# nooice98/HM16.9-NN_FME

Hardware: AMD Instinct MI355X
Metric: sub-pel PU refinements/sec @ 1080p lowdelay_P QP22; bit-exact MV/SATD vs HM (higher is better)
Workload: dtype int16/int32 (NN f32)

## Files before the change

### hm16.9-nn_fme_amd/csrc/fme_api.cpp

```cpp
#include <dlfcn.h>
#include <hsa/hsa.h>
#include <hsa/hsa_ext_amd.h>

#include <chrono>
#include <cmath>
#include <cstdarg>
#include <cstdio>
#include <memory>

#include "fme_ctx.h"

using namespace fme;

namespace {
thread_local std::string g_last_error = "";
}


int fme::fail(int code, const char* fmt, ...) {
  char buf[512];
  va_list ap;
  va_start(ap, fmt);
  vsnprintf(buf, sizeof(buf), fmt, ap);
  va_end(ap);
  g_last_error = buf;
  return code;
}


extern "C" {

int fme_abi_version(void) { return FME_ABI_VERSION; }

const char* fme_last_error(void) { return g_last_error.c_str(); }

int fme_create(int device, const fme_config* cfg, fme_ctx** out_ctx) {
  if (!cfg || !out_ctx) return fail(FME_E_INVALID, "fme_create: null argument");
  *out_ctx = nullptr;
  if (cfg->bit_depth != 8 && cfg->bit_depth != 10)
    return fail(FME_E_UNSUPPORTED, "fme_create: bit_depth %d (8, or 10 for the main10 configurations)", cfg->bit_depth);
  if (cfg->nn_mode < 0 || cfg->nn_mode > 2) return fail(FME_E_INVALID, "fme_create: nn_mode %d", cfg->nn_mode);
  int ndev = 0;
  HIP_TRY(hipGetDeviceCount(&ndev));
  if (device < 0 || device >= ndev) return fail(FME_E_INVALID, "fme_create: device %d of %d", device, ndev);
  HIP_TRY(hipSetDevice(device));
  std::unique_ptr<fme_ctx> c(new fme_ctx());
  c->device = device;
  c->cfg = *cfg;
  HIP_TRY(c->d_pics.reserve(kOvSlots * FME_MAX_PICTURES));
  HIP_TRY(c->d_mlambda.reserve(kOvSlots * FME_MAX_LAMBDAS));
  HIP_TRY(c->d_nn.reserve(kNnPkFloats));
  HIP_TRY(c->counts.reserve(kOvBlocks * kCountWords));
  HIP_TRY(hipMemset(c->counts.p, 0, kOvBlocks * kCountWords * sizeof(int32_t)));
  HIP_TRY(c->d_sched.reserve(kOvSlots));
  HIP_TRY(hipMemset(c->d_sched.p, 0, kOvSlots * sizeof(Schedule)));
  for (auto& e : c->done_ev) HIP_TRY(hipEventCreateWithFlags(&e, hipEventDisableTiming));
  c->sched_p = sched_params();
  {
    const char* m10 = std::getenv("FME_MAIN10_SEARCH");
    c->main10_px = m10 && std::strcmp(m10, "px") == 0;
  }
  HIP_TRY(c->nn_state.reserve(24));
  HIP_TRY(hipMemset(c->nn_state.p, 0, 24 * sizeof(uint32_t)));
  HIP_TRY(c->d_key_invalid.reserve(1));
  HIP_TRY(hipMemset(c->d_key_invalid.p, 0, sizeof(int32_t)));
  HIP_TRY(hipHostMalloc(reinterpret_cast<void**>(&c->h_counts), kCountWords * sizeof(int32_t), hipHostMallocDefault));
  if (cfg->max_jobs > 0) {
    const size_t n = (size_t)cfg->max_jobs;
    const size_t nb = (n + kJobsPerScanBlock - 1) / kJobsPerScanBlock;
    if (n * kNumClasses > (size_t)INT32_MAX) return fail(FME_E_INVALID, "fme_create: max_jobs %d", cfg->max_jobs);
    for (int b = 0; b < kOvSlots; b++) {
      HIP_TRY(c->cls[b].reserve(n));
      HIP_TRY(c->perm[b].reserve(n * kNumClasses));
      HIP_TRY(c->blk_agg[b].reserve(nb * 9));
      HIP_TRY(c->blk_prefix[b].reserve(nb * 9));
    }
  }
  *out_ctx = c.release();
  return FME_OK;
}

}
static int srv_stop(fme_ctx* c);
static hipEvent_t done_event(const fme_ctx* c, int back) {
  if (back < 1 || back > 2 || !c->ov.live[back - 1]) return nullptr;
  return c->done_ev[(c->ov.seq - back) % fme_ctx::kDoneRing];
}
static int wait_batches(fme_ctx* c, hipStream_t s) {
  for (int back = 1; back <= 2; back++)
    if (hipEvent_t e = done_event(c, back))
      if (c->ov.stream[back - 1] != s) HIP_TRY(hipStreamWaitEvent(s, e, 0));
  return FME_OK;
}
static void note_stream(fme_ctx* c, hipStream_t s) {
  for (int i = 0; i < c->n_used_streams; i++)
    if (c->used_streams[i] == s) return;
  if (c->n_used_streams < fme_ctx::kMaxStreams) c->used_streams[c->n_used_streams++] = s;
  else c->used_overflow = true;
}
static int drain_ctx(fme_ctx* c) {
  if (c->used_overflow) {
    HIP_TRY(hipDeviceSynchronize());
  } else {
    for (int i = 0; i < c->n_used_streams; i++) HIP_TRY(hipStreamSynchronize(c->used_streams[i]));
  }
  return FME_OK;
}
int fme::grow_keys(fme_ctx* c, size_t n) {
  c->keys_fresh = true;
  if (n <= c->d_keys.cap) return FME_OK;
  FME_TRY(drain_ctx(c));
  HIP_TRY(c->d_keys.reserve(n));
  return FME_OK;
}
extern "C" {
int fme_destroy(fme_ctx* c) {
  if (!c) return FME_OK;
  (void)hipSetDevice(c->device);
  (void)srv_stop(c);
  (void)hipDeviceSynchronize();
  for (int i = 0; i < FME_MAX_PICTURES; i++)
    if (c->pic_owned[i] && c->pics[i].luma) (void)hipFree(const_cast<uint8_t*>(c->pics[i].luma));
  for (int i = 0; i < FME_MAX_PICTURES; i++)
    if (c->chroma_owned[i]) (void)hipFree(c->chroma_owned[i]);
  c->d_mc_jobs.release(); c->d_mc_planes.release(); c->d_mc_invalid.release(); c->d_mc_wp.release();
  c->d_tz_ext.release(); c->d_tz_sad.release(); c->d_tz_nn_in.release();
  c->d_amvp.release(); c->d_amvp_sad.release(); c->d_bikey.release(); c->d_key_invalid.release(); c->d_ch_i32.release(); c->d_tz_emi.release();
  c->h_pi_tasks.release(); c->h_pi_tsad.release(); c->h_pi_jobs.release(); c->h_pi_ext.release();
  c->h_pi_idx.release(); c->h_pi_psrc.release(); c->h_pi_mv.release(); c->h_pi_last.release();
  c->h_pi_ures.release(); c->h_pi_seq.release(); c->h_pi_rs.release(); c->h_pi_rows.release();
  c->d_pi_jobs.release(); c->d_pi_ext.release(); c->d_pi_idx.release();
  for (auto& e : c->ev_tz)
    if (e) (void)hipEventDestroy(e);
  for (auto& e : c->ev_mc)
    if (e) (void)hipEventDestroy(e);
  c->d_pe_tasks.release(); c->d_pe_dist.release(); c->d_pe_invalid.release();
  for (auto& e : c->ev_pe)
    if (e) (void)hipEventDestroy(e);
  c->d_sse_tasks.release(); c->d_sse_out.release(); c->d_sse_invalid.release();
  for (auto& e : c->ev_sse)
    if (e) (void)hipEventDestroy(e);
  c->d_surf_jobs.release(); c->d_surf_probe.release(); c->d_surf_out.release(); c->d_surf_pick.release();
  c->d_surf_invalid.release();
  for (auto& e : c->ev_surf)
    if (e) (void)hipEventDestroy(e);
  c->d_pics.release(); c->d_mlambda.release(); c->d_keys.release(); c->d_nn.release(); c->d_net.release();
  c->d_jobs.release(); c->d_res.release(); c->d_res1.release(); c->d_mv.release();
  for (int b = 0; b < kOvSlots; b++) {
    c->koff[b].release(); c->cls[b].release(); c->perm[b].release(); c->blk_agg[b].release(); c->blk_prefix[b].release();
  }
  c->counts.release(); c->nn_state.release();
  c->d_sched.release();
  for (auto& e : c->done_ev)
    if (e) (void)hipEventDestroy(e);
  for (auto& e : c->state_read_ev)
    if (e) (void)hipEventDestroy(e);
  if (c->stage) (void)hipHostFree(c->stage);
  if (c->single_stream) (void)hipStreamDestroy(c->single_stream);
  if (c->box) (void)hipHostFree(c->box);
  if (c->srv_stream) (void)hipStreamDestroy(c->srv_stream);
  if (c->h_counts) (void)hipHostFree(c->h_counts);
  if (c->h_tab) (void)hipHostFree(c->h_tab);
  for (auto& e : c->tab_ev)
    if (e) (void)hipEventDestroy(e);
  for (auto& set : c->ev)
    for (auto& e : set)
      if (e) (void)hipEventDestroy(e);
  if (c->ev_fork) (void)hipEventDestroy(c->ev_fork);
  if (c->ev_join2) (void)hipEventDestroy(c->ev_join2);
  if (c->aux2) (void)hipStreamDestroy(c->aux2);
  if (c->ev_join) (void)hipEventDestroy(c->ev_join);
  if (c->aux) (void)hipStreamDestroy(c->aux);
  delete c;
  return FME_OK;
}

static void keep_chroma(fme_ctx* c, int id, int width, int height) {
  const PicDesc& o = c->pics[id];
  if (o.luma && o.width == width && o.height == height) return;
  if (c->chroma_owned[id]) (void)hipFree(c->chroma_owned[id]);
  c->chroma_owned[id] = nullptr;
  c->chroma_bytes[id] = 0;
  c->pics[id].cb = c->pics[id].cr = nullptr;
  c->pics[id].cstride = 0;
}

int fme_set_picture(fme_ctx* c, int id, const uint8_t* luma, int stride, int width, int height, void* stream) {
  if (!c || !luma) return fail(FME_E_INVALID, "fme_set_picture: null argument");
  if (id < 0 || id >= FME_MAX_PICTURES) return fail(FME_E_INVALID, "fme_set_picture: id %d", id);
  if (width <= 0 || height <= 0 || stride < width || width > 65535 || height > 65535)
    return fail(FME_E_INVALID, "fme_set_picture: %dx%d stride %d", width, height, stride);
  HIP_TRY(hipSetDevice(c->device));
  const size_t bps = c->cfg.bit_depth > 8 ? 2 : 1;
  const size_t bytes = (size_t)width * height * bps;
  uint8_t* dst = c->pic_owned[id] ? const_cast<uint8_t*>(c->pics[id].luma) : nullptr;
  if (!dst || c->pic_bytes[id] < bytes) {
    if (dst) HIP_TRY(hipFree(dst));
    dst = nullptr;
    HIP_TRY(hipMalloc(reinterpret_cast<void**>(&dst), bytes));
    c->pic_bytes[id] = bytes;
  }
  hipStream_t s = static_cast<hipStream_t>(stream);
  HIP_TRY(hipMemcpy2DAsync(dst, width * bps, luma, stride * bps, width * bps, height, hipMemcpyHostToDevice, s));
  HIP_TRY(hipStreamSynchronize(s));
  keep_chroma(c, id, width, height);
  c->pics[id] = PicDesc{dst, width, width, height, c->pics[id].cb, c->pics[id].cr, c->pics[id].cstride, 0};
  c->pic_owned[id] = true;
  c->tables_dirty = true;
  return FME_OK;
}

int fme_bind_picture_device(fme_ctx* c, int id, const uint8_t* d_luma, int stride, int width, int height) {
  if (!c || !d_luma) return fail(FME_E_INVALID, "fme_bind_picture_device: null argument");
  if (id < 0 || id >= FME_MAX_PICTURES) return fail(FME_E_INVALID, "fme_bind_picture_device: id %d", id);
  if (width <= 0 || height <= 0 || stride < width) return fail(FME_E_INVALID, "fme_bind_picture_device: geometry");
  HIP_TRY(hipSetDevice(c->device));
  if (c->pic_owned[id] && c->pics[id].luma) HIP_TRY(hipFree(const_cast<uint8_t*>(c->pics[id].luma)));
  c->pic_owned[id] = false;
  c->pic_bytes[id] = 0;
  keep_chroma(c, id, width, height);
  c->pics[id] = PicDesc{d_luma, stride, width, height, c->pics[id].cb, c->pics[id].cr, c->pics[id].cstride, 0};
  c->tables_dirty = true;
  return FME_OK;
}

int fme_set_picture_chroma(fme_ctx* c, int id, const uint8_t* cb, const uint8_t* cr, int stride, void* stream) {
  if (!c || !cb || !cr) return fail(FME_E_INVALID, "fme_set_picture_chroma: null argument");
  if (id < 0 || id >= FME_MAX_PICTURES) return fail(FME_E_INVALID, "fme_set_picture_chroma: id %d", id);
  if (!c->pics[id].luma) return fail(FME_E_STATE, "fme_set_picture_chroma: picture %d has no luma plane", id);
  const int cw = c->pics[id].width >> 1, ch = c->pics[id].height >> 1;
  if (stride < cw) return fail(FME_E_INVALID, "fme_set_picture_chroma: stride %d < %d", stride, cw);
  HIP_TRY(hipSetDevice(c->device));
  const size_t bps = c->cfg.bit_depth > 8 ? 2 : 1;
  const size_t bytes = 2 * (size_t)cw * ch * bps;
  if (!c->chroma_owned[id] || c->chroma_bytes[id] < bytes) {
    if (c->chroma_owned[id]) HIP_TRY(hipFree(c->chroma_owned[id]));
    c->chroma_owned[id] = nullptr;
    HIP_TRY(hipMalloc(reinterpret_cast<void**>(&c->chroma_owned[id]), bytes));
    c->chroma_bytes[id] = bytes;
  }
  uint8_t* dcb = c->chroma_owned[id];
  uint8_t* dcr = dcb + (size_t)cw * ch * bps;
  hipStream_t s = static_cast<hipStream_t>(stream);
  HIP_TRY(hipMemcpy2DAsync(dcb, cw * bps, cb, stride * bps, cw * bps, ch, hipMemcpyHostToDevice, s));
  HIP_TRY(hipMemcpy2DAsync(dcr, cw * bps, cr, stride * bps, cw * bps, ch, hipMemcpyHostToDevice, s));
  HIP_TRY(hipStreamSynchronize(s));
  c->pics[id].cb = dcb;
  c->pics[id].cr = dcr;
  c->pics[id].cstride = cw;
  c->tables_dirty = true;
  return FME_OK;
}

int fme_bind_picture_chroma_device(fme_ctx* c, int id, const uint8_t* d_cb, const uint8_t* d_cr, int stride) {
  if (!c || !d_cb || !d_cr) return fail(FME_E_INVALID, "fme_bind_picture_chroma_device: null argument");
  if (id < 0 || id >= FME_MAX_PICTURES) return fail(FME_E_INVALID, "fme_bind_picture_chroma_device: id %d", id);
  if (!c->pics[id].luma) return fail(FME_E_STATE, "fme_bind_picture_chroma_device: picture %d has no luma plane", id);
  if (stride < (c->pics[id].width >> 1)) return fail(FME_E_INVALID, "fme_bind_picture_chroma_device: stride %d", stride);
  HIP_TRY(hipSetDevice(c->device));
  if (c->chroma_owned[id]) HIP_TRY(hipFree(c->chroma_owned[id]));
  c->chroma_owned[id] = nullptr;
  c->chroma_bytes[id] = 0;
  c->pics[id].cb = d_cb;
  c->pics[id].cr = d_cr;
  c->pics[id].cstride = stride;
  c->tables_dirty = true;
  return FME_OK;
}

int fme_set_lambda(fme_ctx* c, int id, double lambda) {
  if (!c || id < 0 || id >= FME_MAX_LAMBDAS || !(lambda >= 0.0)) return fail(FME_E_INVALID, "fme_set_lambda: bad argument");
  const double sq = std::sqrt(lambda);
  c->mlambda[id] = 65536.0 * sq + 0;
  c->lambda_set[id] = true;
  c->tables_dirty = true;
  return FME_OK;
}

int fme_set_motion_lambda(fme_ctx* c, int id, double ml) {
  if (!c || id < 0 || id >= FME_MAX_LAMBDAS || !(ml >= 0.0)) return fail(FME_E_INVALID, "fme_set_motion_lambda: bad argument");
  c->mlambda[id] = ml;
  c->lambda_set[id] = true;
  c->tables_dirty = true;
  return FME_OK;
}

int fme_set_keys(fme_ctx* c, const int16_t* keys, size_t count, void* stream) {
  if (!c || (!keys && count)) return fail(FME_E_INVALID, "fme_set_keys: null argument");
  HIP_TRY(hipSetDevice(c->device));
  FME_TRY(srv_stop(c));
  FME_TRY(grow_keys(c, count));
  hipStream_t s = static_cast<hipStream_t>(stream);
  FME_TRY(wait_batches(c, s));
  if (count) HIP_TRY(hipMemcpyAsync(c->d_keys.p, keys, count * sizeof(int16_t), hipMemcpyHostToDevice, s));
  HIP_TRY(hipMemsetAsync(c->d_key_invalid.p, 0, sizeof(int32_t), s));
  HIP_TRY(hipStreamSynchronize(s));
  c->n_keys = count;
  return FME_OK;
}

int fme_load_nn_weights(fme_ctx* c, const float* params, int count) {
  if (!c || !params) return fail(FME_E_INVALID, "fme_load_nn_weights: null argument");
  if (count != FME_NN_PARAMS) return fail(FME_E_INVALID, "fme_load_nn_weights: %d params, expected %d", count, FME_NN_PARAMS);
  HIP_TRY(hipSetDevice(c->device));
  std::vector<float> packed(kNnPkFloats);
  nn_pack(params, packed.data());
  HIP_TRY(hipMemcpy(c->d_nn.p, packed.data(), kNnPkFloats * sizeof(float), hipMemcpyHostToDevice));
  c->nn_loaded = true;
  c->nn_gen++;
  return FME_OK;
}

int fme_nn_param_count(const fme_nn_net* n) {
  if (!n) return fail(FME_E_INVALID, "fme_nn_param_count: null descriptor");
  if (n->n_hidden < 1 || n->n_hidden > FME_NN_MAX_HIDDEN)
    return fail(FME_E_INVALID, "fme_nn_param_count: n_hidden %d", n->n_hidden);
  if (n->precision != FME_NN_F32 && n->precision != FME_NN_F64)
    return fail(FME_E_INVALID, "fme_nn_param_count: precision %d", n->precision);
  if (n->embedding < FME_NN_EMB_NONE || n->embedding > FME_NN_EMB_SWAP)
    return fail(FME_E_INVALID, "fme_nn_param_count: embedding %d", n->embedding);
  if (n->out_act != FME_NN_OUT_LINEAR && n->out_act != FME_NN_OUT_SIGMOID)
    return fail(FME_E_INVALID, "fme_nn_param_count: out_act %d", n->out_act);
  if (n->carry_hidden >> n->n_hidden) return fail(FME_E_INVALID, "fme_nn_param_count: carry_hidden 0x%x", n->carry_hidden);
  if (n->input_flags & ~(FME_NN_IN_SLOT_RESET | FME_NN_IN_TZ_RING))
    return fail(FME_E_INVALID, "fme_nn_param_count: input_flags 0x%x", n->input_flags);
  if ((n->input_flags & FME_NN_IN_TZ_RING) && ((n->input_flags & FME_NN_IN_SLOT_RESET) || n->carry_hidden))
    return fail(FME_E_INVALID, "fme_nn_param_count: FME_NN_IN_TZ_RING with FME_NN_IN_SLOT_RESET or carry_hidden");
  int count = n->embedding ? 64 : 0, fan = n->embedding ? 17 : 9;
  for (int l = 0; l < n->n_hidden; l++) {
    const int w = n->width[l];
    if (w < 1 || w > FME_NN_MAX_WIDTH) return fail(FME_E_INVALID, "fme_nn_param_count: width[%d] = %d", l, w);
    count += w * fan + 3 * w;
    fan = w;
  }
  return count + 49 * fan + 49 + 27;
}

int fme_load_nn_net(fme_ctx* c, const fme_nn_net* n, const double* params, int count) {
  if (!c || !n || !params) return fail(FME_E_INVALID, "fme_load_nn_net: null argument");
  const int need = fme_nn_param_count(n);
  if (need < 0) return need;
  if (count != need) return fail(FME_E_INVALID, "fme_load_nn_net: %d params, the descriptor needs %d", count, need);
  if (n->carry_hidden)
    return fail(FME_E_UNSUPPORTED, "fme_load_nn_net: carry_hidden 0x%x (hidden layers carried across calls) is not "
                "supported by the batch engines", n->carry_hidden);
  HIP_TRY(hipSetDevice(c->device));
  const size_t bytes = nn_deep_packed_bytes(*n);
  if (!bytes) return fail(FME_E_UNSUPPORTED, "fme_load_nn_net: no kernel for this net");
  std::vector<unsigned char> packed(bytes);
  nn_deep_pack(*n, params, packed.data());
  FME_TRY(drain_ctx(c));
  HIP_TRY(c->d_net.reserve(bytes));
  HIP_TRY(hipMemcpy(c->d_net.p, packed.data(), bytes, hipMemcpyHostToDevice));
  c->net = *n;
  c->net_loaded = true;
  return FME_OK;
}

int fme_set_nn_engine(fme_ctx* c, int engine) {
  if (!c || (engine != FME_NN_ENGINE_EXACT && engine != FME_NN_ENGINE_MFMA))
    return fail(FME_E_INVALID, "fme_set_nn_engine: bad argument");
  c->nn_engine = engine;
  return FME_OK;
}

int fme_set_nn_logit_output(fme_ctx* c, void* d_logits, int capacity) {
  if (!c) return fail(FME_E_INVALID, "fme_set_nn_logit_output: null ctx");
  if (d_logits && capacity <= 0) return fail(FME_E_INVALID, "fme_set_nn_logit_output: capacity %d", capacity);
  c->nn_logits = capacity > 0 ? d_logits : nullptr;
  c->nn_logits_cap = d_logits ? capacity : 0;
  return FME_OK;
}

int fme_set_nn_inputs(fme_ctx* c, const uint32_t* d_rows, int capacity) {
  if (!c) return fail(FME_E_INVALID, "fme_set_nn_inputs: null ctx");
  if (d_rows && capacity <= 0) return fail(FME_E_INVALID, "fme_set_nn_inputs: capacity %d", capacity);
  c->nn_in = capacity > 0 ? d_rows : nullptr;
  c->nn_in_cap = d_rows ? capacity : 0;
  return FME_OK;
}

int fme_set_nn_margin_output(fme_ctx* c, float* d_margin, int capacity) {
  if (!c) return fail(FME_E_INVALID, "fme_set_nn_margin_output: null ctx");
  if (d_margin && capacity <= 0) return fail(FME_E_INVALID, "fme_set_nn_margin_output: capacity %d", capacity);
  c->nn_margin = capacity > 0 ? d_margin : nullptr;
  c->nn_margin_cap = d_margin ? capacity : 0;
  return FME_OK;
}

int fme_nn_reset_state(fme_ctx* c) {
  if (!c) return fail(FME_E_INVALID, "fme_nn_reset_state: null ctx");
  for (uint32_t& v : c->pending_state) v = 0;
  c->state_pending = true;
  return FME_OK;
}

int fme_nn_get_state(fme_ctx* c, uint32_t* out12) {
  if (!c || !out12) return fail(FME_E_INVALID, "fme_nn_get_state: null argument");
  if (c->state_pending) {
    std::memcpy(out12, c->pending_state, sizeof(c->pending_state));
    return FME_OK;
  }
  HIP_TRY(hipSetDevice(c->device));
  FME_TRY(drain_ctx(c));
  HIP_TRY(hipMemcpy(out12, c->nn_state.p + 12 * c->state_cur, 12 * sizeof(uint32_t), hipMemcpyDeviceToHost));
  return FME_OK;
}

int fme_nn_set_state(fme_ctx* c, const uint32_t* in12) {
  if (!c || !in12) return fail(FME_E_INVALID, "fme_nn_set_state: null argument");
  std::memcpy(c->pending_state, in12, sizeof(c->pending_state));
  c->state_pending = true;
  return FME_OK;
}

int fme_nn_copy_state_device(fme_ctx* c, uint32_t* d_out12, void* stream) {
  if (!c || !d_out12) return fail(FME_E_INVALID, "fme_nn_copy_state_device: null argument");
  HIP_TRY(hipSetDevice(c->device));
  hipStream_t s = static_cast<hipStream_t>(stream);
  if (c->state_pending) {
    HIP_TRY(launch_put_state(d_out12, c->pending_state, s));
    return FME_OK;
  }
  FME_TRY(wait_batches(c, s));
  HIP_TRY(hipMemcpyAsync(d_out12, c->nn_state.p + 12 * c->state_cur, 12 * sizeof(uint32_t),
                         hipMemcpyDeviceToDevice, s));
  hipEvent_t& e = c->state_read_ev[c->state_reads++ % fme_ctx::kDoneRing];
  if (!e) HIP_TRY(hipEventCreateWithFlags(&e, hipEventDisableTiming));
  HIP_TRY(hipEventRecord(e, s));
  c->state_read_last = e;
  c->state_read_stream = s;
  return FME_OK;
}

}

static int ensure_work(fme_ctx* c, int n, bool* grows = nullptr) {
  const size_t nb = ((size_t)n + kJobsPerScanBlock - 1) / kJobsPerScanBlock;
  if ((size_t)n * kNumClasses > (size_t)INT32_MAX) return fail(FME_E_INVALID, "%d jobs in one batch", n);
  if (grows) *grows = (size_t)n > c->cls[0].cap || (size_t)n > c->koff[0].cap;
  for (int b = 0; b < kOvSlots; b++) {
    HIP_TRY(c->cls[b].reserve(n));
    HIP_TRY(c->perm[b].reserve((size_t)n * kNumClasses));
    HIP_TRY(c->blk_agg[b].reserve(nb * 9));
    HIP_TRY(c->blk_prefix[b].reserve(nb * 9));
    HIP_TRY(c->koff[b].reserve(n));
  }
  return FME_OK;
}

static WorkBufs work_bufs(fme_ctx* c, int slot, int block, int zeroed) {
  WorkBufs w{};
  w.cls = c->cls[slot].p;
  w.perm = c->perm[slot].p;
  w.perm_cap = (int32_t)(c->perm[slot].cap / kNumClasses);
  w.koff = c->koff[slot].p;
  w.counts = c->counts.p + block * kCountWords;
  w.counts_next = c->counts.p + zeroed * kCountWords;
  w.cursor = w.counts + kCursorWord;
  w.tile_ctr = w.counts + kTileCtrWord;
  w.blk_agg = c->blk_agg[slot].p;
  w.blk_prefix = c->blk_prefix[slot].p;
  w.nn_state = c->nn_state.p;
  w.sched = c->d_sched.p + slot;
  w.mv_out = nullptr;
  return w;
}

BatchArgs fme::batch_args(const fme_ctx* c, const fme_job* jobs, int n) {
  BatchArgs a{};
  a.jobs = jobs;
  a.keys = c->d_keys.p;
  a.n_keys = (int64_t)c->n_keys;
  a.key_invalid = c->d_key_invalid.p;
  a.mlambda = c->d_mlambda.p;
  a.pics = c->d_pics.p;
  a.n = n;
  a.use_hadamard = c->cfg.use_hadamard ? 1 : 0;
  a.fen = c->cfg.fast_inter_mode;
  return a;
}

static int put_tables(fme_ctx* c, int slot, hipStream_t s) {
  note_stream(c, s);
  FME_TRY(srv_stop(c));
  if (c->tables_dirty) {
    c->tab_gen++;
    c->tables_dirty = false;
  }
  if (c->slot_gen[slot] == c->tab_gen) return FME_OK;
  if (!c->h_tab) {
    void* p = nullptr;
    HIP_TRY(hipHostMalloc(&p, fme_ctx::kTabSlots * sizeof(TablesSlot), hipHostMallocMapped));
    c->h_tab = static_cast<TablesSlot*>(p);
    void* d = nullptr;
    HIP_TRY(hipHostGetDevicePointer(&d, p, 0));
    c->h_tab_dev = static_cast<TablesSlot*>(d);
    for (auto& e : c->tab_ev) HIP_TRY(hipEventCreateWithFlags(&e, hipEventDisableTiming));
  }
  const int k = c->tab_next;
  c->tab_next = (k + 1) % fme_ctx::kTabSlots;
  if (c->tab_used[k]) HIP_TRY(hipEventSynchronize(c->tab_ev[k]));
  std::memcpy(c->h_tab[k].pics, c->pics, sizeof(c->pics));
  std::memcpy(c->h_tab[k].ml, c->mlambda, sizeof(c->mlambda));
  HIP_TRY(launch_put_tables(c->d_pics.p + slot * FME_MAX_PICTURES, c->d_mlambda.p + slot * FME_MAX_LAMBDAS,
                            c->h_tab_dev + k, s));
  HIP_TRY(hipEventRecord(c->tab_ev[k], s));
  c->tab_used[k] = true;
  c->slot_gen[slot] = c->tab_gen;
  return FME_OK;
}

int fme::sync_tables(fme_ctx* c, hipStream_t s) {
  FME_TRY(wait_batches(c, s));
  return put_tables(c, 0, s);
}

static int batch_begin(fme_ctx* c, const OverlapPlan& plan, hipStream_t s, hipEvent_t* done) {
  hipEvent_t const prev_done = done_event(c, 1), slot_done = done_event(c, 2);
  *done = c->done_ev[c->ov.seq % fme_ctx::kDoneRing];
  if (c->ov.seq >= fme_ctx::kDoneRing)
    HIP_TRY(hipEventSynchronize(c->done_ev[(c->ov.seq + 2) % fme_ctx::kDoneRing]));
  if (plan.wait_prev_front) HIP_TRY(hipStreamWaitEvent(s, prev_done, 0));
  if (plan.wait_slot) HIP_TRY(hipStreamWaitEvent(s, slot_done, 0));
  if (plan.fill_blocks) {
    FME_TRY(drain_ctx(c));
    HIP_TRY(hipMemsetAsync(c->counts.p, 0, kOvBlocks * kCountWords * sizeof(int32_t), s));
  }
  return FME_OK;
}

static int apply_pending_state(fme_ctx* c, hipStream_t s) {
  if (!c->state_pending) return FME_OK;
  HIP_TRY(launch_put_state(c->nn_state.p + 12 * c->state_cur, c->pending_state, s));
  c->state_pending = false;
  return FME_OK;
}

static int harvest_events(fme_ctx* c, bool wait_all) {
  while (c->ev_tail != c->ev_head) {
    const int b = c->ev_tail % fme_ctx::kEvSets;
    hipEvent_t* e = c->ev[b];
    if (wait_all) {
      HIP_TRY(hipEventSynchronize(e[6]));
    } else {
      const hipError_t q = hipEventQuery(e[6]);
      if (q == hipErrorNotReady) break;
      HIP_TRY(q);
    }
    float* ms = c->last_ms;
    HIP_TRY(hipEventElapsedTime(&ms[0], e[0], e[3]));
    ms[1] = 0.f;
    HIP_TRY(hipEventElapsedTime(&ms[2], e[3], e[5]));
    HIP_TRY(hipEventElapsedTime(&ms[3], e[5], e[6]));
    HIP_TRY(hipEventElapsedTime(&ms[4], e[0], e[6]));
    HIP_TRY(hipEventElapsedTime(&ms[5], e[3], e[4]));
    ms[6] = 0.f;
    for (int i = 0; i < FME_NUM_TIMINGS; i++) c->acc_ms[i] += ms[i];
    c->acc_batches++;
    c->timed = true;
    c->ev_tail++;
  }
  return FME_OK;
}

int fme::refine_batch(fme_ctx* c, const fme_job* d_jobs, fme_result* d_res, fme_mv_result* d_mv, int n,
                      hipStream_t s, const fme_job_packed* d_pjobs, const int32_t* d_key_base) {
  if (c->cfg.nn_mode == 1 && !c->nn_loaded) return fail(FME_E_STATE, "fme_refine_device: nn_mode set but no weights loaded");
  if (c->cfg.nn_mode == 2 && !c->net_loaded) return fail(FME_E_STATE, "fme_refine_device: nn_mode 2 but no net loaded");
  if (c->cfg.nn_mode == 2 && c->nn_margin && n > c->nn_margin_cap)
    return fail(FME_E_INVALID, "fme_refine: %d jobs but the margin output holds %d", n, c->nn_margin_cap);
  if (c->cfg.nn_mode == 2 && c->nn_logits && n > c->nn_logits_cap)
    return fail(FME_E_INVALID, "fme_refine: %d jobs but the logit output holds %d", n, c->nn_logits_cap);
  HIP_TRY(hipSetDevice(c->device));
  bool grows = false;
  FME_TRY(ensure_work(c, n, &grows));
  const uint32_t features = (c->keys_fresh ? kOvKeys : 0u) | (c->cfg.nn_mode == 2 ? kOvDeepNn : 0u) |
                            (c->cfg.bit_depth > 8 && c->main10_px ? kOvPx : 0u) |
                            (d_jobs && d_jobs == c->d_jobs.p ? kOvStaged : 0u) | (grows ? kOvGrow : 0u);
  const OverlapPlan plan = overlap_plan(c->ov, s, features);
  hipEvent_t const prev_done = done_event(c, 1);
  hipEvent_t done = nullptr;
  FME_TRY(batch_begin(c, plan, s, &done));
  FME_TRY(put_tables(c, plan.slot, s));

  BatchArgs a = batch_args(c, d_jobs, n);
  a.pics = c->d_pics.p + plan.slot * FME_MAX_PICTURES;
  a.mlambda = c->d_mlambda.p + plan.slot * FME_MAX_LAMBDAS;
  a.pjobs = d_jobs ? nullptr : d_pjobs;
  a.key_base = d_key_base;
  a.koff = c->koff[plan.slot].p;
  a.res = d_res;
  a.nn_mode = c->cfg.nn_mode ? 1 : 0;
  a.nn_in = c->nn_in;
  a.nn_in_cap = c->nn_in_cap;
  WorkBufs w = work_bufs(c, plan.slot, plan.block, plan.block_zeroed);
  w.mv_out = d_mv;

  const bool prof = c->profiling;
  hipEvent_t* ev = nullptr;
  int eb = 0;
  if (prof) {
    FME_TRY(harvest_events(c, false));
    if (c->ev_head - c->ev_tail == fme_ctx::kEvSets) {
      HIP_TRY(hipEventSynchronize(c->ev[c->ev_tail % fme_ctx::kEvSets][6]));
      FME_TRY(harvest_events(c, false));
    }
    eb = c->ev_head % fme_ctx::kEvSets;
    ev = c->ev[eb];
    HIP_TRY(hipEventRecord(ev[0], s));
  }
  overlap_begin(c->ov);
  HIP_TRY(launch_front(a, w, c->sched_p, s));
  if (prof) HIP_TRY(hipEventRecord(ev[3], s));
  if (c->ev_search) HIP_TRY(hipEventRecord(c->ev_search, s));
  if (c->cfg.bit_depth > 8) {
    if (c->main10_px)
      HIP_TRY(launch_search_px(a, w, c->cfg.bit_depth, s, nullptr));
    else
      HIP_TRY(launch_search_lane10(a, w, s));
  } else {
    HIP_TRY(launch_search_lane(a, w, c->search_reserve, s));
  }
  if (prof) HIP_TRY(hipEventRecord(ev[4], s));
  if (plan.wait_prev_tail) HIP_TRY(hipStreamWaitEvent(s, prev_done, 0));
  if (c->state_read_last) {
    if (c->state_read_stream != s) HIP_TRY(hipStreamWaitEvent(s, c->state_read_last, 0));
    c->state_read_last = nullptr;
  }
  FME_TRY(apply_pending_state(c, s));
  if (prof) HIP_TRY(hipEventRecord(ev[5], s));
  HIP_TRY(c->cfg.nn_mode == 2
              ? launch_nn_deep_tail(c->net, c->d_net.p, c->nn_margin, c->nn_logits, a, w, c->state_cur, c->nn_engine, s)
              : launch_nn_tail(a, w, c->d_nn.p, c->state_cur, s));
  if (prof) {
    HIP_TRY(hipEventRecord(ev[6], s));
    c->ev_head++;
  }
  HIP_TRY(hipEventRecord(done, s));
  c->ev_done = done;
  c->last_slot = plan.slot;
  c->keys_fresh = false;
  overlap_commit(c->ov, s, features, plan);
  c->batch_issued = true;
  if (a.nn_mode) c->state_cur ^= 1;
  return FME_OK;
}

int fme::check_rejected(fme_ctx* c, hipStream_t s, const char* name, const char* what) {
  HIP_TRY(hipMemcpyAsync(c->h_counts, &c->d_sched.p[c->last_slot].invalid, sizeof(int32_t), hipMemcpyDeviceToHost, s));
  HIP_TRY(hipStreamSynchronize(s));
  if (c->h_counts[0] > 0)
    return fail(FME_E_INVALID, "%s: %d job(s) %s", name, c->h_counts[0], what);
  return FME_OK;
}

static int slot_records(fme_ctx* c, int n, fme_result** out) {
  DevBuf<fme_result>& b = c->ov.seq % kOvSlots ? c->d_res1 : c->d_res;
  HIP_TRY(b.reserve(n));
  *out = b.p;
  return FME_OK;
}

extern "C" {

int fme_refine_device(fme_ctx* c, const fme_job* d_jobs, fme_result* d_res, int n, void* stream) {
  if (!c || (n > 0 && (!d_jobs || !d_res))) return fail(FME_E_INVALID, "fme_refine_device: null argument");
  if (n < 0) return fail(FME_E_INVALID, "fme_refine_device: n = %d", n);
  if (n == 0) return FME_OK;
  return refine_batch(c, d_jobs, d_res, nullptr, n, static_cast<hipStream_t>(stream));
}

int fme_refine_mv_device(fme_ctx* c, const fme_job* d_jobs, fme_mv_result* d_out, int n, void* stream) {
  if (!c || (n > 0 && (!d_jobs || !d_out))) return fail(FME_E_INVALID, "fme_refine_mv_device: null argument");
  if (n < 0) return fail(FME_E_INVALID, "fme_refine_mv_device: n = %d", n);
  if (n == 0) return FME_OK;
  HIP_TRY(hipSetDevice(c->device));
  fme_result* d_res = nullptr;
  FME_TRY(slot_records(c, n, &d_res));
  return refine_batch(c, d_jobs, d_res, d_out, n, static_cast<hipStream_t>(stream));
}

int fme_pack_jobs(const fme_job* jobs, int n, fme_job_packed* out, int32_t* key_base) {
  if (n < 0 || (n > 0 && (!jobs || !out || !key_base))) return fail(FME_E_INVALID, "fme_pack_jobs: bad argument");
  const int waves = (n + FME_PACK_WAVE - 1) / FME_PACK_WAVE;
  for (int wv = 0; wv < waves; wv++) {
    int64_t next = -1;
    key_base[wv] = -1;
    const int e = std::min(n, (wv + 1) * FME_PACK_WAVE);
    for (int i = wv * FME_PACK_WAVE; i < e; i++) {
      const fme_job& j = jobs[i];
      const char* why = nullptr;
      if ((j.x & 3) || (j.y & 3) || (j.w & 3) || (j.h & 3) || j.w < 4 || j.w > 64 || j.h < 4 || j.h > 64)
        why = "PU off the 4x4 grid or not 4..64";
      else if (j.x >= 8192 || j.y >= 8192) why = "x or y >= 8192";
      else if (j.org_id >= 64 || j.ref_id >= 64 || j.lambda_id >= 32) why = "slot id >= 64 or lambda_id >= 32";
      else if (j.flags & ~15u) why = "unknown flags";
      else if (j.bits_in >= 64) why = "bits_in >= 64";
      else if (j.mv_x <= -32767 || j.mv_x >= 32766 || j.mv_y <= -32767 || j.mv_y >= 32766) why = "int16-extreme mv";
      else if (j.key_offset >= 0) {
        if (next < 0) key_base[wv] = j.key_offset;
        else if ((int64_t)j.key_offset != next) why = "key block not dense in job order within its wave";
        next = (int64_t)j.key_offset + (int64_t)j.w * j.h;
      }
      if (why) return fail(FME_E_UNSUPPORTED, "fme_pack_jobs: job %d: %s (use fme_job)", i, why);
      uint32_t rg = 0;
      if (j.mv_y - 1 >= j.lt_y) rg |= FME_PK_RANGE_TOP;
      if (j.mv_y + 1 <= j.rb_y) rg |= FME_PK_RANGE_BOTTOM;
      if (j.mv_x - 1 >= j.lt_x) rg |= FME_PK_RANGE_LEFT;
      if (j.mv_x + 1 <= j.rb_x) rg |= FME_PK_RANGE_RIGHT;
      fme_job_packed p;
      p.pu = (uint32_t)(j.x >> 2) | ((uint32_t)(j.y >> 2) << 11) | ((uint32_t)((j.w >> 2) - 1) << 22) |
             ((uint32_t)((j.h >> 2) - 1) << 26);
      p.ctl = (uint32_t)j.org_id | ((uint32_t)j.ref_id << 6) | ((uint32_t)j.lambda_id << 12) |
              ((uint32_t)j.flags << 17) | ((uint32_t)(j.key_offset >= 0) << 21) | (rg << 22) |
              ((uint32_t)j.bits_in << 26);
      p.mv_x = j.mv_x;
      p.mv_y = j.mv_y;
      p.mvp_x = j.mvp_x;
      p.mvp_y = j.mvp_y;
      out[i] = p;
    }
  }
  return FME_OK;
}

int fme_unpack_jobs(const fme_job_packed* packed, const int32_t* key_base, int n, fme_job* out) {
  if (n < 0 || (n > 0 && (!packed || !key_base || !out))) return fail(FME_E_INVALID, "fme_unpack_jobs: bad argument");
  int64_t next = 0;
  for (int i = 0; i < n; i++) {
    const fme_job_packed& p = packed[i];
    if (i % FME_PACK_WAVE == 0) next = key_base[i / FME_PACK_WAVE];
    fme_job j;
    j.x = (uint16_t)((p.pu & 2047u) * 4u);
    j.y = (uint16_t)(((p.pu >> 11) & 2047u) * 4u);
    j.w = (uint8_t)((((p.pu >> 22) & 15u) + 1u) * 4u);
    j.h = (uint8_t)((((p.pu >> 26) & 15u) + 1u) * 4u);
    j.org_id = (uint8_t)(p.ctl & 63u);
    j.ref_id = (uint8_t)((p.ctl >> 6) & 63u);
    j.lambda_id = (uint8_t)((p.ctl >> 12) & 31u);
    j.flags = (uint8_t)((p.ctl >> 17) & 15u);
    const uint32_t rg = (p.ctl >> 22) & 15u;
    j.bits_in = (uint16_t)(p.ctl >> 26);
    j.mv_x = p.mv_x;
    j.mv_y = p.mv_y;
    j.mvp_x = p.mvp_x;
    j.mvp_y = p.mvp_y;
    j.lt_x = (int16_t)(p.mv_x - ((rg & FME_PK_RANGE_LEFT) ? 1 : 0));
    j.rb_x = (int16_t)(p.mv_x + ((rg & FME_PK_RANGE_RIGHT) ? 1 : 0));
    j.lt_y = (int16_t)(p.mv_y - ((rg & FME_PK_RANGE_TOP) ? 1 : 0));
    j.rb_y = (int16_t)(p.mv_y + ((rg & FME_PK_RANGE_BOTTOM) ? 1 : 0));
    if ((p.ctl >> 21) & 1u) {
      j.key_offset = (int32_t)next;
      next += (int64_t)j.w * j.h;
    } else {
      j.key_offset = -1;
    }
    out[i] = j;
  }
  return FME_OK;
}

static int refine_packed(fme_ctx* c, const fme_job_packed* d_jobs, const int32_t* d_key_base, fme_result* d_res,
                         fme_mv_result* d_mv, int n, void* stream, const char* fn) {
  if (!c || (n > 0 && (!d_jobs || !d_key_base || !(d_res || d_mv)))) return fail(FME_E_INVALID, "%s: null argument", fn);
  if (n < 0) return fail(FME_E_INVALID, "%s: n = %d", fn, n);
  if (n == 0) return FME_OK;
  HIP_TRY(hipSetDevice(c->device));
  if (!d_res) FME_TRY(slot_records(c, n, &d_res));
  return refine_batch(c, nullptr, d_res, d_mv, n, static_cast<hipStream_t>(stream), d_jobs, d_key_base);
}

int fme_refine_packed_device(fme_ctx* c, const fme_job_packed* d_jobs, const int32_t* d_key_base, fme_result* d_res,
                             int n, void* stream) {
  if (c && n > 0 && !d_res) return fail(FME_E_INVALID, "fme_refine_packed_device: null argument");
  return refine_packed(c, d_jobs, d_key_base, d_res, nullptr, n, stream, "fme_refine_packed_device");
}

int fme_refine_mv_packed_device(fme_ctx* c, const fme_job_packed* d_jobs, const int32_t* d_key_base,
                                fme_mv_result* d_out, int n, void* stream) {
  if (c && n > 0 && !d_out) return fail(FME_E_INVALID, "fme_refine_mv_packed_device: null argument");
  return refine_packed(c, d_jobs, d_key_base, nullptr, d_out, n, stream, "fme_refine_mv_packed_device");
}

int fme_set_search_event(fme_ctx* c, void* event) {
  if (!c) return fail(FME_E_INVALID, "fme_set_search_event: null ctx");
  c->ev_search = static_cast<hipEvent_t>(event);
  return FME_OK;
}

int fme_set_search_reserve(fme_ctx* c, int workgroups) {
  if (!c || workgroups < 0 || workgroups > 4096) return fail(FME_E_INVALID, "fme_set_search_reserve: bad argument");
  c->search_reserve = workgroups;
  return FME_OK;
}

int fme_download_device(fme_ctx* c, const void* d_src, void* h_dst, size_t bytes, int workgroups, void* stream) {
  if (!c || (bytes && (!d_src || !h_dst))) return fail(FME_E_INVALID, "fme_download_device: null argument");
  if ((bytes & 15) || (reinterpret_cast<uintptr_t>(d_src) & 15) || (reinterpret_cast<uintptr_t>(h_dst) & 15))
    return fail(FME_E_INVALID, "fme_download_device: pointers and size must be 16-byte multiples");
  if (workgroups < 0 || workgroups > 1024) return fail(FME_E_INVALID, "fme_download_device: %d workgroups", workgroups);
  if (!bytes) return FME_OK;
  HIP_TRY(hipSetDevice(c->device));
  void* dst = nullptr;
  if (hipHostGetDevicePointer(&dst, h_dst, 0) != hipSuccess || !dst) {
    (void)hipGetLastError();
    return fail(FME_E_INVALID, "fme_download_device: h_dst is not pinned host memory");
  }
  HIP_TRY(launch_download(d_src, dst, bytes / 16, workgroups ? workgroups : 8, static_cast<hipStream_t>(stream)));
  return FME_OK;
}

namespace {
struct HsaCopyApi {
  hsa_status_t (*iterate_agents)(hsa_status_t (*)(hsa_agent_t, void*), void*);
  hsa_status_t (*agent_get_info)(hsa_agent_t, hsa_agent_info_t, void*);
  hsa_status_t (*signal_create)(hsa_signal_value_t, uint32_t, const hsa_agent_t*, hsa_signal_t*);
  hsa_status_t (*signal_destroy)(hsa_signal_t);
  hsa_signal_value_t (*signal_wait)(hsa_signal_t, hsa_signal_condition_t, hsa_signal_value_t, uint64_t,
                                    hsa_wait_state_t);
  hsa_status_t (*copy_on_engine)(void*, hsa_agent_t, const void*, hsa_agent_t, size_t, uint32_t,
                                 const hsa_signal_t*, hsa_signal_t, hsa_amd_sdma_engine_id_t, bool);
};
bool hsa_copy_api(HsaCopyApi& a) {
  void* h = dlopen("libhsa-runtime64.so.1", RTLD_LAZY | RTLD_NOLOAD);
  if (!h) h = dlopen("libhsa-runtime64.so.1", RTLD_LAZY);
  if (!h) return false;
  a.iterate_agents = reinterpret_cast<decltype(a.iterate_agents)>(dlsym(h, "hsa_iterate_agents"));
  a.agent_get_info = reinterpret_cast<decltype(a.agent_get_info)>(dlsym(h, "hsa_agent_get_info"));
  a.signal_create = reinterpret_cast<decltype(a.signal_create)>(dlsym(h, "hsa_signal_create"));
  a.signal_destroy = reinterpret_cast<decltype(a.signal_destroy)>(dlsym(h, "hsa_signal_destroy"));
  a.signal_wait = reinterpret_cast<decltype(a.signal_wait)>(dlsym(h, "hsa_signal_wait_scacquire"));
  a.copy_on_engine = reinterpret_cast<decltype(a.copy_on_engine)>(dlsym(h, "hsa_amd_memory_async_copy_on_engine"));
  return a.iterate_agents && a.agent_get_info && a.signal_create && a.signal_destroy && a.signal_wait &&
         a.copy_on_engine;
}
struct AgentPick {
  const HsaCopyApi* api;
  uint32_t bdf, domain;
  bool have_gpu = false, have_cpu = false;
  hsa_agent_t gpu{}, cpu{};
};
hsa_status_t pick_agent(hsa_agent_t ag, void* data) {
  AgentPick* p = static_cast<AgentPick*>(data);
  hsa_device_type_t t;
  if (p->api->agent_get_info(ag, HSA_AGENT_INFO_DEVICE, &t) != HSA_STATUS_SUCCESS) return HSA_STATUS_SUCCESS;
  if (t == HSA_DEVICE_TYPE_CPU && !p->have_cpu) {
    p->cpu = ag;
    p->have_cpu = true;
  } else if (t == HSA_DEVICE_TYPE_GPU && !p->have_gpu) {
    uint32_t bdf = 0, dom = 0;
    p->api->agent_get_info(ag, static_cast<hsa_agent_info_t>(HSA_AMD_AGENT_INFO_BDFID), &bdf);
    p->api->agent_get_info(ag, static_cast<hsa_agent_info_t>(HSA_AMD_AGENT_INFO_DOMAIN), &dom);
    if (bdf == p->bdf && dom == p->domain) {
      p->gpu = ag;
      p->have_gpu = true;
    }
  }
  return HSA_STATUS_SUCCESS;
}
}

int fme_warm_copy_engines(fme_ctx* c, int* engines) {
  if (!c) return fail(FME_E_INVALID, "fme_warm_copy_engines: null ctx");
  if (engines) *engines = 0;
  HIP_TRY(hipSetDevice(c->device));
  HsaCopyApi api{};
  if (!hsa_copy_api(api)) return fail(FME_E_DEVICE, "fme_warm_copy_engines: HSA runtime symbols not found");
  int bus = 0, dev = 0, dom = 0;
  HIP_TRY(hipDeviceGetAttribute(&bus, hipDeviceAttributePciBusId, c->device));
  HIP_TRY(hipDeviceGetAttribute(&dev, hipDeviceAttributePciDeviceId, c->device));
  HIP_TRY(hipDeviceGetAttribute(&dom, hipDeviceAttributePciDomainID, c->device));
  AgentPick pk{&api, (uint32_t)((bus << 8) | (dev << 3)), (uint32_t)dom};
  api.iterate_agents(pick_agent, &pk);
  if (!pk.have_gpu || !pk.have_cpu) return fail(FME_E_DEVICE, "fme_warm_copy_engines: HSA agents not found");
  uint32_t n_sdma = 0, n_xgmi = 0;
  api.agent_get_info(pk.gpu, static_cast<hsa_agent_info_t>(HSA_AMD_AGENT_INFO_NUM_SDMA_ENG), &n_sdma);
  api.agent_get_info(pk.gpu, static_cast<hsa_agent_info_t>(HSA_AMD_AGENT_INFO_NUM_SDMA_XGMI_ENG), &n_xgmi);
  const int n_eng = std::min(16, (int)(n_sdma + n_xgmi));
  constexpr size_t kBytes = 4096;
  void* d = nullptr;
  void* h = nullptr;
  HIP_TRY(hipMalloc(&d, kBytes));
  if (hipHostMalloc(&h, kBytes, hipHostMallocDefault) != hipSuccess) {
    (void)hipFree(d);
    return fail(FME_E_NOMEM, "fme_warm_copy_engines: host buffer");
  }
  std::memset(h, 0, kBytes);
  int warmed = 0;
  for (int e = 0; e < n_eng; e++) {
    bool ok = true;
    for (int dir = 0; dir < 2 && ok; dir++) {
      hsa_signal_t sig;
      if (api.signal_create(1, 0, nullptr, &sig) != HSA_STATUS_SUCCESS) {
        ok = false;
        break;
      }
      const auto eid = static_cast<hsa_amd_sdma_engine_id_t>(1u << e);
      const hsa_status_t st = dir == 0 ? api.copy_on_engine(d, pk.gpu, h, pk.cpu, kBytes, 0, nullptr, sig, eid, true)
                                       : api.copy_on_engine(h, pk.cpu, d, pk.gpu, kBytes, 0, nullptr, sig, eid, true);
      if (st == HSA_STATUS_SUCCESS)
        api.signal_wait(sig, HSA_SIGNAL_CONDITION_LT, 1, UINT64_MAX, HSA_WAIT_STATE_BLOCKED);
      else
        ok = false;
      api.signal_destroy(sig);
    }
    warmed += ok ? 1 : 0;
  }
  (void)hipHostFree(h);
  (void)hipFree(d);
  if (engines) *engines = warmed;
  return FME_OK;
}

int fme_refine_status(fme_ctx* c) {
  if (!c) return fail(FME_E_INVALID, "fme_refine_status: null ctx");
  if (!c->batch_issued) return 0;
  HIP_TRY(hipSetDevice(c->device));
  HIP_TRY(hipEventSynchronize(c->ev_done));
  int32_t v = 0;
  HIP_TRY(hipMemcpy(&v, &c->d_sched.p[c->last_slot].invalid, sizeof(v), hipMemcpyDeviceToHost));
  return v;
}

int fme_debug_front(fme_ctx* c, int32_t* perm_out, long long perm_words, int32_t* sched_out, int sched_words,
                    int32_t* cap_out) {
  if (!c || !c->batch_issued) return fail(FME_E_STATE, "fme_debug_front: no batch issued");
  if (perm_words < 0 || (size_t)perm_words > c->perm[c->last_slot].cap || sched_words < 0 ||
      (size_t)sched_words * sizeof(int32_t) > sizeof(Schedule))
    return fail(FME_E_INVALID, "fme_debug_front: length");
  HIP_TRY(hipSetDevice(c->device));
  HIP_TRY(hipEventSynchronize(c->ev_done));
  if (perm_out && perm_words) HIP_TRY(hipMemcpy(perm_out, c->perm[c->last_slot].p, (size_t)perm_words * sizeof(int32_t), hipMemcpyDeviceToHost));
  if (sched_out && sched_words) HIP_TRY(hipMemcpy(sched_out, c->d_sched.p + c->last_slot, (size_t)sched_words * sizeof(int32_t), hipMemcpyDeviceToHost));
  if (cap_out) *cap_out = (int32_t)(c->perm[c->last_slot].cap / kNumClasses);
  return FME_OK;
}

}

int fme::tz_run(fme_ctx* c, fme_job* d_jobs, const fme_tz_ext* d_ext, uint32_t* d_sad, int n, void* stream,
                int16_t* d_emi, uint32_t* d_nn_in, int ext_stride) {
  if (!c || (n > 0 && (!d_jobs || !d_ext))) return fail(FME_E_INVALID, "fme_integer_search_device: null argument");
  if (n < 0) return fail(FME_E_INVALID, "fme_integer_search_device: n = %d", n);
  if (n == 0) return FME_OK;
  int cw = 0, ch = 0, npic = 0;
  for (int i = 0; i < FME_MAX_PICTURES; i++)
    if (c->pics[i].luma) {
      cw = std::max(cw, (c->pics[i].width + 63) / 64);
      ch = std::max(ch, (c->pics[i].height + 63) / 64);
      npic = i + 1;
    }
  const long long np = (long long)npic * cw * ch;
  if (np > kTzMaxPairs)
    return fail(FME_E_UNSUPPORTED, "fme_integer_search_device: %lld (picture slot, CTU) pairs (%d slots x %d x %d CTUs), the limit is %lld",
                np, npic, cw, ch, kTzMaxPairs);
  HIP_TRY(hipSetDevice(c->device));
  hipStream_t s = static_cast<hipStream_t>(stream);
  FME_TRY(ensure_work(c, n));
  FME_TRY(sync_tables(c, s));
  BatchArgs a = batch_args(c, d_jobs, n);
  a.nn_in = c->nn_in;
  a.nn_in_cap = c->nn_in_cap;
  const OverlapPlan plan = overlap_plan(c->ov, s, kOvForeign);
  hipEvent_t done = nullptr;
  FME_TRY(batch_begin(c, plan, s, &done));
  WorkBufs w = work_bufs(c, plan.slot, plan.block, plan.block_zeroed);
  if (c->profiling) {
    if (!c->ev_tz[0]) {
      HIP_TRY(hipEventCreate(&c->ev_tz[0]));
      HIP_TRY(hipEventCreate(&c->ev_tz[1]));
    }
  }
  overlap_begin(c->ov);
  HIP_TRY(launch_classify(a, w, s));
  HIP_TRY(hipMemcpyAsync(c->h_counts, w.counts, kCountWords * sizeof(int32_t), hipMemcpyDeviceToHost, s));
  HIP_TRY(hipStreamSynchronize(s));
  if (c->h_counts[kNumClasses] > 0)
    return fail(FME_E_INVALID, "fme_integer_search_device: %d job(s) with an unsupported PU size or unset picture/lambda/key",
                c->h_counts[kNumClasses]);
  const bool keyed = c->h_counts[kKeyedWord] > 0;
  HIP_TRY(launch_scatter(a, w, c->sched_p, s));
  TzArgs ta{};
  ta.a = a;
  ta.perm = w.perm;
  ta.jobs_out = d_jobs;
  ta.ext = d_ext;
  ta.ext_stride = ext_stride;
  ta.sad = d_sad;
  ta.emi_mv = d_emi;
  ta.nn_in = d_nn_in;
  if (c->profiling) HIP_TRY(hipEventRecord(c->ev_tz[0], s));
  if (!c->aux) HIP_TRY(hipStreamCreateWithFlags(&c->aux, hipStreamNonBlocking));
  if (!c->aux2) HIP_TRY(hipStreamCreateWithFlags(&c->aux2, hipStreamNonBlocking));
  if (!c->ev_fork) HIP_TRY(hipEventCreateWithFlags(&c->ev_fork, hipEventDisableTiming));
  if (!c->ev_join) HIP_TRY(hipEventCreateWithFlags(&c->ev_join, hipEventDisableTiming));
  if (!c->ev_join2) HIP_TRY(hipEventCreateWithFlags(&c->ev_join2, hipEventDisableTiming));
  const size_t words = 8 + 12 * (size_t)np;
  if (c->d_tzp.cap < words || c->d_tzp_perm.cap < (size_t)n) {
    FME_TRY(drain_ctx(c));
    HIP_TRY(c->d_tzp.reserve(words));
    HIP_TRY(c->d_tzp_perm.reserve(n));
  }
  TzPairs tp{};
  int32_t* b = c->d_tzp.p;
  tp.nseg = b;
  tp.cnt = b + 8;
  tp.cursor = tp.cnt + 3 * np;
  tp.off = tp.cursor + 3 * np;
  tp.seg = tp.off + 3 * np;
  tp.perm = c->d_tzp_perm.p;
  tp.np = (int32_t)np;
  tp.cw = cw;
  tp.ch = ch;
  HIP_TRY(hipMemsetAsync(b, 0, (8 + 3 * (size_t)np) * sizeof(int32_t), s));
  HIP_TRY(launch_tz_pairs(ta, tp, w.cls, n, s));
  HIP_TRY(hipEventRecord(c->ev_fork, s));
  HIP_TRY(hipStreamWaitEvent(c->aux, c->ev_fork, 0));
  HIP_TRY(hipStreamWaitEvent(c->aux2, c->ev_fork, 0));
  HIP_TRY(launch_tz_staged(ta, tp, 0, keyed, c->cfg.bit_depth, c->aux));
  HIP_TRY(launch_tz_staged(ta, tp, 1, keyed, c->cfg.bit_depth, c->aux2));
  HIP_TRY(launch_tz_staged(ta, tp, 2, keyed, c->cfg.bit_depth, s));
  HIP_TRY(hipEventRecord(c->ev_join, c->aux));
  HIP_TRY(hipEventRecord(c->ev_join2, c->aux2));
  HIP_TRY(hipStreamWaitEvent(s, c->ev_join, 0));
  HIP_TRY(hipStreamWaitEvent(s, c->ev_join2, 0));
  if (c->profiling) HIP_TRY(hipEventRecord(c->ev_tz[1], s));
  c->tz_timed = c->profiling;
  HIP_TRY(hipEventRecord(done, s));
  overlap_commit(c->ov, s, kOvForeign, plan);
  return FME_OK;
}

static int tz_run_host(fme_ctx* c, fme_job* jobs, const fme_tz_ext* ext, uint32_t* sad, int n, void* stream,
                       int16_t* emi, uint32_t* nn_in = nullptr, int ext_stride = (int)sizeof(fme_tz_ext)) {
  if (!c || (n > 0 && (!jobs || !ext))) return fail(FME_E_INVALID, "fme_integer_search: null argument");
  if (n <= 0) return n == 0 ? FME_OK : fail(FME_E_INVALID, "fme_integer_search: n = %d", n);
  HIP_TRY(hipSetDevice(c->device));
  hipStream_t s = static_cast<hipStream_t>(stream);
  HIP_TRY(c->d_jobs.reserve(n));
  HIP_TRY(c->d_tz_ext.reserve(((size_t)n * ext_stride + sizeof(fme_tz_ext) - 1) / sizeof(fme_tz_ext)));
  HIP_TRY(c->d_tz_sad.reserve(n));
  if (emi) HIP_TRY(c->d_tz_emi.reserve((size_t)2 * n));
  if (nn_in) HIP_TRY(c->d_tz_nn_in.reserve((size_t)9 * n));
  HIP_TRY(hipMemcpyAsync(c->d_jobs.p, jobs, (size_t)n * sizeof(fme_job), hipMemcpyHostToDevice, s));
  HIP_TRY(hipMemcpyAsync(c->d_tz_ext.p, ext, (size_t)n * ext_stride, hipMemcpyHostToDevice, s));
  if (nn_in) HIP_TRY(hipMemcpyAsync(c->d_tz_nn_in.p, nn_in, (size_t)9 * n * sizeof(uint32_t), hipMemcpyHostToDevice, s));
  int rc = tz_run(c, c->d_jobs.p, c->d_tz_ext.p, c->d_tz_sad.p, n, stream, emi ? c->d_tz_emi.p : nullptr,
                  nn_in ? c->d_tz_nn_in.p : nullptr, ext_stride);
  if (rc) return rc;
  HIP_TRY(hipMemcpyAsync(jobs, c->d_jobs.p, (size_t)n * sizeof(fme_job), hipMemcpyDeviceToHost, s));
  if (sad) HIP_TRY(hipMemcpyAsync(sad, c->d_tz_sad.p, (size_t)n * sizeof(uint32_t), hipMemcpyDeviceToHost, s));
  if (emi) HIP_TRY(hipMemcpyAsync(emi, c->d_tz_emi.p, (size_t)n * 2 * sizeof(int16_t), hipMemcpyDeviceToHost, s));
  if (nn_in) HIP_TRY(hipMemcpyAsync(nn_in, c->d_tz_nn_in.p, (size_t)9 * n * sizeof(uint32_t), hipMemcpyDeviceToHost, s));
  HIP_TRY(hipStreamSynchronize(s));
  return FME_OK;
}

extern "C" {

int fme_integer_search_device(fme_ctx* c, fme_job* d_jobs, const fme_tz_ext* d_ext, uint32_t* d_sad, int n,
                              void* stream) {
  return tz_run(c, d_jobs, d_ext, d_sad, n, stream, nullptr);
}

int fme_integer_search(fme_ctx* c, fme_job* jobs, const fme_tz_ext* ext, uint32_t* sad, int n, void* stream) {
  return tz_run_host(c, jobs, ext, sad, n, stream, nullptr);
}

int fme_integer_search2_device(fme_ctx* c, fme_job* d_jobs, const fme_tz_ext2* d_ext, uint32_t* d_sad, int n,
                               void* stream) {
  return tz_run(c, d_jobs, reinterpret_cast<const fme_tz_ext*>(d_ext), d_sad, n, stream, nullptr, nullptr,
                (int)sizeof(fme_tz_ext2));
}

int fme_integer_search2(fme_ctx* c, fme_job* jobs, const fme_tz_ext2* ext, uint32_t* sad, int n, void* stream) {
  return tz_run_host(c, jobs, reinterpret_cast<const fme_tz_ext*>(ext), sad, n, stream, nullptr, nullptr,
                     (int)sizeof(fme_tz_ext2));
}

int fme_integer_search_ring_device(fme_ctx* c, fme_job* d_jobs, const fme_tz_ext* d_ext, uint32_t* d_sad,
                                   uint32_t* d_nn_in, int n, void* stream) {
  if (!d_nn_in && n > 0) return fail(FME_E_INVALID, "fme_integer_search_ring_device: null nn_in");
  return tz_run(c, d_jobs, d_ext, d_sad, n, stream, nullptr, d_nn_in);
}

int fme_integer_search_ring(fme_ctx* c, fme_job* jobs, const fme_tz_ext* ext, uint32_t* sad, uint32_t* nn_in,
                            int n, void* stream) {
  if (!nn_in && n > 0) return fail(FME_E_INVALID, "fme_integer_search_ring: null nn_in");
  return tz_run_host(c, jobs, ext, sad, n, stream, nullptr, nn_in);
}

int fme_integer_search_last_ms(fme_ctx* c, float* ms) {
  if (!c || !ms) return fail(FME_E_INVALID, "fme_integer_search_last_ms: null argument");
  if (!c->tz_timed) return fail(FME_E_STATE, "fme_integer_search_last_ms: no profiled integer search");
  HIP_TRY(hipEventSynchronize(c->ev_tz[1]));
  HIP_TRY(hipEventElapsedTime(ms, c->ev_tz[0], c->ev_tz[1]));
  return FME_OK;
}

static int refine_host(fme_ctx* c, const fme_job* jobs, fme_result* res, fme_mv_result* mv, int n, void* stream,
                       const char* name) {
  if (!c || (n > 0 && (!jobs || (!res && !mv)))) return fail(FME_E_INVALID, "%s: null argument", name);
  if (n <= 0) return n == 0 ? FME_OK : fail(FME_E_INVALID, "%s: n = %d", name, n);
  HIP_TRY(hipSetDevice(c->device));
  hipStream_t s = static_cast<hipStream_t>(stream);
  HIP_TRY(c->d_jobs.reserve(n));
  HIP_TRY(c->d_res.reserve(n));
  if (mv) HIP_TRY(c->d_mv.reserve(n));
  HIP_TRY(hipMemcpyAsync(c->d_jobs.p, jobs, (size_t)n * sizeof(fme_job), hipMemcpyHostToDevice, s));
  FME_TRY(refine_batch(c, c->d_jobs.p, c->d_res.p, mv ? c->d_mv.p : nullptr, n, s));
  if (mv)
    HIP_TRY(hipMemcpyAsync(mv, c->d_mv.p, (size_t)n * sizeof(fme_mv_result), hipMemcpyDeviceToHost, s));
  else
    HIP_TRY(hipMemcpyAsync(res, c->d_res.p, (size_t)n * sizeof(fme_result), hipMemcpyDeviceToHost, s));
  return check_rejected(c, s, name, "with an unsupported PU size or unset picture/lambda/key");
}

int fme_refine(fme_ctx* c, const fme_job* jobs, fme_result* res, int n, void* stream) {
  return refine_host(c, jobs, res, nullptr, n, stream, "fme_refine");
}

int fme_refine_mv(fme_ctx* c, const fme_job* jobs, fme_mv_result* out, int n, void* stream) {
  return refine_host(c, jobs, nullptr, out, n, stream, "fme_refine_mv");
}

static int ensure_stage(fme_ctx* c) {
  if (c->stage) return FME_OK;
  void* p = nullptr;
  HIP_TRY(hipHostMalloc(&p, sizeof(SingleStage), hipHostMallocMapped));
  c->stage = static_cast<SingleStage*>(p);
  void* d = nullptr;
  HIP_TRY(hipHostGetDevicePointer(&d, p, 0));
  c->stage_dev = static_cast<uint8_t*>(d);
  HIP_TRY(hipStreamCreateWithFlags(&c->single_stream, hipStreamNonBlocking));
  std::memset(c->stage, 0, sizeof(SingleStage));
  return FME_OK;
}

static int class_of(int w, int h) {
  for (int k = 0; k < kNumClasses; k++)
    if (kClassW[k] == w && kClassH[k] == h) return k;
  return -1;
}

static int single_wait(fme_ctx* c, uint32_t seq) {
  volatile uint32_t* f = &c->stage->flag;
  for (long it = 1; *f != seq; it++) {
    __builtin_ia32_pause();
    if ((it & 1023) == 0) {
      const hipError_t q = hipStreamQuery(c->single_stream);
      if (q != hipErrorNotReady && *f != seq) {
        if (q != hipSuccess) return fail(FME_E_DEVICE, "single-PU kernel: %s", hipGetErrorString(q));
        return fail(FME_E_DEVICE, "single-PU kernel ended without its completion word");
      }
    }
  }
  __atomic_thread_fence(__ATOMIC_ACQUIRE);
  return FME_OK;
}

constexpr uint64_t kSrvIdleUs = 2000;
constexpr uint64_t kSrvLifeMs = 100;

static int srv_open(fme_ctx* c) {
  if (c->box) return FME_OK;
  void* p = nullptr;
  HIP_TRY(hipHostMalloc(&p, sizeof(SrvBox), hipHostMallocMapped));
  std::memset(p, 0, sizeof(SrvBox));
  c->box = static_cast<SrvBox*>(p);
  void* d = nullptr;
  HIP_TRY(hipHostGetDevicePointer(&d, p, 0));
  c->box_dev = static_cast<SrvBox*>(d);
  HIP_TRY(hipStreamCreateWithFlags(&c->srv_stream, hipStreamNonBlocking));
  int khz = 0;
  if (hipDeviceGetAttribute(&khz, hipDeviceAttributeWallClockRate, c->device) == hipSuccess && khz > 0)
    c->srv_khz = (uint64_t)khz;
  return FME_OK;
}

static int srv_launch(fme_ctx* c) {
  if (c->srv_orphan) {
    const hipError_t q = hipStreamQuery(c->srv_stream);
    if (q == hipErrorNotReady)
      return fail(FME_E_DEVICE, "single-call server: the instance that timed out is still running");
    (void)hipGetLastError();
    c->srv_orphan = false;
  }
  __atomic_store_n(&c->box->req[0][3], 0u, __ATOMIC_RELEASE);
  const uint32_t epoch = ++c->srv_epoch;
  c->srv_nn_gen = c->nn_gen;
  HIP_TRY(launch_server(c->box_dev, c->nn_loaded ? c->d_nn.p : nullptr, c->srv_done, epoch,
                        kSrvIdleUs * c->srv_khz / 1000, kSrvLifeMs * c->srv_khz, c->cfg.bit_depth, c->srv_stream));
  c->srv_running = true;
  return FME_OK;
}

constexpr double kSrvWaitLimitS = 2.0;
static bool srv_waited_too_long(std::chrono::steady_clock::time_point t0) {
  return std::chrono::duration<double>(std::chrono::steady_clock::now() - t0).count() > kSrvWaitLimitS;
}

static int srv_join(fme_ctx* c) {
  volatile uint32_t* st = &c->box->stopped;
  const auto t0 = std::chrono::steady_clock::now();
  for (long it = 1; *st != c->srv_epoch; it++) {
    __builtin_ia32_pause();
    if ((it & 1023) == 0) {
      const hipError_t q = hipStreamQuery(c->srv_stream);
      if (q != hipErrorNotReady && *st != c->srv_epoch) {
        c->srv_running = false;
        if (q != hipSuccess) return fail(FME_E_DEVICE, "single-call server: %s", hipGetErrorString(q));
        return fail(FME_E_DEVICE, "single-call server ended without its stop word");
      }
      if (srv_waited_too_long(t0)) {
        c->srv_running = false;
        c->srv_orphan = true;
        return fail(FME_E_DEVICE, "single-call server: no stop word after %.1f s", kSrvWaitLimitS);
      }
    }
  }
  c->srv_running = false;
  HIP_TRY(hipStreamSynchronize(c->srv_stream));
  return FME_OK;
}

static int srv_stop(fme_ctx* c) {
  if (!c->srv_running) return FME_OK;
  __atomic_store_n(&c->box->req[0][3], 1u, __ATOMIC_RELEASE);
  return srv_join(c);
}

static int srv_call(fme_ctx* c, bool uses_nn) {
  int rc = FME_OK;
  if (c->srv_running && uses_nn && c->srv_nn_gen != c->nn_gen) rc = srv_stop(c);
  if (!rc && !c->srv_running) rc = srv_launch(c);
  if (rc) return rc;
  const uint32_t seq = c->srv_done + 1;
  __atomic_store_n(&c->box->req[0][0], seq, __ATOMIC_RELEASE);
  volatile uint32_t* done = &c->box->res[0];
  volatile uint32_t* st = &c->box->stopped;
  const auto t0 = std::chrono::steady_clock::now();
  for (long it = 1; *done != seq; it++) {
    __builtin_ia32_pause();
    if (*st == c->srv_epoch && *done != seq) {
      c->srv_running = false;
      HIP_TRY(hipStreamSynchronize(c->srv_stream));
      if (srv_waited_too_long(t0))
        return fail(FME_E_DEVICE, "single-call server: call %u unanswered after %.1f s", seq, kSrvWaitLimitS);
      FME_TRY(srv_launch(c));
    } else if ((it & 4095) == 0) {
      const hipError_t q = hipStreamQuery(c->srv_stream);
      if (q != hipErrorNotReady && q != hipSuccess) {
        c->srv_running = false;
        return fail(FME_E_DEVICE, "single-call server: %s", hipGetErrorString(q));
      }
      if (srv_waited_too_long(t0)) {
        __atomic_store_n(&c->box->req[0][3], 1u, __ATOMIC_RELEASE);
        if (srv_join(c) != FME_OK) c->srv_orphan = true;
        c->srv_running = false;
        return fail(FME_E_DEVICE, "single-call server: call %u unanswered after %.1f s", seq, kSrvWaitLimitS);
      }
    }
  }
  __atomic_thread_fence(__ATOMIC_ACQUIRE);
  c->srv_done = seq;
  return FME_OK;
}

int fme_frac_dif_single(fme_ctx* c, int lossless, const int16_t* key, int key_stride, int w, int h,
                        const int16_t* ref, int ref_stride, int mv_int_x, int mv_int_y, int mvp_x,
                        int mvp_y, double motion_lambda, int16_t* half_xy, int16_t* qtr_xy,
                        uint32_t* cost) {
  if (!c || !key || !ref || !half_xy || !qtr_xy || !cost) return fail(FME_E_INVALID, "fme_frac_dif_single: null argument");
  const int cls = class_of(w, h);
  if (cls < 0) return fail(FME_E_UNSUPPORTED, "fme_frac_dif_single: %dx%d", w, h);
  const int px = mvp_x - 4 * mv_int_x, py = mvp_y - 4 * mv_int_y;
  if (px < -32768 || px > 32767 || py < -32768 || py > 32767) return fail(FME_E_INVALID, "fme_frac_dif_single: predictor out of range");
  HIP_TRY(hipSetDevice(c->device));
  FME_TRY(srv_open(c));
  SrvBox* b = c->box;
  srv_pack_frac(b, c->srv_done + 1, c->cfg.bit_depth, lossless || !c->cfg.use_hadamard, c->srv_marks, key, key_stride, w,
                h, ref, ref_stride, mv_int_x, mv_int_y, px, py, motion_lambda);
  FME_TRY(srv_call(c, false));
  const uint32_t hq = b->res[2];
  half_xy[0] = (int16_t)(int8_t)(hq & 0xFF);
  half_xy[1] = (int16_t)(int8_t)((hq >> 8) & 0xFF);
  qtr_xy[0] = (int16_t)(int8_t)((hq >> 16) & 0xFF);
  qtr_xy[1] = (int16_t)(int8_t)(hq >> 24);
  *cost = b->res[1];
  return FME_OK;
}

int fme_nn_pred_single(fme_ctx* c, const uint32_t* e, uint32_t cc, int pu_h, int pu_w, int* nn_class, int16_t* out4) {
  if (!c || !e || !nn_class) return fail(FME_E_INVALID, "fme_nn_pred_single: null argument");
  const bool deep = c->cfg.nn_mode == 2;
  if (deep ? !c->net_loaded : !c->nn_loaded) return fail(FME_E_STATE, "fme_nn_pred_single: no weights loaded");
  HIP_TRY(hipSetDevice(c->device));
  int rc;
  if (!deep) {
    FME_TRY(srv_open(c));
    const uint32_t in[12] = {e[0], e[1], e[2], e[3], e[4], e[5], e[6], e[7], cc, (uint32_t)pu_h, (uint32_t)pu_w, 0u};
    const uint32_t seq = c->srv_done + 1;
    for (int b = 1; b < 5; b++) {
      for (int k = 0; k < 3; k++) c->box->req[b][1 + k] = in[3 * (b - 1) + k];
      __atomic_store_n(&c->box->req[b][0], seq, __ATOMIC_RELEASE);
    }
    c->box->req[0][1] = kSrvNn | (c->srv_marks ? (uint32_t)kSrvMarks : 0u);
    FME_TRY(srv_call(c, true));
    *nn_class = (int)c->box->res[1];
  } else {
  rc = srv_stop(c);
  if (!rc) rc = ensure_stage(c);
  if (rc) return rc;
  NnIn11 in{};
  for (int s = 0; s < 8; s++) in.v[s] = e[s];
  in.v[8] = cc;
  in.v[9] = (uint32_t)pu_h;
  in.v[10] = (uint32_t)pu_w;
  int32_t* d_out = reinterpret_cast<int32_t*>(c->stage_dev + offsetof(SingleStage, nn_out));
  uint32_t* d_flag = reinterpret_cast<uint32_t*>(c->stage_dev + offsetof(SingleStage, flag));
  const uint32_t seq = ++c->single_seq;
  HIP_TRY(launch_nn_deep_single(c->net, c->d_net.p, in, d_out, d_flag, seq, c->single_stream));
  FME_TRY(single_wait(c, seq));
  *nn_class = c->stage->nn_out[0];
  }
  const int cls = *nn_class;
  if (out4) {
    const int ox = cls % 7 - 3, oy = cls / 7 - 3;
    auto split = [](int o, int16_t& hf, int16_t& qt) {
      static const int8_t H[7] = {-1, -1, 0, 0, 0, 1, 1}, Q[7] = {-1, 0, -1, 0, 1, 0, 1};
      hf = H[o + 3];
      qt = Q[o + 3];
    };
    split(ox, out4[0], out4[1]);
    split(oy, out4[2], out4[3]);
  }
  return FME_OK;
}

int fme_single_last_device_us(fme_ctx* c, float* us, int count) {
  if (!c || (count > 0 && !us)) return fail(FME_E_INVALID, "fme_single_last_device_us: null argument");
  const double k = 1000.0 / (double)c->srv_khz;
  if (count > 1) c->srv_marks = true;
  for (int i = 0; i < count && i < 5; i++)
    us[i] = !c->box ? 0.0f : (float)((double)(i == 0 ? c->box->res[3] : c->box->marks[i - 1]) * k);
  return FME_OK;
}

int fme_search_kernel_of_shape(int width, int height) {
  for (int k = 0; k < kNumClasses; k++)
    if (kClassW[k] == width && kClassH[k] == height) {
      return 0;
    }
  return -1;
}

static const char* mc_job_problem(const fme_ctx* c, const fme_mc_job& j, int width, int height) {
  if (j.w < 4 || j.h < 4 || j.w > 64 || j.h > 64 || (j.w & 3) || (j.h & 3)) return "PU size";
  if (!(j.flags & (FME_MC_L0 | FME_MC_L1)) || (j.flags & ~(FME_MC_L0 | FME_MC_L1 | FME_MC_WP))) return "list flags";
  if ((int)j.x + j.w > width || (int)j.y + j.h > height) return "PU outside the picture";
  for (int l = 0; l < 2; l++) {
    if (!(j.flags & (1u << l))) continue;
    if (j.ref_id[l] >= FME_MAX_PICTURES) return "reference id";
    const PicDesc& p = c->pics[j.ref_id[l]];
    if (!p.luma || !p.cb || !p.cr) return "reference picture without luma + chroma";
    if (p.width != width || p.height != height) return "reference picture dimensions";
  }
  return nullptr;
}

static int mc_launch(fme_ctx* c, const fme_mc_job* d_jobs, int n, uint8_t* y, int ys, uint8_t* cb, uint8_t* cr,
                     int cs, int width, int height, hipStream_t s) {
  HIP_TRY(c->d_mc_invalid.reserve(1));
  HIP_TRY(hipMemsetAsync(c->d_mc_invalid.p, 0, sizeof(int32_t), s));
  if (int e = sync_tables(c, s)) return e;
  if (!c->wp_init) {
    for (auto& l : c->h_wp)
      for (auto& p : l)
        for (auto& q : p) q = fme_wp_param{1, 0, 0, {0, 0, 0}};
    c->wp_init = true;
  }
  if (c->wp_dirty) {
    HIP_TRY(c->d_mc_wp.reserve(sizeof(c->h_wp) / sizeof(fme_wp_param)));
    HIP_TRY(hipMemcpyAsync(c->d_mc_wp.p, c->h_wp, sizeof(c->h_wp), hipMemcpyHostToDevice, s));
    c->wp_dirty = false;
  }
  McArgs a{};
  a.wp = c->d_mc_wp.p;
  a.jobs = d_jobs;
  a.pics = c->d_pics.p;
  a.y = y;
  a.cb = cb;
  a.cr = cr;
  a.invalid = c->d_mc_invalid.p;
  a.n = n;
  a.y_stride = ys;
  a.c_stride = cs;
  a.width = width;
  a.height = height;
  a.bit_depth = c->cfg.bit_depth;
  if (c->profiling) {
    if (!c->ev_mc[0]) {
      HIP_TRY(hipEventCreate(&c->ev_mc[0]));
      HIP_TRY(hipEventCreate(&c->ev_mc[1]));
    }
    HIP_TRY(hipEventRecord(c->ev_mc[0], s));
  }
  HIP_TRY(launch_mc(a, s));
  if (c->profiling) HIP_TRY(hipEventRecord(c->ev_mc[1], s));
  c->mc_timed = c->profiling;
  return FME_OK;
}

static int mc_check_planes(const void* y, int ys, const void* cb, const void* cr, int cs, int width, int height) {
  if (!y || !cb || !cr) return fail(FME_E_INVALID, "motion compensation: null plane");
  if (width <= 0 || height <= 0 || (width & 1) || (height & 1) || ys < width || cs < width / 2)
    return fail(FME_E_INVALID, "motion compensation: geometry %dx%d strides %d/%d", width, height, ys, cs);
  return FME_OK;
}

int fme_motion_compensate(fme_ctx* c, const fme_mc_job* jobs, int n, uint8_t* y, int ys, uint8_t* cb, uint8_t* cr,
                          int cs, int width, int height, void* stream) {
  if (!c || (n > 0 && !jobs) || n < 0) return fail(FME_E_INVALID, "fme_motion_compensate: bad argument");
  if (int e = mc_check_planes(y, ys, cb, cr, cs, width, height)) return e;
  for (int i = 0; i < n; i++)
    if (const char* why = mc_job_problem(c, jobs[i], width, height))
      return fail(FME_E_INVALID, "fme_motion_compensate: job %d: %s", i, why);
  if (n == 0) return FME_OK;
  HIP_TRY(hipSetDevice(c->device));
  hipStream_t s = static_cast<hipStream_t>(stream);
  const size_t bps = c->cfg.bit_depth > 8 ? 2 : 1;
  const size_t ly = (size_t)width * height * bps, lc = ly / 4;
  HIP_TRY(c->d_mc_jobs.reserve(n));
  HIP_TRY(c->d_mc_planes.reserve(ly + 2 * lc));
  uint8_t* dy = c->d_mc_planes.p;
  uint8_t* dcb = dy + ly;
  uint8_t* dcr = dcb + lc;
  const int cw = width / 2, ch = height / 2;
  HIP_TRY(hipMemcpyAsync(c->d_mc_jobs.p, jobs, n * sizeof(fme_mc_job), hipMemcpyHostToDevice, s));
  HIP_TRY(hipMemcpy2DAsync(dy, width * bps, y, ys * bps, width * bps, height, hipMemcpyHostToDevice, s));
  HIP_TRY(hipMemcpy2DAsync(dcb, cw * bps, cb, cs * bps, cw * bps, ch, hipMemcpyHostToDevice, s));
  HIP_TRY(hipMemcpy2DAsync(dcr, cw * bps, cr, cs * bps, cw * bps, ch, hipMemcpyHostToDevice, s));
  if (int e = mc_launch(c, c->d_mc_jobs.p, n, dy, width, dcb, dcr, cw, width, height, s)) return e;
  HIP_TRY(hipMemcpy2DAsync(y, ys * bps, dy, width * bps, width * bps, height, hipMemcpyDeviceToHost, s));
  HIP_TRY(hipMemcpy2DAsync(cb, cs * bps, dcb, cw * bps, cw * bps, ch, hipMemcpyDeviceToHost, s));
  HIP_TRY(hipMemcpy2DAsync(cr, cs * bps, dcr, cw * bps, cw * bps, ch, hipMemcpyDeviceToHost, s));
  HIP_TRY(hipStreamSynchronize(s));
  return FME_OK;
}

int fme_motion_compensate_device(fme_ctx* c, const fme_mc_job* d_jobs, int n, uint8_t* d_y, int ys, uint8_t* d_cb,
                                 uint8_t* d_cr, int cs, int width, int height, void* stream) {
  if (!c || (n > 0 && !d_jobs) || n < 0) return fail(FME_E_INVALID, "fme_motion_compensate_device: bad argument");
  if (int e = mc_check_planes(d_y, ys, d_cb, d_cr, cs, width, height)) return e;
  HIP_TRY(hipSetDevice(c->device));
  return mc_launch(c, d_jobs, n, d_y, ys, d_cb, d_cr, cs, width, height, static_cast<hipStream_t>(stream));
}

int fme_mc_invalid_count(fme_ctx* c) {
  if (!c) return fail(FME_E_INVALID, "fme_mc_invalid_count: null ctx");
  if (!c->d_mc_invalid.p) return 0;
  HIP_TRY(hipSetDevice(c->device));
  int32_t v = 0;
  FME_TRY(drain_ctx(c));
  HIP_TRY(hipMemcpy(&v, c->d_mc_invalid.p, sizeof(v), hipMemcpyDeviceToHost));
  return v;
}

int fme_set_wp(fme_ctx* c, int list, int ref_id, const fme_wp_param* p) {
  if (!c || !p) return fail(FME_E_INVALID, "fme_set_wp: null argument");
  if (list < 0 || list > 1 || ref_id < 0 || ref_id >= FME_MAX_PICTURES)
    return fail(FME_E_INVALID, "fme_set_wp: list %d reference %d", list, ref_id);
  for (int k = 0; k < 3; k++)
    if (p[k].log2_denom > 7) return fail(FME_E_INVALID, "fme_set_wp: log2 denominator %d", (int)p[k].log2_denom);
  if (!c->wp_init) {
    for (auto& l : c->h_wp)
      for (auto& q : l)
        for (auto& r : q) r = fme_wp_param{1, 0, 0, {0, 0, 0}};
    c->wp_init = true;
  }
  for (int k = 0; k < 3; k++) c->h_wp[list][ref_id][k] = p[k];
  c->wp_dirty = true;
  return FME_OK;
}

int fme_mc_last_ms(fme_ctx* c, float* ms) {
  if (!c || !ms) return fail(FME_E_INVALID, "fme_mc_last_ms: null argument");
  if (!c->mc_timed) return fail(FME_E_STATE, "fme_mc_last_ms: no profiled motion compensation");
  HIP_TRY(hipEventSynchronize(c->ev_mc[1]));
  HIP_TRY(hipEventElapsedTime(ms, c->ev_mc[0], c->ev_mc[1]));
  return FME_OK;
}

int fme_set_profiling(fme_ctx* c, int enable) {
  if (!c) return fail(FME_E_INVALID, "fme_set_profiling: null ctx");
  HIP_TRY(hipSetDevice(c->device));
  if (enable && !c->events_made) {
    for (auto& set : c->ev)
      for (auto& e : set) HIP_TRY(hipEventCreate(&e));
    c->events_made = true;
  }
  if (!enable) FME_TRY(harvest_events(c, true));
  c->profiling = enable != 0;
  return FME_OK;
}

int fme_last_timings(fme_ctx* c, float* ms, int count) {
  if (!c || !ms || count < 0) return fail(FME_E_INVALID, "fme_last_timings: null argument");
  HIP_TRY(hipSetDevice(c->device));
  FME_TRY(harvest_events(c, true));
  if (!c->timed) return fail(FME_E_STATE, "fme_last_timings: no profiled batch");
  for (int i = 0; i < count && i < FME_NUM_TIMINGS; i++) ms[i] = c->last_ms[i];
  return FME_OK;
}

int fme_accumulated_timings(fme_ctx* c, double* ms, int count, int reset) {
  if (!c || (count > 0 && !ms) || count < 0) return fail(FME_E_INVALID, "fme_accumulated_timings: null argument");
  HIP_TRY(hipSetDevice(c->device));
  FME_TRY(harvest_events(c, true));
  const int n = c->acc_batches;
  for (int i = 0; i < count && i < FME_NUM_TIMINGS; i++) ms[i] = c->acc_ms[i];
  if (reset) {
    for (double& v : c->acc_ms) v = 0.0;
    c->acc_batches = 0;
  }
  return n;
}

}
```

### hm16.9-nn_fme_amd/csrc/fme_ctx.h

```cpp
#pragma once

#include <hip/hip_runtime.h>

#include <algorithm>
#include <cstdlib>
#include <cstring>
#include <string>
#include <thread>
#include <vector>

#include "fme_device.h"
#include "fme_overlap_host.h"

namespace fme {

int fail(int code, const char* fmt, ...);

#define HIP_TRY(expr)                                                                            \
  do {                                                                                           \
    hipError_t _e = (expr);                                                                      \
    if (_e != hipSuccess)                                                                        \
      return fme::fail(_e == hipErrorOutOfMemory ? FME_E_NOMEM : FME_E_DEVICE, "%s: %s (%s:%d)", \
                       #expr, hipGetErrorString(_e), __FILE__, __LINE__);                        \
  } while (0)

#define FME_TRY(expr)           \
  do {                          \
    const int _rc = (expr);     \
    if (_rc) return _rc;        \
  } while (0)

template <typename T, bool kPinned>
struct Buf {
  T* p = nullptr;
  size_t cap = 0;
  hipError_t reserve(size_t n) {
    if (n <= cap) return hipSuccess;
    release();
    const size_t want = std::max<size_t>(kPinned ? n + n / 4 : n, 1);
    void** const pp = reinterpret_cast<void**>(&p);
    hipError_t e = kPinned ? hipHostMalloc(pp, want * sizeof(T), hipHostMallocDefault) : hipMalloc(pp, want * sizeof(T));
    if (e == hipSuccess) cap = kPinned ? want : n;
    return e;
  }
  void release() {
    if (p) (void)(kPinned ? hipHostFree(p) : hipFree(p));
    p = nullptr;
    cap = 0;
  }
};
template <typename T> using DevBuf = Buf<T, false>;
template <typename T> using HostBuf = Buf<T, true>;

template <typename F>
void par_for(int n, F&& f) {
  const unsigned hc = std::thread::hardware_concurrency();
  const int nt = n < 32768 ? 1 : (int)std::min<unsigned>(8u, hc ? hc : 1u);
  if (nt <= 1) {
    f(0, n);
    return;
  }
  std::vector<std::thread> th;
  th.reserve((size_t)nt - 1);
  for (int t = 1; t < nt; t++)
    th.emplace_back([&f, n, nt, t] { f((int)((long long)n * t / nt), (int)((long long)n * (t + 1) / nt)); });
  f(0, (int)((long long)n / nt));
  for (auto& x : th) x.join();
}
}

struct SingleStage {
  int32_t nn_out[4];
  uint32_t flag;
};

struct fme_ctx {
  int device = 0;
  fme_config cfg{};
  fme::PicDesc pics[FME_MAX_PICTURES]{};
  bool pic_owned[FME_MAX_PICTURES]{};
  size_t pic_bytes[FME_MAX_PICTURES]{};
  double mlambda[FME_MAX_LAMBDAS]{};
  bool lambda_set[FME_MAX_LAMBDAS]{};
  bool tables_dirty = true;

  fme::DevBuf<fme::PicDesc> d_pics;
  fme::DevBuf<double> d_mlambda;
  unsigned long long tab_gen = 1, slot_gen[fme::kOvSlots] = {};
  static constexpr int kTabSlots = 16;
  fme::TablesSlot* h_tab = nullptr;
  fme::TablesSlot* h_tab_dev = nullptr;
  hipEvent_t tab_ev[kTabSlots] = {};
  bool tab_used[kTabSlots] = {};
  int tab_next = 0;
  fme::DevBuf<int16_t> d_keys;
  size_t n_keys = 0;
  fme::DevBuf<float> d_nn;
  bool nn_loaded = false;
  fme_nn_net net{};
  fme::DevBuf<uint8_t> d_net;
  bool net_loaded = false;
  int nn_engine = FME_NN_ENGINE_EXACT;
  float* nn_margin = nullptr;
  int nn_margin_cap = 0;
  void* nn_logits = nullptr;
  int nn_logits_cap = 0;
  const uint32_t* nn_in = nullptr;
  int nn_in_cap = 0;

  fme::DevBuf<fme_job> d_jobs;
  fme::DevBuf<fme_result> d_res;
  fme::DevBuf<fme_result> d_res1;
  fme::DevBuf<fme_mv_result> d_mv;
  fme::DevBuf<int32_t> koff[fme::kOvSlots];
  fme::DevBuf<uint8_t> cls[fme::kOvSlots];
  fme::DevBuf<int32_t> perm[fme::kOvSlots];
  fme::DevBuf<int32_t> blk_agg[fme::kOvSlots];
  fme::DevBuf<int32_t> blk_prefix[fme::kOvSlots];
  fme::DevBuf<int32_t> counts;
  fme::OverlapState ov;
  static constexpr int kDoneRing = 16;
  hipEvent_t done_ev[kDoneRing] = {};
  hipEvent_t state_read_ev[kDoneRing] = {};
  long long state_reads = 0;
  hipEvent_t state_read_last = nullptr;
  hipStream_t state_read_stream = nullptr;
  int last_slot = 0;
  bool keys_fresh = false;
  fme::DevBuf<uint32_t> nn_state;
  int state_cur = 0;
  bool state_pending = false;
  uint32_t pending_state[12] = {};
  fme::DevBuf<fme::Schedule> d_sched;
  fme::SchedParams sched_p{};
  int32_t* h_counts = nullptr;

  uint8_t* chroma_owned[FME_MAX_PICTURES]{};
  size_t chroma_bytes[FME_MAX_PICTURES]{};
  fme::DevBuf<fme_mc_job> d_mc_jobs;
  fme::DevBuf<uint8_t> d_mc_planes;
  fme::DevBuf<int32_t> d_mc_invalid;
  fme_wp_param h_wp[2][FME_MAX_PICTURES][3] = {};
  bool wp_init = false, wp_dirty = true;
  fme::DevBuf<fme_wp_param> d_mc_wp;
  hipEvent_t ev_mc[2] = {nullptr, nullptr};
  bool mc_timed = false;
  fme::DevBuf<fme_pe_task> d_pe_tasks;
  fme::DevBuf<uint32_t> d_pe_dist;
  fme::DevBuf<int32_t> d_pe_invalid;
  std::vector<fme_pe_task> h_pe_tasks;
  std::vector<uint32_t> h_pe_dist;
  hipStream_t pe_stream = nullptr;
  hipEvent_t ev_pe[2] = {nullptr, nullptr};
  bool pe_timed = false;
  fme::DevBuf<fme_sse_task> d_sse_tasks;
  fme::DevBuf<uint32_t> d_sse_out;
  fme::DevBuf<int32_t> d_sse_invalid;
  std::vector<fme_sse_task> h_sse_tasks;
  std::vector<uint32_t> h_sse_out;
  hipStream_t sse_stream = nullptr;
  hipEvent_t ev_sse[2] = {nullptr, nullptr};
  bool sse_timed = false;
  fme::DevBuf<fme_job> d_surf_jobs;
  fme::DevBuf<uint8_t> d_surf_probe;
  fme::DevBuf<fme_surface> d_surf_out;
  fme::DevBuf<fme_surface_pick> d_surf_pick;
  fme::DevBuf<int32_t> d_surf_invalid;
  hipStream_t surf_stream = nullptr;
  hipEvent_t ev_surf[2] = {nullptr, nullptr};
  bool surf_timed = false;
  fme::DevBuf<fme_tz_ext> d_tz_ext;
  fme::DevBuf<uint32_t> d_tz_sad;
  fme::DevBuf<uint32_t> d_tz_nn_in;
  hipEvent_t ev_tz[2] = {nullptr, nullptr};
  bool tz_timed = false;
  double pi_ms[FME_PI_PHASES] = {};
  int16_t int_mv_2n[2][FME_MAX_REFS][2] = {};
  fme::DevBuf<fme::AmvpTask> d_amvp;
  fme::DevBuf<int16_t> d_tz_emi;
  fme::DevBuf<uint32_t> d_amvp_sad;
  fme::DevBuf<fme::BiKeyTask> d_bikey;
  fme::DevBuf<int32_t> d_key_invalid;
  fme::DevBuf<int32_t> d_ch_i32;
  fme::DevBuf<int32_t> d_tzp;
  fme::DevBuf<int32_t> d_tzp_perm;
  fme::HostBuf<fme::AmvpTask> h_pi_tasks;
  fme::HostBuf<uint32_t> h_pi_tsad;
  fme::HostBuf<fme_job> h_pi_jobs;
  fme::HostBuf<fme_tz_ext> h_pi_ext;
  fme::HostBuf<int32_t> h_pi_idx;
  fme::HostBuf<int32_t> h_pi_psrc;
  fme::HostBuf<fme_mv_result> h_pi_mv;
  fme::HostBuf<fme_result> h_pi_last;
  fme::HostBuf<fme_result> h_pi_ures;
  fme::HostBuf<fme_job> h_pi_seq;
  fme::HostBuf<fme_mv_result> h_pi_rs;
  fme::HostBuf<uint32_t> h_pi_rows;
  std::vector<int> pi_base, pi_task, pi_src, pi_lvl, pi_start, pi_byarea;
  std::vector<int32_t> pi_off, pi_fill;
  std::vector<uint8_t> pi_amvp_idx;
  fme::DevBuf<fme_job> d_pi_jobs;
  fme::DevBuf<fme_tz_ext> d_pi_ext;
  fme::DevBuf<int32_t> d_pi_idx;

  struct SingleStage* stage = nullptr;
  uint8_t* stage_dev = nullptr;
  hipStream_t single_stream = nullptr;
  uint32_t single_seq = 0;
  fme::SrvBox* box = nullptr;
  fme::SrvBox* box_dev = nullptr;
  hipStream_t srv_stream = nullptr;
  bool srv_running = false;
  bool srv_orphan = false;
  static constexpr int kMaxStreams = 8;
  hipStream_t used_streams[kMaxStreams] = {};
  int n_used_streams = 0;
  bool used_overflow = false;
  uint32_t srv_epoch = 0;
  uint32_t srv_done = 0;
  uint32_t srv_nn_gen = 0;
  uint32_t nn_gen = 0;
  uint64_t srv_khz = 100000;
  bool srv_marks = false;

  static constexpr int kEv = 9;
  static constexpr int kEvSets = 32;
  bool profiling = false;
  bool events_made = false;
  hipEvent_t ev[kEvSets][kEv] = {};
  long long ev_head = 0;
  long long ev_tail = 0;
  bool timed = false;
  hipEvent_t ev_done = nullptr;
  hipEvent_t ev_search = nullptr;
  int search_reserve = 0;
  bool main10_px = false;
  bool batch_issued = false;
  float last_ms[FME_NUM_TIMINGS] = {};
  double acc_ms[FME_NUM_TIMINGS] = {};
  int acc_batches = 0;

  hipStream_t aux = nullptr;
  hipStream_t aux2 = nullptr;
  hipEvent_t ev_join2 = nullptr;
  hipEvent_t ev_fork = nullptr, ev_join = nullptr;
};

namespace fme {
size_t nn_deep_packed_bytes(const fme_nn_net& n);
void nn_deep_pack(const fme_nn_net& n, const double* params, void* out);
hipError_t launch_nn_deep_tail(const fme_nn_net& n, const void* packed, float* margin, void* logits, const BatchArgs& a,
                               const WorkBufs& w, int state_in, int engine, hipStream_t s);
hipError_t launch_nn_deep_single(const fme_nn_net& n, const void* packed, const NnIn11& in11, int32_t* out,
                                 uint32_t* flag, uint32_t seq, hipStream_t s);

int sync_tables(fme_ctx* c, hipStream_t s);
int grow_keys(fme_ctx* c, size_t n);
BatchArgs batch_args(const fme_ctx* c, const fme_job* jobs, int n);
int refine_batch(fme_ctx* c, const fme_job* d_jobs, fme_result* d_res, fme_mv_result* d_mv, int n, hipStream_t s,
                 const fme_job_packed* d_pjobs = nullptr, const int32_t* d_key_base = nullptr);
int tz_run(fme_ctx* c, fme_job* d_jobs, const fme_tz_ext* d_ext, uint32_t* d_sad, int n, void* stream, int16_t* d_emi,
           uint32_t* d_nn_in = nullptr, int ext_stride = (int)sizeof(fme_tz_ext));
int check_rejected(fme_ctx* c, hipStream_t s, const char* name, const char* what);
}
```

### hm16.9-nn_fme_amd/csrc/fme_device.h

```cpp
#pragma once

#include <hip/hip_runtime.h>
#include <stdint.h>

#include "../../include/fme.h"
#include "../../include/fme_merge.h"
#include "../../include/fme_skip.h"
#include "../../include/fme_surface.h"
#include "fme_srv_pack.h"

namespace fme {

constexpr int kNumClasses = 24;

#ifndef FME_LANE_ORDER
#define FME_LANE_ORDER 0
#endif
__host__ __device__ __forceinline__ constexpr int lane_class_at(int pos) {
  return FME_LANE_ORDER == 1 ? kNumClasses - 1 - pos
         : FME_LANE_ORDER == 2 ? ((pos & 1) ? kNumClasses - 1 - (pos >> 1) : (pos >> 1))
                               : pos;
}
constexpr int kBlock = 256;
constexpr int kJobsPerScanBlock = 1024;
constexpr int kKeyedWord = 25;
constexpr int kTicketWord = 28;
constexpr int kCursorWord = 32;
constexpr int kTileCtrWord = 64;
constexpr int kCountWords = 96;
static_assert(kNumClasses < kKeyedWord && kKeyedWord < kTicketWord && kTicketWord < 32 && kCursorWord + kNumClasses + 2 <= 64 &&
                  kTileCtrWord + 8 <= kCountWords, "counter block");

constexpr int kClassW[kNumClasses] = {4, 8, 8, 4, 16, 8, 16, 12, 16, 16, 8, 32,
                                      16, 32, 24, 32, 32, 16, 64, 32, 64, 48, 64, 64};
constexpr int kClassH[kNumClasses] = {8, 4, 8, 16, 4, 16, 8, 16, 12, 16, 32, 8,
                                      32, 16, 32, 24, 32, 64, 16, 64, 32, 64, 48, 64};

struct PicDesc {
  const uint8_t* luma;
  int32_t stride, width, height;
  const uint8_t* cb;
  const uint8_t* cr;
  int32_t cstride;
  int32_t pad_;
};

template <class Args>
inline hipError_t launch_by_depth(void (*k8)(Args), void (*k10)(Args), int grid, int block, const Args& a,
                                  hipStream_t s) {
  if (a.n > 0) hipLaunchKernelGGL(a.bit_depth > 8 ? k10 : k8, dim3(grid), dim3(block), 0, s, a);
  return hipGetLastError();
}

struct McArgs {
  const fme_mc_job* jobs;
  const PicDesc* pics;
  uint8_t* y;
  uint8_t* cb;
  uint8_t* cr;
  int32_t* invalid;
  int32_t n, y_stride, c_stride, width, height;
  int32_t bit_depth;
  const fme_wp_param* wp;
};
hipError_t launch_mc(const McArgs& a, hipStream_t s);

struct AmvpTask {
  uint16_t x, y;
  uint8_t w, h, org_id, ref_id;
  uint16_t cu_x, cu_y;
  int16_t mv_x, mv_y;
};
static_assert(sizeof(AmvpTask) == 16, "AmvpTask layout");
struct AmvpArgs {
  const AmvpTask* tasks;
  const PicDesc* pics;
  uint32_t* sad;
  int32_t n;
  int32_t bit_depth;
};
hipError_t launch_amvp_sad(const AmvpArgs& a, hipStream_t s);

struct BiKeyTask {
  uint16_t x, y;
  uint8_t w, h, org_id, ref_id;
  uint16_t cu_x, cu_y;
  int16_t mv_x, mv_y;
  int32_t key_off;
  uint32_t clip;
};
static_assert(sizeof(BiKeyTask) == 24, "BiKeyTask layout");
struct BiKeyArgs {
  const BiKeyTask* tasks;
  const PicDesc* pics;
  int16_t* keys;
  int32_t n;
  int32_t* invalid;
  int64_t n_keys;
  int32_t bit_depth;
};
hipError_t launch_bi_key(const BiKeyArgs& a, hipStream_t s);

struct PeArgs {
  const fme_pe_task* tasks;
  const PicDesc* pics;
  uint32_t* dist;
  int32_t* invalid;
  int32_t n;
  int32_t bit_depth;
  int32_t use_hadamard;
};
hipError_t launch_pred_err(const PeArgs& a, hipStream_t s);

struct SseArgs {
  const fme_sse_task* tasks;
  const PicDesc* pics;
  uint32_t* sse;
  int32_t* invalid;
  int32_t n;
  int32_t bit_depth;
};
hipError_t launch_pred_sse(const SseArgs& a, hipStream_t s);

struct SurfArgs {
  const fme_job* jobs;
  const uint8_t* probe;
  fme_surface* surf;
  fme_surface_pick* pick;
  const PicDesc* pics;
  const double* mlambda;
  const int16_t* keys;
  int64_t n_keys;
  int32_t* invalid;
  int32_t n;
  int32_t bit_depth;
  int32_t use_hadamard;
};
hipError_t launch_cost_surface(const SurfArgs& a, hipStream_t s);


struct BatchArgs {
  const fme_job* jobs;
  const fme_job_packed* pjobs;
  const int32_t* key_base;
  const int32_t* koff;
  fme_result* res;
  const int16_t* keys;
  int64_t n_keys;
  const double* mlambda;
  const PicDesc* pics;
  int32_t n;
  int32_t use_hadamard;
  int32_t fen;
  int32_t nn_mode;
  const int32_t* key_invalid;
  const uint32_t* nn_in;
  int32_t nn_in_cap;
};

struct Schedule;

struct WorkBufs {
  uint8_t* cls;
  int32_t* perm;
  int32_t* koff;
  int32_t* counts;
  int32_t* counts_next;
  int32_t* cursor;
  int32_t* blk_agg;
  int32_t* blk_prefix;
  uint32_t* nn_state;
  Schedule* sched;
  int32_t* tile_ctr;
  fme_mv_result* mv_out;
  int32_t perm_cap;
};
__device__ __forceinline__ const fme_result* search_rec(const BatchArgs& a, const WorkBufs&, int i) { return a.res + i; }

struct Schedule {
  int32_t prefix[kNumClasses + 1];
  int32_t class_off[kNumClasses];
  int32_t class_cnt[kNumClasses];
  int32_t xq[8][kNumClasses + 1];
  int32_t invalid;
  int32_t pad_[3];
};
__device__ __forceinline__ int sched_count(const Schedule* sc, int c0, int c1) {
  int n = 0;
  for (int c = c0; c < c1; c++) n += sc->class_cnt[c];
  return n;
}
__device__ __forceinline__ int sched_perm_index(const Schedule* sc, int c0, int c1, int q) {
  int c = c0;
  for (; c < c1 - 1 && q >= sc->class_cnt[c]; c++) q -= sc->class_cnt[c];
  return sc->class_off[c] + q;
}

struct SchedParams {
  int32_t lanes[kNumClasses];
};
SchedParams sched_params();

struct TzArgs {
  BatchArgs a;
  const int32_t* perm;
  fme_job* jobs_out;
  const fme_tz_ext* ext;
  uint32_t* sad;
  int16_t* emi_mv;
  uint32_t* nn_in;
  int32_t ext_stride;
};
__device__ __forceinline__ fme_tz_ext tz_ext_at(const TzArgs& ta, int i) {
  return *reinterpret_cast<const fme_tz_ext*>(reinterpret_cast<const uint8_t*>(ta.ext) + (size_t)ta.ext_stride * i);
}
__device__ __forceinline__ void tz_pred_at(const TzArgs& ta, int i, int k, int& x, int& y) {
  if (ta.ext_stride < (int)sizeof(fme_tz_ext2)) {
    x = y = 0;
    return;
  }
  const fme_tz_ext2* e = reinterpret_cast<const fme_tz_ext2*>(reinterpret_cast<const uint8_t*>(ta.ext) + (size_t)ta.ext_stride * i);
  x = e->preds[k][0];
  y = e->preds[k][1];
}
constexpr long long kTzMaxPairs = 1LL << 20;
struct TzPairs {
  int32_t* cnt;
  int32_t* cursor;
  int32_t* off;
  int32_t* seg;
  int32_t* nseg;
  int32_t* perm;
  int32_t np, cw, ch;
};
hipError_t launch_tz_pairs(const TzArgs& ta, const TzPairs& tp, const uint8_t* cls, int n, hipStream_t s);
hipError_t launch_tz_staged(const TzArgs& ta, const TzPairs& tp, int kid, bool keyed, int bit_depth, hipStream_t s);
struct TzChain {
  const int32_t* psrc;
  int32_t nlev;
};
hipError_t launch_tz_levels(const TzArgs& ta, const TzChain& ch, const int32_t* h_lvl_off, int bit_depth, hipStream_t s);

hipError_t launch_front(const BatchArgs& a, const WorkBufs& w, const SchedParams& p, hipStream_t s);
hipError_t launch_classify(const BatchArgs& a, const WorkBufs& w, hipStream_t s);
hipError_t launch_scatter(const BatchArgs& a, const WorkBufs& w, const SchedParams& p, hipStream_t s);
hipError_t launch_put_state(uint32_t* dst, const uint32_t* v12, hipStream_t s);
struct TablesSlot {
  PicDesc pics[FME_MAX_PICTURES];
  double ml[FME_MAX_LAMBDAS];
};
hipError_t launch_put_tables(PicDesc* d_pics, double* d_ml, const TablesSlot* t_dev, hipStream_t s);
hipError_t launch_search_lane(const BatchArgs& a, const WorkBufs& w, int reserve, hipStream_t s);
hipError_t launch_search_px(const BatchArgs& a, const WorkBufs& w, int bit_depth, hipStream_t s, hipStream_t s_big);
hipError_t launch_search_lane10(const BatchArgs& a, const WorkBufs& w, hipStream_t s);
struct NnIn11 {
  uint32_t v[11];
};
hipError_t launch_server(SrvBox* box, const float* nn, uint32_t served, uint32_t epoch, uint64_t idle_ticks,
                         uint64_t life_ticks, int bit_depth, hipStream_t s);
int lane_lanes_per_pu(int cls);
int lane_grid(int n, int reserve);
int cu_count(int device);
constexpr int kNnPkPfx = 0;
constexpr int kNnPkW1 = kNnPkPfx + 64 * 22;
constexpr int kNnPkW2 = kNnPkW1 + 11 * 9 * 2;
constexpr int kNnPkW3 = kNnPkW2 + 10 * 22 * 2;
constexpr int kNnPkB1 = kNnPkW3 + 25 * 20 * 2;
constexpr int kNnPkG1 = kNnPkB1 + 22;
constexpr int kNnPkBE1 = kNnPkG1 + 22;
constexpr int kNnPkB2 = kNnPkBE1 + 22;
constexpr int kNnPkG2 = kNnPkB2 + 20;
constexpr int kNnPkBE2 = kNnPkG2 + 20;
constexpr int kNnPkBout = kNnPkBE2 + 20;
constexpr int kNnPkGin = kNnPkBout + 50;
constexpr int kNnPkMean = kNnPkGin + 9;
constexpr int kNnPkStd = kNnPkMean + 9;
constexpr int kNnPkFloats = kNnPkStd + 9 + 1;
static_assert(kNnPkW1 % 2 == 0 && kNnPkW2 % 2 == 0 && kNnPkW3 % 2 == 0 && kNnPkB1 % 2 == 0 &&
              kNnPkG1 % 2 == 0 && kNnPkBE1 % 2 == 0 && kNnPkB2 % 2 == 0 && kNnPkG2 % 2 == 0 &&
              kNnPkBE2 % 2 == 0 && kNnPkBout % 2 == 0, "pair regions must be 8-byte aligned");
void nn_pack(const float* params, float* packed);
__device__ __forceinline__ int emb_row_h(int h) {
  return h == 4 ? 1 : h == 8 ? 2 : h == 16 ? 3 : h == 12 ? 4 : h == 24 ? 5 : h == 32 ? 6 : h == 64 ? 7 : 0;
}
__device__ __forceinline__ int emb_row_w(int w) {
  return w == 4 ? 1 : w == 8 ? 2 : w == 12 ? 3 : w == 16 ? 4 : w == 24 ? 5 : w == 32 ? 6 : w == 64 ? 7 : 0;
}
typedef float f2 __attribute__((ext_vector_type(2)));
__device__ __forceinline__ f2 ld2(const float* __restrict__ Q, int o) { return *(const f2*)(Q + o); }
__device__ __forceinline__ f2 relu2(f2 s) {
  s.x = s.x < 0.0f ? 0.0f : s.x;
  s.y = s.y < 0.0f ? 0.0f : s.y;
  return s;
}
hipError_t launch_download(const void* src, void* dst, size_t n16, int wgs, hipStream_t s);
hipError_t launch_gather_jobs(const fme_job* src, const fme_tz_ext* src_ext, const int32_t* idx, fme_job* dst,
                              fme_tz_ext* dst_ext, int n, hipStream_t s);
hipError_t launch_nn_tail(const BatchArgs& a, const WorkBufs& w, const float* nn_params,
                          int state_in, hipStream_t s);

typedef uint32_t job_u4 __attribute__((ext_vector_type(4), aligned(4)));
typedef __attribute__((address_space(1))) const job_u4 g_job_u4;
typedef __attribute__((address_space(1))) const uint32_t g_job_u32;
typedef __attribute__((address_space(1))) const int32_t g_job_i32;

__device__ __forceinline__ bool packed_keyed(uint32_t ctl) { return ((ctl >> 21) & 1u) != 0; }
__device__ __forceinline__ fme_job expand_job(job_u4 p, int32_t key_offset) {
  const uint32_t pu = p.x, ctl = p.y;
  const uint32_t rg = (ctl >> 22) & 15u;
  const int16_t mv_x = (int16_t)(p.z & 0xFFFFu), mv_y = (int16_t)(p.z >> 16);
  fme_job j;
  j.x = (uint16_t)((pu & 2047u) * 4u);
  j.y = (uint16_t)(((pu >> 11) & 2047u) * 4u);
  j.w = (uint8_t)((((pu >> 22) & 15u) + 1u) * 4u);
  j.h = (uint8_t)((((pu >> 26) & 15u) + 1u) * 4u);
  j.org_id = (uint8_t)(ctl & 63u);
  j.ref_id = (uint8_t)((ctl >> 6) & 63u);
  j.lambda_id = (uint8_t)((ctl >> 12) & 31u);
  j.flags = (uint8_t)((ctl >> 17) & 15u);
  j.bits_in = (uint16_t)(ctl >> 26);
  j.mv_x = mv_x;
  j.mv_y = mv_y;
  j.mvp_x = (int16_t)(p.w & 0xFFFFu);
  j.mvp_y = (int16_t)(p.w >> 16);
  j.lt_x = (int16_t)(mv_x - ((rg & FME_PK_RANGE_LEFT) ? 1 : 0));
  j.rb_x = (int16_t)(mv_x + ((rg & FME_PK_RANGE_RIGHT) ? 1 : 0));
  j.lt_y = (int16_t)(mv_y - ((rg & FME_PK_RANGE_TOP) ? 1 : 0));
  j.rb_y = (int16_t)(mv_y + ((rg & FME_PK_RANGE_BOTTOM) ? 1 : 0));
  j.key_offset = packed_keyed(ctl) ? key_offset : -1;
  return j;
}
__device__ __forceinline__ job_u4 packed_row(const BatchArgs& a, int i) { return *((g_job_u4*)a.pjobs + i); }

__device__ __forceinline__ fme_job load_job(const BatchArgs& a, int i) {
  if (a.pjobs) {
    const job_u4 p = packed_row(a, i);
    int32_t ko = -1;
    if (packed_keyed(p.y)) ko = ((g_job_i32*)a.koff)[i];
    return expand_job(p, ko);
  }
  g_job_u4* const src = (g_job_u4*)(a.jobs + i);
  const job_u4 q0 = src[0], q1 = src[1];
  const uint32_t tmp[8] = {q0.x, q0.y, q0.z, q0.w, q1.x, q1.y, q1.z, q1.w};
  fme_job j;
  __builtin_memcpy(&j, tmp, sizeof(j));
  return j;
}
static_assert(sizeof(fme_job) == 32 && sizeof(fme_job_packed) == 16, "job layouts");
__device__ __forceinline__ void load_job_wh(const BatchArgs& a, int i, uint32_t& w, uint32_t& h) {
  if (a.pjobs) {
    const uint32_t pu = *(g_job_u32*)&a.pjobs[i].pu;
    w = (((pu >> 22) & 15u) + 1u) * 4u;
    h = (((pu >> 26) & 15u) + 1u) * 4u;
  } else {
    const uint32_t q = ((g_job_u32*)(a.jobs + i))[1];
    w = q & 0xFFu;
    h = (q >> 8) & 0xFFu;
  }
}

__device__ __forceinline__ int nn_pushes(const fme_job& j) {
  if (j.flags & FME_JOB_NN_IN) return 8;
  if (!(j.flags & FME_JOB_EMI)) return 0;
  const bool top = j.mv_y - 1 >= j.lt_y, bot = j.mv_y + 1 <= j.rb_y;
  const bool left = j.mv_x - 1 >= j.lt_x, right = j.mv_x + 1 <= j.rb_x;
  const int cols = 1 + (left ? 1 : 0) + (right ? 1 : 0);
  return (top ? cols : 0) + (left ? 1 : 0) + (right ? 1 : 0) + (bot ? cols : 0);
}
__device__ __forceinline__ bool nn_writes_c(const fme_job& j) { return (j.flags & (FME_JOB_EMI | FME_JOB_NN_IN)) != 0; }

__device__ __forceinline__ void store_outputs(fme_result* r, const fme_result* src, fme_mv_result* mv_out, int i,
                                              int fx, int fy, uint32_t cost, uint32_t bits, uint8_t cls,
                                              uint16_t status) {
  if (mv_out) {
    fme_mv_result o;
    o.mv_x = (int16_t)fx;
    o.mv_y = (int16_t)fy;
    o.cost = cost;
    o.bits = bits;
    o.nn_class = cls;
    o.reserved = 0;
    o.status = status;
    mv_out[i] = o;
  } else {
    if (src != r) *r = *src;
    r->mv_x = (int16_t)fx;
    r->mv_y = (int16_t)fy;
    r->cost = cost;
    r->bits = bits;
    r->nn_class = cls;
    r->status = status;
  }
}

template <int NW>
__device__ __forceinline__ void writer_scan(const int (&run)[9], const int (&carry)[9], int base,
                                            int32_t (*wave_tot)[9], int (&src)[9], int (&tot)[9]) {
  const int lane = (int)threadIdx.x & 63, wid = (int)threadIdx.x >> 6;
  const int wbase = base + 64 * wid;
  const unsigned long long below = ~0ull >> (63 - lane);
  int incl[9];
#pragma unroll
  for (int f = 0; f < 9; f++) {
    const unsigned long long mask = __ballot(run[f] >= 0);
    const unsigned long long m = mask & below;
    incl[f] = m ? wbase + 63 - __clzll(m) : -1;
    if (lane == 0) wave_tot[wid][f] = mask ? wbase + 63 - __clzll(mask) : -1;
  }
  __syncthreads();
#pragma unroll
  for (int f = 0; f < 9; f++) {
    const int t = lane < NW ? wave_tot[lane][f] : -1;
    const unsigned long long pm = __ballot(lane < wid && t >= 0);
    const unsigned long long am = __ballot(t >= 0);
    const int prev = pm ? __builtin_amdgcn_readlane(t, 63 - __clzll(pm)) : carry[f];
    src[f] = max(incl[f], prev);
    tot[f] = am ? __builtin_amdgcn_readlane(t, 63 - __clzll(am)) : carry[f];
  }
}

__device__ __forceinline__ void writer_scan_wave(const BatchArgs& a, const int (&run)[9], const int32_t* carry,
                                                 int wbase, int (&src)[9]) {
  const int lane = (int)threadIdx.x & 63;
  const unsigned long long below = ~0ull >> (63 - lane);
  int prev[9];
  unsigned open = 0x1FFu;
  for (int pb = wbase - 64; pb >= (wbase & ~(kJobsPerScanBlock - 1)) && open; pb -= 64) {
    const fme_job pj = load_job(a, pb + lane);
    const bool wr = nn_writes_c(pj);
    const int np = wr ? nn_pushes(pj) : 0;
#pragma unroll
    for (int f = 0; f < 9; f++) {
      const unsigned long long mask = __ballot(f < 8 ? np > f : wr);
      if ((open >> f & 1u) && mask) {
        prev[f] = pb + 63 - __clzll(mask);
        open &= ~(1u << f);
      }
    }
  }
#pragma unroll
  for (int f = 0; f < 9; f++) {
    if (open >> f & 1u) prev[f] = carry[f];
    const unsigned long long m = __ballot(run[f] >= 0) & below;
    src[f] = m ? wbase + 63 - __clzll(m) : prev[f];
  }
}

__device__ __forceinline__ void reject_job(const BatchArgs& a, const WorkBufs& w, int i, int state_in) {
  if (w.mv_out)
    w.mv_out[i].status = FME_RES_REJECTED;
  else
    a.res[i].status = FME_RES_REJECTED;
  if (i == 0)
    for (int k = 0; k < 12; k++) w.nn_state[12 * (state_in ^ 1) + k] = w.nn_state[12 * state_in + k];
}
}
```

### hm16.9-nn_fme_amd/csrc/fme_kernels.hip

```cpp
#include <hip/hip_runtime.h>

#include <algorithm>

#include "fme_device.h"
#include "fme_simd.h"

namespace fme {

__device__ __forceinline__ void luma_taps(int f, int (&c)[8]) {
  if (f == 1) {
    c[0] = -1; c[1] = 4; c[2] = -10; c[3] = 58; c[4] = 17; c[5] = -5; c[6] = 1; c[7] = 0;
  } else if (f == 2) {
    c[0] = -1; c[1] = 4; c[2] = -11; c[3] = 40; c[4] = 40; c[5] = -11; c[6] = 4; c[7] = -1;
  } else {
    c[0] = 0; c[1] = 1; c[2] = -5; c[3] = 17; c[4] = 58; c[5] = -10; c[6] = 4; c[7] = -1;
  }
}

__device__ __forceinline__ int decode_offset(uint32_t code) { return code == 1 ? -1 : (code == 2 ? 1 : 0); }
__device__ __forceinline__ int refine_dx(int half, int i) {
  (void)half;
  return decode_offset((0x666u >> (2 * (8 - i))) & 3u);
}
__device__ __forceinline__ int refine_dy(int half, int i) {
  return decode_offset(((half ? 0x605au : 0x650au) >> (2 * (8 - i))) & 3u);
}

__host__ __device__ __forceinline__ int class_of(int w, int h) {
  for (int c = 0; c < kNumClasses; c++)
    if (kClassW[c] == w && kClassH[c] == h) return c;
  return 255;
}

struct ClassLut {
  uint8_t v[256];
  constexpr ClassLut() : v() {
    for (int i = 0; i < 256; i++) v[i] = 255;
    for (int c = 0; c < kNumClasses; c++) v[((kClassW[c] >> 2) - 1) * 16 + (kClassH[c] >> 2) - 1] = (uint8_t)c;
  }
};
__constant__ ClassLut kClassLut = ClassLut();

struct FrontTables {
  uint8_t lut[256];
  int32_t pic_w[FME_MAX_PICTURES], pic_h[FME_MAX_PICTURES];
  int32_t keys_bad;
};
constexpr int kFrontQ = kJobsPerScanBlock / kBlock;

__device__ __forceinline__ void front_load(const BatchArgs& a, const WorkBufs& w, int base, fme_job (&jb)[kFrontQ]) {
  const int tid = threadIdx.x;
  if (a.pjobs) {
    job_u4 row[kFrontQ];
#pragma unroll
    for (int q = 0; q < kFrontQ; q++) {
      const int i = base + q * kBlock + tid;
      row[q] = job_u4{0u, 0u, 0u, 0u};
      if (i < a.n) row[q] = packed_row(a, i);
    }
#pragma unroll
    for (int q = 0; q < kFrontQ; q++) {
      const int i = base + q * kBlock + tid;
      const bool keyed_q = i < a.n && packed_keyed(row[q].y);
      int ko = -1;
      if (__ballot(keyed_q)) {
        const int wh = (int)((((row[q].x >> 22) & 15u) + 1u) * 4u) * (int)((((row[q].x >> 26) & 15u) + 1u) * 4u);
        const int lane = tid & 63;
        int s = keyed_q ? wh : 0;
#pragma unroll
        for (int off = 1; off < 64; off <<= 1) {
          const int o = __shfl_up(s, off, 64);
          if (lane >= off) s += o;
        }
        if (keyed_q) {
          ko = a.key_base[i >> 6] + s - wh;
          w.koff[i] = ko;
        }
      }
      jb[q] = expand_job(row[q], ko);
    }
  } else {
#pragma unroll
    for (int q = 0; q < kFrontQ; q++) {
      const int i = base + q * kBlock + tid;
      if (i < a.n) jb[q] = load_job(a, i);
    }
  }
}

__device__ __forceinline__ void front_tables(const BatchArgs& a, FrontTables& T) {
  const int tid = threadIdx.x;
  if (tid == 0) T.keys_bad = a.key_invalid ? *a.key_invalid : 0;
  T.lut[tid] = kClassLut.v[tid];
  if (tid < FME_MAX_PICTURES) {
    const PicDesc p = a.pics[tid];
    T.pic_w[tid] = p.luma ? p.width : -1;
    T.pic_h[tid] = p.height;
  }
}

__device__ __forceinline__ int front_class(const BatchArgs& a, const FrontTables& T, const fme_job& j, int i) {
  const int c = ((j.w | j.h) & 3) == 0 && j.w >= 4 && j.w <= 64 && j.h >= 4 && j.h <= 64
                    ? T.lut[((j.w >> 2) - 1) * 16 + (j.h >> 2) - 1] : 255;
  bool ok = j.ref_id < FME_MAX_PICTURES && j.lambda_id < FME_MAX_LAMBDAS && T.pic_w[j.ref_id] >= 0;
  if (ok) {
    if (j.key_offset >= 0) {
      ok = (int64_t)j.key_offset + (int64_t)j.w * j.h <= a.n_keys && T.keys_bad == 0;
    } else {
      ok = j.org_id < FME_MAX_PICTURES && T.pic_w[j.org_id] >= 0 &&
           (int)j.x + j.w <= T.pic_w[j.org_id] && (int)j.y + j.h <= T.pic_h[j.org_id];
    }
  }
  if ((j.flags & FME_JOB_NN_IN) && (!a.nn_in || i >= a.nn_in_cap)) ok = false;
  return ok ? c : 255;
}

__device__ __forceinline__ void front_writers(const fme_job& j, int i, int (&mx)[9]) {
  if (!nn_writes_c(j)) return;
  const int np = nn_pushes(j);
#pragma unroll
  for (int s = 0; s < 8; s++)
    if (np > s) mx[s] = max(mx[s], i);
  mx[8] = max(mx[8], i);
}

__global__ __launch_bounds__(kBlock) void k_classify(BatchArgs a, WorkBufs w) {
  __shared__ FrontTables T;
  __shared__ int32_t hist[kNumClasses + 1];
  __shared__ int32_t agg[9];
  __shared__ int32_t keyed;
  const int tid = threadIdx.x;
  const int base = blockIdx.x * kJobsPerScanBlock;
  fme_job jb[kFrontQ];
  front_load(a, w, base, jb);
  front_tables(a, T);
  if (tid == 0) keyed = 0;
  if (tid < kNumClasses + 1) hist[tid] = 0;
  if (tid < 9) agg[tid] = -1;
  __syncthreads();
  int mx[9];
#pragma unroll
  for (int f = 0; f < 9; f++) mx[f] = -1;
#pragma unroll
  for (int q = 0; q < kFrontQ; q++) {
    const int i = base + q * kBlock + tid;
    if (i < a.n) {
      const fme_job& j = jb[q];
      const int c = front_class(a, T, j, i);
      w.cls[i] = (uint8_t)c;
      atomicAdd(&hist[c == 255 ? kNumClasses : c], 1);
      if (j.key_offset >= 0) atomicAdd(&keyed, 1);
      front_writers(j, i, mx);
    }
  }
#pragma unroll
  for (int f = 0; f < 9; f++)
    if (mx[f] >= 0) atomicMax(&agg[f], mx[f]);
  __syncthreads();
  if (tid < kNumClasses + 1 && hist[tid]) atomicAdd(&w.counts[tid], hist[tid]);
  if (tid == 0 && keyed) atomicAdd(&w.counts[kKeyedWord], keyed);
  if (tid < 9) w.blk_agg[blockIdx.x * 9 + tid] = agg[tid];
}

__device__ __forceinline__ int wave_excl_scan(int v) {
  const int lane = (int)threadIdx.x & 63;
  int s = v;
#pragma unroll
  for (int off = 1; off < 64; off <<= 1) {
    const int o = __shfl_up(s, off, 64);
    if (lane >= off) s += o;
  }
  return s - v;
}

__device__ __forceinline__ int build_schedule(int cnt, int inv, const SchedParams& p, Schedule* sc, bool publish, int cap) {
  const int c = (int)threadIdx.x & 63;
  const int off = cap > 0 ? c * cap : wave_excl_scan(cnt);
  if (!publish) return off;
  const int nb = cnt > 0 ? (int)(((long long)cnt * p.lanes[c < kNumClasses ? c : 0] + 63) / 64) : 0;
  if (c < kNumClasses) {
    sc->class_off[c] = off;
    sc->class_cnt[c] = cnt;
  }
  {
    const int ex = wave_excl_scan(nb);
    if (c <= kNumClasses) sc->prefix[c] = ex;
  }
  auto band_lo = [&](int B) { return (int)(((long long)nb * B) / 8); };
#pragma unroll 1
  for (int x = 0; x < 8; x++) {
    const int mine_c = c < kNumClasses ? band_lo(x + 1) - band_lo(x) : 0;
    const int mine = __shfl(mine_c, c < kNumClasses ? lane_class_at(c) : c);
    const int ex = wave_excl_scan(mine);
    if (c <= kNumClasses) sc->xq[x][c] = ex;
  }
  if (c == 0) sc->invalid = inv;
  return off;
}

__device__ __forceinline__ int ld_agent(const int32_t* p) {
  return __hip_atomic_load(p, __ATOMIC_RELAXED, __HIP_MEMORY_SCOPE_AGENT);
}
__device__ __forceinline__ void st_agent(int32_t* p, int v) {
  __hip_atomic_store(p, v, __ATOMIC_RELAXED, __HIP_MEMORY_SCOPE_AGENT);
}

constexpr int kPfxAhead = 4;
__device__ __forceinline__ void front_agg_load(const WorkBufs& w, int b, int b1, int (&v)[kPfxAhead][9]) {
#pragma unroll
  for (int k = 0; k < kPfxAhead; k++) {
#pragma unroll
    for (int f = 0; f < 9; f++) v[k][f] = b + k < b1 ? ld_agent(w.blk_agg + (b + k) * 9 + f) : -1;
  }
}
__device__ __forceinline__ void front_blk_prefix(const WorkBufs& w, int nb) {
  __shared__ int32_t red[kBlock / 64][9];
  const int tid = threadIdx.x, lane = tid & 63, wv = tid >> 6;
  const int per = (nb + kBlock - 1) / kBlock;
  const int b0 = min(tid * per, nb), b1 = min(b0 + per, nb);
  int m[9], v[kPfxAhead][9];
#pragma unroll
  for (int f = 0; f < 9; f++) m[f] = -1;
  for (int b = b0; b < b1 || b == b0; b += kPfxAhead) {
    front_agg_load(w, b, b1, v);
#pragma unroll
    for (int k = 0; k < kPfxAhead; k++) {
#pragma unroll
      for (int f = 0; f < 9; f++) m[f] = max(m[f], v[k][f]);
    }
  }
  int run[9];
#pragma unroll
  for (int f = 0; f < 9; f++) {
    int s = m[f];
#pragma unroll
    for (int off = 1; off < 64; off <<= 1) {
      const int o = __shfl_up(s, off, 64);
      if (lane >= off) s = max(s, o);
    }
    if (lane == 63) red[wv][f] = s;
    const int e = __shfl_up(s, 1, 64);
    run[f] = lane ? e : -1;
  }
  __syncthreads();
#pragma unroll
  for (int f = 0; f < 9; f++)
    for (int q = 0; q < wv; q++) run[f] = max(run[f], red[q][f]);
  for (int b = b0; b < b1; b += kPfxAhead) {
    if (per > kPfxAhead) front_agg_load(w, b, b1, v);
#pragma unroll
    for (int k = 0; k < kPfxAhead; k++) {
      if (b + k < b1) {
#pragma unroll
        for (int f = 0; f < 9; f++) {
          w.blk_prefix[(b + k) * 9 + f] = run[f];
          run[f] = max(run[f], v[k][f]);
        }
      }
    }
  }
}

__global__ __launch_bounds__(kBlock) void k_front(BatchArgs a, WorkBufs w, SchedParams sp) {
  constexpr int kSeg = kFrontQ * (kBlock / 64);
  __shared__ FrontTables T;
  __shared__ int32_t seg[kSeg][kNumClasses + 1];
  __shared__ int32_t basep[kNumClasses];
  __shared__ int32_t agg[9];
  __shared__ int32_t keyed, last;
  const int tid = threadIdx.x, lane = tid & 63;
  const int base = blockIdx.x * kJobsPerScanBlock;
  fme_job jb[kFrontQ];
  front_load(a, w, base, jb);
  front_tables(a, T);
  if (tid == 0) keyed = 0;
  for (int k = tid; k < kSeg * (kNumClasses + 1); k += kBlock) (&seg[0][0])[k] = 0;
  if (tid < 9) agg[tid] = -1;
  __syncthreads();
  int mx[9], cls[kFrontQ], rank[kFrontQ];
#pragma unroll
  for (int f = 0; f < 9; f++) mx[f] = -1;
  int nkeyed = 0;
#pragma unroll
  for (int q = 0; q < kFrontQ; q++) {
    const int i = base + q * kBlock + tid;
    const bool valid = i < a.n;
    cls[q] = kNumClasses;
    rank[q] = 0;
    if (valid) {
      const fme_job& j = jb[q];
      const int c = front_class(a, T, j, i);
      w.cls[i] = (uint8_t)c;
      cls[q] = c == 255 ? kNumClasses : c;
      front_writers(j, i, mx);
    }
    nkeyed += __popcll(__ballot(valid && jb[q].key_offset >= 0));
    int32_t* sg = seg[q * (kBlock / 64) + (tid >> 6)];
    unsigned long long rem = __ballot(valid);
    while (rem) {
      const int cl = __shfl(cls[q], __ffsll((long long)rem) - 1);
      const unsigned long long m = __ballot(valid && cls[q] == cl);
      if (valid && cls[q] == cl) {
        rank[q] = __popcll(m & ((1ull << lane) - 1ull));
        if (rank[q] == 0) sg[cl] = __popcll(m);
      }
      rem &= ~m;
    }
  }
  if (lane == 0 && nkeyed) atomicAdd(&keyed, nkeyed);
#pragma unroll
  for (int f = 0; f < 9; f++) {
#pragma unroll
    for (int off = 32; off >= 1; off >>= 1) mx[f] = max(mx[f], __shfl_xor(mx[f], off));
  }
  if (lane < 9) {
    int v = mx[0];
#pragma unroll
    for (int f = 1; f < 9; f++) v = lane == f ? mx[f] : v;
    if (v >= 0) atomicMax(&agg[lane], v);
  }
  __syncthreads();
  if (tid < kNumClasses + 2) {
    int tot = keyed;
    if (tid < kNumClasses + 1) {
      tot = 0;
      for (int s = 0; s < kSeg; s++) {
        const int t = seg[s][tid];
        seg[s][tid] = tot;
        tot += t;
      }
    }
    const int old = tot ? atomicAdd(&w.cursor[tid], tot) : 0;
    if (tid < kNumClasses) basep[tid] = old;
  } else if (tid >= 64 && tid < 64 + 9) {
    st_agent(w.blk_agg + blockIdx.x * 9 + tid - 64, agg[tid - 64]);
  }
  asm volatile("s_waitcnt vmcnt(0)" ::: "memory");
  __syncthreads();
  if (tid == 0)
    last = __hip_atomic_fetch_add(&w.counts[kTicketWord], 1, __ATOMIC_RELAXED, __HIP_MEMORY_SCOPE_AGENT) == (int)gridDim.x - 1;
#pragma unroll
  for (int q = 0; q < kFrontQ; q++) {
    const int i = base + q * kBlock + tid;
    const int c = cls[q];
    if (c < kNumClasses)
      w.perm[(size_t)c * w.perm_cap + basep[c] + seg[q * (kBlock / 64) + (tid >> 6)][c] + rank[q]] = i;
  }
  __syncthreads();
  if (!last) return;
  if (tid == 0) {
    __builtin_amdgcn_fence(__ATOMIC_ACQUIRE, "agent");
    asm volatile("s_waitcnt vmcnt(0)" ::: "memory");
  }
  __syncthreads();
  int inv = 0, tot = 0;
  if (tid < 64) {
    inv = ld_agent(w.cursor + kNumClasses);
    tot = tid < kNumClasses ? ld_agent(w.cursor + tid) : 0;
  } else if (tid < 64 + kCountWords) {
    w.counts_next[tid - 64] = 0;
  }
  front_blk_prefix(w, (int)gridDim.x);
  if (tid < 64) build_schedule(inv == 0 ? tot : 0, inv, sp, w.sched, true, w.perm_cap);
}

__global__ __launch_bounds__(kBlock) void k_scatter(BatchArgs a, WorkBufs w, SchedParams sp) {
  __shared__ int32_t cnt[kNumClasses], basep[kNumClasses], class_off[kNumClasses];
  const int tid = threadIdx.x;
  const int base = blockIdx.x * kJobsPerScanBlock;
  int rank[kJobsPerScanBlock / kBlock];
  int cls[kJobsPerScanBlock / kBlock];
#pragma unroll
  for (int q = 0; q < kJobsPerScanBlock / kBlock; q++) {
    const int i = base + q * kBlock + tid;
    cls[q] = 255;
    if (i < a.n) cls[q] = w.cls[i];
  }
  if (tid < 64) {
    const int inv = w.counts[kNumClasses];
    const int off = build_schedule((tid < kNumClasses && inv == 0) ? w.counts[tid] : 0, inv, sp, w.sched, blockIdx.x == 0, 0);
    if (tid < kNumClasses) class_off[tid] = off;
  } else if (blockIdx.x == 0 && tid < 64 + kCountWords) {
    w.counts_next[tid - 64] = 0;
  }
  if (w.counts[kNumClasses]) return;
  if (tid < kNumClasses) cnt[tid] = 0;
  __syncthreads();
#pragma unroll
  for (int q = 0; q < kJobsPerScanBlock / kBlock; q++)
    if (cls[q] < kNumClasses) rank[q] = atomicAdd(&cnt[cls[q]], 1);
  __syncthreads();
  if (tid < kNumClasses) basep[tid] = cnt[tid] ? atomicAdd(&w.cursor[tid], cnt[tid]) : 0;
  __syncthreads();
#pragma unroll
  for (int q = 0; q < kJobsPerScanBlock / kBlock; q++) {
    const int i = base + q * kBlock + tid;
    if (cls[q] < kNumClasses) w.perm[class_off[cls[q]] + basep[cls[q]] + rank[q]] = i;
  }
}

enum {
  P_EMB0 = 0, P_EMB1 = 32, P_W1 = 64, P_W2 = 438, P_W3 = 878, P_B1 = 1858, P_G1 = 1880,
  P_BE1 = 1902, P_B2 = 1924, P_G2 = 1944, P_BE2 = 1964, P_BOUT = 1984, P_GIN = 2033,
  P_MEAN = 2042, P_STD = 2051
};


void nn_pack(const float* P, float* Q) {
  for (int i = 0; i < kNnPkFloats; i++) Q[i] = 0.0f;
  for (int rh = 0; rh < 8; rh++)
    for (int rw = 0; rw < 8; rw++)
      for (int r = 0; r < 22; r++) {
        float s = 0.0f;
        for (int k = 0; k < 4; k++) s = s + P[P_W1 + r * 17 + k] * P[P_EMB0 + rh * 4 + k];
        for (int k = 0; k < 4; k++) s = s + P[P_W1 + r * 17 + 4 + k] * P[P_EMB1 + rw * 4 + k];
        Q[kNnPkPfx + (rh * 8 + rw) * 22 + r] = s;
      }
  for (int r = 0; r < 22; r++)
    for (int k = 0; k < 9; k++) Q[kNnPkW1 + ((r / 2) * 9 + k) * 2 + (r & 1)] = P[P_W1 + r * 17 + 8 + k];
  for (int r = 0; r < 20; r++)
    for (int k = 0; k < 22; k++) Q[kNnPkW2 + ((r / 2) * 22 + k) * 2 + (r & 1)] = P[P_W2 + r * 22 + k];
  for (int r = 0; r < 49; r++)
    for (int k = 0; k < 20; k++) Q[kNnPkW3 + ((r / 2) * 20 + k) * 2 + (r & 1)] = P[P_W3 + r * 20 + k];
  for (int r = 0; r < 22; r++) {
    Q[kNnPkB1 + r] = P[P_B1 + r];
    Q[kNnPkG1 + r] = P[P_G1 + r];
    Q[kNnPkBE1 + r] = P[P_BE1 + r];
  }
  for (int r = 0; r < 20; r++) {
    Q[kNnPkB2 + r] = P[P_B2 + r];
    Q[kNnPkG2 + r] = P[P_G2 + r];
    Q[kNnPkBE2 + r] = P[P_BE2 + r];
  }
  for (int r = 0; r < 49; r++) Q[kNnPkBout + r] = P[P_BOUT + r];
  for (int k = 0; k < 9; k++) {
    Q[kNnPkGin + k] = P[P_GIN + k];
    Q[kNnPkMean + k] = P[P_MEAN + k];
    Q[kNnPkStd + k] = P[P_STD + k];
  }
}


__device__ __forceinline__ int nn_forward(const float* __restrict__ Q, const uint32_t (&e)[8], uint32_t c, int pu_h,
                                          int pu_w) {
  const int t = emb_row_h(pu_h) * 8 + emb_row_w(pu_w);
  float in[9];
  const uint32_t raw[9] = {e[0], e[1], e[2], e[3], c, e[4], e[5], e[6], e[7]};
#pragma unroll
  for (int k = 0; k < 9; k++) {
    float v = (float)raw[k];
    v = (v - Q[kNnPkMean + k]) / Q[kNnPkStd + k];
    in[k] = v * Q[kNnPkGin + k];
  }
  const float* pfx = Q + kNnPkPfx + t * 22;
  f2 x1[11];
#pragma unroll
  for (int rp = 0; rp < 11; rp++) {
    f2 s = {pfx[2 * rp], pfx[2 * rp + 1]};
#pragma unroll
    for (int k = 0; k < 9; k++) s = s + ld2(Q, kNnPkW1 + (rp * 9 + k) * 2) * (f2){in[k], in[k]};
    s = relu2(s + ld2(Q, kNnPkB1 + 2 * rp));
    x1[rp] = s * ld2(Q, kNnPkG1 + 2 * rp) + ld2(Q, kNnPkBE1 + 2 * rp);
  }
  f2 x2[10];
#pragma unroll
  for (int rp = 0; rp < 10; rp++) {
    f2 s = {0.0f, 0.0f};
#pragma unroll
    for (int k = 0; k < 22; k++) {
      const float xk = (k & 1) ? x1[k / 2].y : x1[k / 2].x;
      s = s + ld2(Q, kNnPkW2 + (rp * 22 + k) * 2) * (f2){xk, xk};
    }
    s = relu2(s + ld2(Q, kNnPkB2 + 2 * rp));
    x2[rp] = s * ld2(Q, kNnPkG2 + 2 * rp) + ld2(Q, kNnPkBE2 + 2 * rp);
  }
  int best = 0;
  float bv = 0.0f;
#pragma unroll 1
  for (int rp = 0; rp < 25; rp++) {
    f2 s = {0.0f, 0.0f};
#pragma unroll
    for (int k = 0; k < 20; k++) {
      const float xk = (k & 1) ? x2[k / 2].y : x2[k / 2].x;
      s = s + ld2(Q, kNnPkW3 + (rp * 20 + k) * 2) * (f2){xk, xk};
    }
    s = s + ld2(Q, kNnPkBout + 2 * rp);
    if (rp == 0 || s.x > bv) {
      bv = s.x;
      best = 2 * rp;
    }
    if (rp < 24 && s.y > bv) {
      bv = s.y;
      best = 2 * rp + 1;
    }
  }
  return best;
}

typedef uint32_t u32x4 __attribute__((ext_vector_type(4)));

__device__ __forceinline__ void tail_job(const BatchArgs& a, const WorkBufs& w, const float* __restrict__ nnp_g,
                                         int state_in, int i, const fme_job& j, const int (&src)[9], u32x4 r0,
                                         u32x4 r1, u32x4 r2, u32x4 r3) {
  const uint32_t* st_in = w.nn_state + 12 * state_in;
  uint32_t* st_out = w.nn_state + 12 * (state_in ^ 1);
  fme_result* r = a.res + i;
  const fme_result* sr = search_rec(a, w, i);
  const double ml = a.mlambda[j.lambda_id];
  const int mvx = (int16_t)(r0.x & 0xFFFF), mvy = (int16_t)(r0.x >> 16);
  const uint32_t own_emi[8] = {r1.w, r2.x, r2.y, r2.z, r2.w, r3.x, r3.y, r3.z};
  const uint32_t own_c = r1.z, own_n_emi = r3.w & 0xFF, frac_cost = r0.w;
  int offx, offy, cls = 255;
  uint16_t status = 0;
  if (a.nn_mode) {
    uint32_t e[8];
    uint32_t written = st_in[11];
#pragma unroll
    for (int s = 0; s < 8; s++) {
      if (src[s] == i) {
        e[s] = own_emi[s];
        written |= 1u << s;
      } else if (src[s] >= 0) {
        e[s] = search_rec(a, w, src[s])->emi[s];
        written |= 1u << s;
      } else {
        e[s] = st_in[s];
      }
    }
    uint32_t c, ph, pw;
    if (src[8] == i) {
      c = own_c;
      ph = j.h;
      pw = j.w;
      written |= 0x100u;
    } else if (src[8] >= 0) {
      c = search_rec(a, w, src[8])->c;
      load_job_wh(a, src[8], pw, ph);
      written |= 0x100u;
    } else {
      c = st_in[8];
      ph = st_in[9];
      pw = st_in[10];
    }
    cls = nn_forward(nnp_g, e, c, (int)ph, (int)pw);
    if (!nn_writes_c(j) || own_n_emi < 8) status |= FME_RES_NN_STALE;
    if ((written & 0x1FFu) != 0x1FFu) status |= FME_RES_NN_UNINIT;
    offx = cls % 7 - 3;
    offy = cls / 7 - 3;
    if (i == a.n - 1) {
#pragma unroll
      for (int s = 0; s < 8; s++) st_out[s] = e[s];
      st_out[8] = c;
      st_out[9] = ph;
      st_out[10] = pw;
      st_out[11] = written;
    }
  } else {
    const int8_t hx = (int8_t)(r0.z & 0xFF), hy = (int8_t)((r0.z >> 8) & 0xFF);
    const int8_t qx = (int8_t)((r0.z >> 16) & 0xFF), qy = (int8_t)(r0.z >> 24);
    offx = 2 * hx + qx;
    offy = 2 * hy + qy;
  }
  const int fx = 4 * mvx + offx, fy = 4 * mvy + offy;
  const uint32_t mvb = simd::mv_bits(fx, fy, 0, j.mvp_x, j.mvp_y);
  const uint32_t bits = (uint32_t)j.bits_in + mvb;
  const double fw = (j.flags & FME_JOB_BIPRED) ? 0.5 : 1.0;
  const double val = floor(fw * ((double)frac_cost - (double)simd::mv_cost(ml, mvb))) + (double)simd::mv_cost(ml, bits);
  store_outputs(r, sr, w.mv_out, i, fx, fy, (uint32_t)(int64_t)val, bits, (uint8_t)cls, status);
}

constexpr int kTailNT = 64;

__global__ __launch_bounds__(kTailNT) __attribute__((amdgpu_waves_per_eu(4, 4)))
void k_nn_tail(BatchArgs a, WorkBufs w, const float* __restrict__ nnp_g, int state_in) {
  const int wbase = (int)blockIdx.x * kTailNT;
  const int i = wbase + (int)threadIdx.x;
  const bool valid = i < a.n;
  if (w.sched->invalid) {
    if (valid) reject_job(a, w, i, state_in);
    return;
  }
  fme_job j{};
  u32x4 r0{}, r1{}, r2{}, r3{};
  if (valid) {
    j = load_job(a, i);
    const u32x4* rb = reinterpret_cast<const u32x4*>(search_rec(a, w, i));
    r0 = rb[0];
    r1 = rb[1];
    r2 = rb[2];
    r3 = rb[3];
  }
  int run[9];
  {
    const bool wr = valid && nn_writes_c(j);
    const int np = wr ? nn_pushes(j) : 0;
#pragma unroll
    for (int s = 0; s < 8; s++) run[s] = (np > s) ? i : -1;
    run[8] = wr ? i : -1;
  }
  int src[9];
  writer_scan_wave(a, run, w.blk_prefix + (wbase / kJobsPerScanBlock) * 9, wbase, src);
  if (valid) tail_job(a, w, nnp_g, state_in, i, j, src, r0, r1, r2, r3);
}


static int nblocks(int n) { return (n + kJobsPerScanBlock - 1) / kJobsPerScanBlock; }

hipError_t launch_front(const BatchArgs& a, const WorkBufs& w, const SchedParams& p, hipStream_t s) {
  hipLaunchKernelGGL(k_front, dim3(nblocks(a.n)), dim3(kBlock), 0, s, a, w, p);
  return hipGetLastError();
}

hipError_t launch_classify(const BatchArgs& a, const WorkBufs& w, hipStream_t s) {
  hipLaunchKernelGGL(k_classify, dim3(nblocks(a.n)), dim3(kBlock), 0, s, a, w);
  return hipGetLastError();
}

struct State12 {
  uint32_t v[12];
};
__global__ void k_put_state(uint32_t* dst, State12 st) {
  if (threadIdx.x < 12) dst[threadIdx.x] = st.v[threadIdx.x];
}

__global__ __launch_bounds__(256) void k_put_tables(PicDesc* __restrict__ pics, double* __restrict__ ml,
                                                    const TablesSlot* __restrict__ t) {
  const int i = threadIdx.x;
  if (i < FME_MAX_PICTURES) pics[i] = t->pics[i];
  if (i < FME_MAX_LAMBDAS) ml[i] = t->ml[i];
}

hipError_t launch_put_tables(PicDesc* d_pics, double* d_ml, const TablesSlot* t_dev, hipStream_t s) {
  hipLaunchKernelGGL(k_put_tables, dim3(1), dim3(256), 0, s, d_pics, d_ml, t_dev);
  return hipGetLastError();
}

hipError_t launch_put_state(uint32_t* dst, const uint32_t* v12, hipStream_t s) {
  State12 st;
  for (int k = 0; k < 12; k++) st.v[k] = v12[k];
  hipLaunchKernelGGL(k_put_state, dim3(1), dim3(64), 0, s, dst, st);
  return hipGetLastError();
}

hipError_t launch_scatter(const BatchArgs& a, const WorkBufs& w, const SchedParams& p, hipStream_t s) {
  hipLaunchKernelGGL(k_scatter, dim3(nblocks(a.n)), dim3(kBlock), 0, s, a, w, p);
  return hipGetLastError();
}

SchedParams sched_params() {
  SchedParams p{};
  for (int c = 0; c < kNumClasses; c++) p.lanes[c] = lane_lanes_per_pu(c);
  return p;
}

int cu_count(int device) {
  int v = 0;
  if (hipDeviceGetAttribute(&v, hipDeviceAttributeMultiprocessorCount, device) != hipSuccess || v <= 0) v = 256;
  return v;
}

constexpr int kDlThreads = 256;
__device__ __forceinline__ void dl_store(u32x4* p, u32x4 v) { __builtin_nontemporal_store(v, p); }
__global__ __launch_bounds__(kDlThreads) void k_download(const u32x4* __restrict__ src, u32x4* dst, long n16) {
  const long stride = (long)gridDim.x * kDlThreads;
  long i = (long)blockIdx.x * kDlThreads + threadIdx.x;
  for (; i + 3 * stride < n16; i += 4 * stride) {
    const u32x4 a = src[i], b = src[i + stride], c = src[i + 2 * stride], d = src[i + 3 * stride];
    dl_store(dst + i, a);
    dl_store(dst + i + stride, b);
    dl_store(dst + i + 2 * stride, c);
    dl_store(dst + i + 3 * stride, d);
  }
  for (; i < n16; i += stride) dl_store(dst + i, src[i]);
}

__global__ __launch_bounds__(kBlock) void k_gather_jobs(const fme_job* __restrict__ src,
                                                       const fme_tz_ext* __restrict__ src_ext,
                                                       const int32_t* __restrict__ idx, fme_job* __restrict__ dst,
                                                       fme_tz_ext* __restrict__ dst_ext, int n) {
  const int q = blockIdx.x * kBlock + threadIdx.x;
  if (q >= n) return;
  const int u = idx[q];
  dst[q] = src[u];
  if (dst_ext) dst_ext[q] = src_ext[u];
}

hipError_t launch_gather_jobs(const fme_job* src, const fme_tz_ext* src_ext, const int32_t* idx, fme_job* dst,
                              fme_tz_ext* dst_ext, int n, hipStream_t s) {
  if (n <= 0) return hipSuccess;
  hipLaunchKernelGGL(k_gather_jobs, dim3((n + kBlock - 1) / kBlock), dim3(kBlock), 0, s, src, src_ext, idx, dst,
                     dst_ext, n);
  return hipGetLastError();
}

hipError_t launch_download(const void* src, void* dst, size_t n16, int wgs, hipStream_t s) {
  const long need = (long)((n16 + kDlThreads - 1) / kDlThreads);
  const int g = (int)std::min<long>(wgs, std::max<long>(need, 1));
  hipLaunchKernelGGL(k_download, dim3(g), dim3(kDlThreads), 0, s, static_cast<const u32x4*>(src),
                     static_cast<u32x4*>(dst), (long)n16);
  return hipGetLastError();
}

hipError_t launch_nn_tail(const BatchArgs& a, const WorkBufs& w, const float* nn_params,
                          int state_in, hipStream_t s) {
  const int nb = (a.n + kTailNT - 1) / kTailNT;
  hipLaunchKernelGGL(k_nn_tail, dim3(nb), dim3(kTailNT), 0, s, a, w, nn_params, state_in);
  return hipGetLastError();
}

}
```

### hm16.9-nn_fme_amd/csrc/fme_overlap_host.h

```cpp
#pragma once

#include <cstdint>

namespace fme {

constexpr int kOvSlots = 2;
constexpr int kOvBlocks = 4;

enum : uint32_t {
  kOvKeys = 1u << 0,
  kOvDeepNn = 1u << 1,
  kOvPx = 1u << 2,
  kOvStaged = 1u << 3,
  kOvGrow = 1u << 4,
  kOvForeign = 1u << 5,
  kOvFill = 1u << 6,
};

struct OverlapPlan {
  int slot = 0;
  int block = 0;
  int block_zeroed = 0;
  bool serial = false;
  bool fill_blocks = false;
  bool wait_slot = false;
  bool wait_prev_front = false;
  bool wait_prev_tail = false;
};

struct OverlapState {
  long long seq = 0;
  bool dirty = false;
  const void* stream[2] = {nullptr, nullptr};
  bool live[2] = {false, false};
  uint32_t prev_features = 0;
};

inline OverlapPlan overlap_plan(const OverlapState& st, const void* stream, uint32_t features) {
  OverlapPlan p;
  p.slot = (int)(st.seq % kOvSlots);
  p.block = (int)(st.seq % kOvBlocks);
  p.block_zeroed = (int)((st.seq + 2) % kOvBlocks);
  p.fill_blocks = st.dirty;
  p.serial = features != 0 || st.dirty || st.prev_features != 0;
  const bool other1 = st.live[0] && st.stream[0] != stream;
  const bool other2 = st.live[1] && st.stream[1] != stream;
  p.wait_slot = other2;
  p.wait_prev_front = p.serial && other1;
  p.wait_prev_tail = other1 && !p.wait_prev_front;
  return p;
}

inline void overlap_begin(OverlapState& st) { st.dirty = true; }

inline void overlap_commit(OverlapState& st, const void* stream, uint32_t features, const OverlapPlan& plan) {
  st.seq++;
  st.prev_features = features | (plan.fill_blocks ? (uint32_t)kOvFill : 0u);
  st.dirty = false;
  st.stream[1] = st.stream[0];
  st.live[1] = st.live[0];
  st.stream[0] = stream;
  st.live[0] = true;
}

}
```

### hm16.9-nn_fme_amd/nnfme/pipeline.py

```python
import ctypes
import sys
import time

import numpy as np

from . import dist as fdist
from .abi import JOB_DTYPE, MV_RESULT_DTYPE

_hip = None


def _hip_lib():
    global _hip
    if _hip is None:
        h = ctypes.CDLL("libamdhip64.so.7")
        h.hipMemcpyAsync.argtypes = [ctypes.c_void_p, ctypes.c_void_p, ctypes.c_size_t, ctypes.c_int, ctypes.c_void_p]
        h.hipMemcpyAsync.restype = ctypes.c_int
        h.hipEventCreateWithFlags.argtypes = [ctypes.POINTER(ctypes.c_void_p), ctypes.c_uint]
        h.hipEventCreateWithFlags.restype = ctypes.c_int
        h.hipEventDestroy.argtypes = [ctypes.c_void_p]
        h.hipEventDestroy.restype = ctypes.c_int
        h.hipStreamWaitEvent.argtypes = [ctypes.c_void_p, ctypes.c_void_p, ctypes.c_uint]
        h.hipStreamWaitEvent.restype = ctypes.c_int
        _hip = h
    return _hip


SLOW_CALLS = []


def _memcpy_async(dst, src, nbytes, kind, stream):
    t0 = time.perf_counter()
    rc = _hip_lib().hipMemcpyAsync(dst.data_ptr(), src.data_ptr(), nbytes, kind, stream.cuda_stream)
    dt = (time.perf_counter() - t0) * 1e3
    if dt > 1.0:
        SLOW_CALLS.append(("hipMemcpyAsync kind %d" % kind, int(nbytes), round(dt, 3)))
    if rc != 0:
        raise RuntimeError(f"hipMemcpyAsync failed ({rc})")


def _timed(what, f):
    t0 = time.perf_counter()
    f()
    dt = (time.perf_counter() - t0) * 1e3
    if dt > 1.0:
        SLOW_CALLS.append((what, 0, round(dt, 3)))


class _RawEvent:

    def __init__(self):
        ev = ctypes.c_void_p()
        if _hip_lib().hipEventCreateWithFlags(ctypes.byref(ev), 2) != 0:
            raise RuntimeError("hipEventCreateWithFlags failed")
        self.cuda_event = ev.value

    def wait(self, stream):
        if _hip_lib().hipStreamWaitEvent(stream.cuda_stream, self.cuda_event, 0) != 0:
            raise RuntimeError("hipStreamWaitEvent failed")

    def destroy(self):
        if self.cuda_event and _hip is not None:
            _hip.hipEventDestroy(self.cuda_event)
        self.cuda_event = None

    def __del__(self):
        if sys.is_finalizing() or not self.cuda_event or _hip is None:
            return
        try:
            _hip.hipEventDestroy(self.cuda_event)
        except Exception:
            pass


H2D, D2H = 1, 2
D2D_NOCU = 1024


def torch_current_stream(t):
    import torch
    return torch.cuda.current_stream(t.device)


ORG0 = 32
REFS = 4


def group_jobs(base, frames, key_count=0):
    out = []
    for j in range(frames):
        g = np.array(base, dtype=JOB_DTYPE, copy=True)
        g["org_id"] = ORG0 + j
        g["ref_id"] = j + 3 - base["ref_id"].astype(np.int64)
        g["lambda_id"] = j
        bi = g["key_offset"] >= 0
        g["key_offset"][bi] += j * key_count
        out.append(g)
    return np.concatenate(out)


def group_key_reqs(base, frames, key_count):
    from .abi import BIKEY_REQ_DTYPE
    out = []
    for j in range(frames):
        g = np.array(base, dtype=BIKEY_REQ_DTYPE, copy=True)
        g["org_id"] = ORG0 + j
        g["ref_id"] = j + 3 - base["ref_id"].astype(np.int64)
        g["key_offset"] += j * key_count
        out.append(g)
    return np.concatenate(out)


class FrameReplay:
    def __init__(self, ctx, base_jobs, pool, lambda_of, n_steps, frames_per_step=1, world=1, rank=0, device=None,
                 group=None, defer_download=True, key_reqs=None, key_count=0, nn_rows=None,
                 download_engine="sdma", download_wgs=8, search_reserve=0, packed=True, copy_streams=1, slots=3,
                 max_ahead=4, precreate_events=True, warm_engines=True, timeline=False, compute_streams=2):
        import torch
        from .abi import JOB_PACKED_DTYPE
        from .runtime import FmeError, pack_jobs
        self.torch, self.ctx = torch, ctx
        self.world, self.rank, self.group = world, rank, group
        self.F = F = frames_per_step
        self.R = R = int(slots)
        if R < 2:
            raise ValueError("slots >= 2")
        self.lambda_of = lambda_of
        self.steps = n_steps
        P, H, W = pool.shape
        self.P, self.H, self.W = P, H, W
        if pool.dtype not in (np.uint8, np.uint16):
            raise ValueError(f"frame pool dtype {pool.dtype}: uint8 or uint16 (main10) samples")
        self.bps = pool.dtype.itemsize
        pdt = torch.uint8 if self.bps == 1 else torch.int16
        host = np.ascontiguousarray(pool).view(np.uint8 if self.bps == 1 else np.int16)
        self.pool = torch.from_numpy(host).pin_memory()
        self.key_count = int(key_count)
        self.jobs = group_jobs(base_jobs, F, self.key_count)
        self.n = n = len(self.jobs)
        self.packed, self.packed_reason = bool(packed), None
        if self.packed:
            try:
                pk, kb = pack_jobs(self.jobs)
            except FmeError as e:
                self.packed, self.packed_reason = False, str(e)
        if self.packed:
            self.h_jobs = torch.from_numpy(pk.view(np.uint8).copy()).pin_memory()
            self.h_kb = torch.from_numpy(kb.view(np.uint8).copy()).pin_memory()
            self.d_kb = [torch.empty(self.h_kb.numel(), dtype=torch.uint8, device=device) for _ in range(R)]
            assert self.h_jobs.numel() == n * JOB_PACKED_DTYPE.itemsize
        else:
            self.h_jobs = torch.from_numpy(self.jobs.view(np.uint8).copy()).pin_memory()
        self.job_bytes = self.h_jobs.numel() + (self.h_kb.numel() if self.packed else 0)
        self.d_jobs = [torch.empty(self.h_jobs.numel(), dtype=torch.uint8, device=device) for _ in range(R)]
        self.kreqs = None
        if key_reqs is not None and len(key_reqs):
            self.kreqs = group_key_reqs(key_reqs, F, self.key_count)
            self.h_kreqs = torch.from_numpy(self.kreqs.view(np.uint8).copy()).pin_memory()
            self.d_kreqs = [torch.empty(self.h_kreqs.numel(), dtype=torch.uint8, device=device) for _ in range(R)]
        self.rows = None
        if nn_rows is not None:
            self.rows = np.tile(np.ascontiguousarray(nn_rows, dtype=np.uint32).reshape(-1, 9), (F, 1))
            assert len(self.rows) == n
            self.h_rows = torch.from_numpy(self.rows.view(np.uint8).copy()).pin_memory()
            self.d_rows = [torch.empty(self.h_rows.numel(), dtype=torch.uint8, device=device) for _ in range(R)]
        self.d_out = [torch.empty(n * MV_RESULT_DTYPE.itemsize, dtype=torch.uint8, device=device) for _ in range(R)]
        self.h_out = torch.empty((n_steps, n * MV_RESULT_DTYPE.itemsize), dtype=torch.uint8).pin_memory()
        frames = n_steps * world * F
        self.recon = torch.empty((frames + REFS, H, W), dtype=pdt, device=device)
        self.org = torch.empty((n_steps * F, H, W), dtype=pdt, device=device)
        self.states = torch.zeros((n_steps, 12), dtype=torch.int32, device=device)
        self.s_comp = torch.cuda.default_stream(device)
        if compute_streams not in (1, 2):
            raise ValueError("compute_streams 1 or 2")
        self.compute_streams = compute_streams
        self.s_comps = [self.s_comp] + [torch.cuda.Stream(device) for _ in range(compute_streams - 1)]
        self.s_copy = torch.cuda.Stream(device)
        if copy_streams not in (1, 2):
            raise ValueError("copy_streams 1 or 2")
        self.copy_streams = copy_streams
        self.s_down = self.s_copy if copy_streams == 1 else torch.cuda.Stream(device)
        self.uploaded = -1
        self.ev_in = [torch.cuda.Event() for _ in range(n_steps)]
        self.ev_comp = [torch.cuda.Event() for _ in range(n_steps)]
        self.ev_out = [torch.cuda.Event() for _ in range(n_steps)]
        self.ev_search = [_RawEvent() for _ in range(n_steps)]
        if precreate_events:
            for e in self.ev_in + self.ev_comp + self.ev_out:
                e.record(self.s_copy)
            self.s_copy.synchronize()
        self.defer_download = defer_download
        if download_engine not in ("kernel", "blit", "sdma"):
            raise ValueError(f"download_engine {download_engine!r}")
        self.download_engine, self.download_wgs = download_engine, int(download_wgs)
        ctx.set_search_reserve(int(search_reserve))
        ctx.set_search_event(None)
        self.pending = None
        self.fixed_jobs = 0
        self.last_prefix = 0
        self.r_out = {}
        self.max_ahead = int(max_ahead)
        self.host_ms = []
        self.host_seg = []
        self.host_seg_names = ("upload", "waits", "bind", "refine", "prefetch", "download")
        self.warm_engines = bool(warm_engines)
        self.engines_warmed = None
        self.tl = None
        if timeline:
            self.tl = {kk: [torch.cuda.Event(enable_timing=True) for _ in range(n_steps)]
                       for kk in ("up0", "up1", "b0", "b1", "d0", "d1")}
            self.tl_base = torch.cuda.Event(enable_timing=True)

    def h2d_bytes_per_step(self):
        b = self.job_bytes + 2 * self.F * self.H * self.W * self.bps
        if self.kreqs is not None:
            b += self.h_kreqs.numel()
        if self.rows is not None:
            b += self.h_rows.numel()
        return b

    def close(self):
        try:
            self.ctx.set_search_event(None)
        except Exception:
            pass
        for sc in self.s_comps:
            sc.synchronize()
        for e in self.ev_search:
            e.destroy()
        self.ev_search = []

    def comp_stream(self, k):
        return self.s_comps[k % len(self.s_comps)]

    def first_frame(self, k):
        return (k * self.world + self.rank) * self.F

    def _publish(self, g, src_rank):
        dst = self.recon[g + REFS]
        if self.rank == src_rank:
            _memcpy_async(dst, self.pool[g % self.P], self.H * self.W * self.bps, H2D, torch_current_stream(dst))
        if self.world > 1:
            import torch.distributed as dist
            if dist.get_backend(self.group) == "gloo":
                tmp = dst.cpu()
                dist.broadcast(tmp, src=src_rank, group=self.group)
                dst.copy_(tmp, non_blocking=False)
            else:
                dist.broadcast(dst, src=src_rank, group=self.group)

    def rank_of_frame(self, g):
        return (g // self.F) % self.world

    def readers(self, h):
        frames = self.steps * self.world * self.F
        out = []
        for d in range(1, REFS + 1):
            f = h + d
            if 0 <= f < frames:
                r = self.rank_of_frame(f)
                if r not in out:
                    out.append(r)
        return out

    def _exchange(self, k, stream):
        import torch.distributed as dist
        F, W = self.F, self.world
        base = k * W * F
        gloo = dist.get_backend(self.group) == "gloo"
        ops, fixups = [], []
        for r in range(W):
            for j in range(F):
                h = base + r * F - 1 + j
                dsts = [d for d in self.readers(h) if d != r]
                if self.rank == r:
                    buf = self.recon[h + REFS]
                    if gloo:
                        stream.synchronize()
                        buf = buf.cpu()
                    for d in dsts:
                        ops.append(dist.P2POp(dist.isend, buf, d, group=self.group))
                elif self.rank in dsts:
                    buf = self.recon[h + REFS]
                    if gloo:
                        tmp = self.torch.empty_like(buf, device="cpu")
                        fixups.append((buf, tmp))
                        buf = tmp
                    ops.append(dist.P2POp(dist.irecv, buf, r, group=self.group))
        if ops:
            for w in dist.batch_isend_irecv(ops):
                w.wait()
        for dst, tmp in fixups:
            dst.copy_(tmp, non_blocking=False)

    def _upload_run(self, dst, d0, g0, count, stream):
        i = 0
        while i < count:
            s = (g0 + i) % self.P
            run = min(count - i, self.P - s)
            _memcpy_async(dst[d0 + i], self.pool[s], run * self.H * self.W * self.bps, H2D, stream)
            i += run

    def _publish_run(self, g0, count, src_rank, stream):
        if self.rank == src_rank:
            self._upload_run(self.recon, g0 + REFS, g0, count, stream)

    def prime(self):
        if self.warm_engines:
            self.engines_warmed = self.ctx.warm_copy_engines()
        with self.torch.cuda.stream(self.s_copy):
            for g in range(-REFS, -1):
                self._publish(g, 0)
        for k in range(self.steps):
            self._copy_down(k, self.s_down)
        self.s_copy.synchronize()
        self.s_down.synchronize()

    def _refine(self, k, out_ptr, n, stream):
        b = k % self.R
        if self.packed:
            self.ctx.refine_mv_packed_device(self.d_jobs[b].data_ptr(), self.d_kb[b].data_ptr(), out_ptr, n,
                                             stream.cuda_stream)
        else:
            self.ctx.refine_mv_device(self.d_jobs[b].data_ptr(), out_ptr, n, stream.cuda_stream)

    def bind_rows(self, b):
        if self.rows is not None:
            self.ctx.set_nn_inputs(self.d_rows[b].data_ptr(), self.n)

    def _bind(self, k):
        ctx, W, H, F = self.ctx, self.W, self.H, self.F
        self.bind_rows(k % self.R)
        f0 = self.first_frame(k)
        for j in range(F):
            ctx.bind_picture_device(ORG0 + j, self.org[k * F + j].data_ptr(), W, W, H)
            ctx.set_lambda(j, self.lambda_of(f0 + j))
        for s in range(F + REFS - 1):
            ctx.bind_picture_device(s, self.recon[f0 - REFS + s + REFS].data_ptr(), W, W, H)

    def _upload(self, k):
        F, R = self.F, self.R
        b = k % R
        f0 = self.first_frame(k)
        cp = self.s_copy
        with self.torch.cuda.stream(cp):
            if k >= R:
                _timed("copy stream wait_event", lambda: cp.wait_event(self.ev_comp[k - R]))
            if self.tl:
                self.tl["up0"][k].record(cp)
            _memcpy_async(self.d_jobs[b], self.h_jobs, self.h_jobs.numel(), H2D, cp)
            if self.packed:
                _memcpy_async(self.d_kb[b], self.h_kb, self.h_kb.numel(), H2D, cp)
            if self.rows is not None:
                _memcpy_async(self.d_rows[b], self.h_rows, self.h_rows.numel(), H2D, cp)
            if self.kreqs is not None:
                _memcpy_async(self.d_kreqs[b], self.h_kreqs, self.h_kreqs.numel(), H2D, cp)
            self._upload_run(self.org, k * F, f0, F, cp)
            base = k * self.world * F
            self._publish_run(base + self.rank * F - 1, F, self.rank, cp)
            if self.world > 1:
                self._exchange(k, cp)
            if self.tl:
                self.tl["up1"][k].record(cp)
            _timed("ev_in record", lambda: self.ev_in[k].record(cp))
        self.uploaded = k

    def issue(self, k, prefetch=True):
        pc = time.perf_counter
        t = [pc()]
        ctx = self.ctx
        b = k % self.R
        if self.max_ahead > 0 and k >= self.max_ahead:
            self.ev_comp[k - self.max_ahead].synchronize()
        if self.uploaded < k:
            self._upload(k)
        t.append(pc())
        comp = self.comp_stream(k)
        comp.wait_event(self.ev_in[k])
        if k >= self.R:
            comp.wait_event(self.ev_out[k - self.R])
        t.append(pc())
        self._bind(k)
        if self.kreqs is not None:
            ctx.build_bipred_keys_device(self.d_kreqs[b].data_ptr(), len(self.kreqs), self.key_count * self.F,
                                         comp.cuda_stream)
        if self.world > 1:
            ctx.nn_reset()
        if self.defer_download:
            ctx.set_search_event(self.ev_search[k])
        t.append(pc())
        if self.tl:
            self.tl["b0"][k].record(comp)
        self._refine(k, self.d_out[b].data_ptr(), self.n, comp)
        if self.world > 1:
            ctx.nn_copy_state_device(self.states[k].data_ptr(), comp.cuda_stream)
        if self.tl:
            self.tl["b1"][k].record(comp)
        self.ev_comp[k].record(comp)
        t.append(pc())
        if prefetch and k + 1 < self.steps:
            self._upload(k + 1)
        t.append(pc())
        if not self.defer_download:
            self._download(k, self.ev_comp[k])
        else:
            if self.pending is not None:
                self._download(self.pending, self.ev_search[k] if self.n > 0 else None)
            self.pending = k
        t.append(pc())
        self.host_ms.append((t[-1] - t[0]) * 1e3)
        self.host_seg.append([round((t[i + 1] - t[i]) * 1e3, 3) for i in range(len(t) - 1)])

    def _copy_down(self, k, dn):
        b = k % self.R
        if self.download_engine == "kernel":
            self.ctx.download_device(self.d_out[b].data_ptr(), self.h_out[k].data_ptr(), self.h_out.shape[1],
                                     self.download_wgs, dn.cuda_stream)
        elif self.download_engine == "sdma":
            _memcpy_async(self.h_out[k], self.d_out[b], self.h_out.shape[1], D2D_NOCU, dn)
        else:
            _memcpy_async(self.h_out[k], self.d_out[b], self.h_out.shape[1], D2H, dn)

    def _download(self, k, after):
        dn = self.s_down
        if isinstance(after, _RawEvent):
            after.wait(dn)
        elif after is not None:
            dn.wait_event(after)
        if after is not self.ev_comp[k]:
            dn.wait_event(self.ev_comp[k])
        if self.tl:
            self.tl["d0"][k].record(dn)
        self._copy_down(k, dn)
        if self.tl:
            self.tl["d1"][k].record(dn)
        self.ev_out[k].record(dn)

    def drain(self):
        if self.pending is not None:
            self._download(self.pending, self.ev_comp[self.pending])
            self.pending = None
        self.s_copy.synchronize()
        for sc in self.s_comps:
            sc.synchronize()
        self.s_down.synchronize()
        self.ctx.set_search_event(None)

    def check_status(self, first_step=0):
        from .abi import RES_REJECTED
        for k in range(first_step, self.steps):
            if np.any(self.results(k)["status"] & RES_REJECTED):
                raise RuntimeError(f"frame replay: step {k}'s batch was rejected on the device")

    def timeline_start(self):
        if self.tl:
            self.tl_base.record(self.s_comp)

    def timeline_rows(self, k0, k1):
        rows = []
        for k in range(k0, k1):
            r = {"step": k}
            for kk in ("up0", "up1", "b0", "b1", "d0", "d1"):
                r[kk] = round(self.tl_base.elapsed_time(self.tl[kk][k]), 4)
            rows.append(r)
        return rows

    def results(self, k):
        return self.h_out[k].numpy().view(MV_RESULT_DTYPE)

    def resident_outputs(self, k0, k1):
        torch = self.torch
        dev = self.d_out[0].device
        self.r_out = {k: torch.empty(self.n * MV_RESULT_DTYPE.itemsize, dtype=torch.uint8, device=dev)
                      for k in range(k0, k1)}

    def _resident_batch(self, k, n):
        ctx, comp = self.ctx, self.comp_stream(k)
        b = k % self.R
        self._bind(k)
        if self.kreqs is not None:
            ctx.build_bipred_keys_device(self.d_kreqs[b].data_ptr(), len(self.kreqs), self.key_count * self.F,
                                         comp.cuda_stream)
        self._refine(k, self.r_out[k].data_ptr(), n, comp)

    def issue_resident(self, k):
        ctx, comp = self.ctx, self.comp_stream(k)
        ctx.set_search_event(None)
        if self.world > 1:
            ctx.nn_reset()
        self._resident_batch(k, self.n)
        if self.world > 1:
            ctx.nn_copy_state_device(self.states[k].data_ptr(), comp.cuda_stream)

    def finish_resident(self, k0, k1, prefix):
        if self.world == 1 or prefix <= 0:
            return 0
        import torch.distributed as dist
        torch = self.torch
        for sc in self.s_comps:
            sc.synchronize()
        st = self.states if dist.get_backend(self.group) != "gloo" else self.states.cpu()
        gathered = [torch.zeros_like(st) for _ in range(self.world)]
        dist.all_gather(gathered, st, group=self.group)
        bs = np.zeros((self.steps * self.world, 12), np.uint32)
        for r in range(self.world):
            g = gathered[r].cpu().numpy().view(np.uint32)
            for k in range(self.steps):
                bs[k * self.world + r] = g[k]
        carries, _ = fdist.chain_states(bs)
        fixed = 0
        for k in range(k0, k1):
            carry = carries[k * self.world + self.rank]
            if not int(carry[11]):
                continue
            self.ctx.nn_set_state(carry)
            self._resident_batch(k, prefix)
            fixed += prefix
        return fixed

    def finish(self, first_step=0):
        torch = self.torch
        self.drain()
        if self.world == 1:
            return 0
        import torch.distributed as dist
        st = self.states if dist.get_backend(self.group) != "gloo" else self.states.cpu()
        gathered = [torch.zeros_like(st) for _ in range(self.world)]
        dist.all_gather(gathered, st, group=self.group)
        bs = np.zeros((self.steps * self.world, 12), np.uint32)
        for r in range(self.world):
            g = gathered[r].cpu().numpy().view(np.uint32)
            for k in range(self.steps):
                bs[k * self.world + r] = g[k]
        carries, _ = fdist.chain_states(bs)
        fixed = 0
        ctx, comp = self.ctx, self.s_comp
        for k in range(first_step, self.steps):
            out = self.results(k)
            p = fdist.uninit_prefix(out)
            self.last_prefix = max(self.last_prefix, p)
            carry = carries[k * self.world + self.rank]
            if p == 0 or not int(carry[11]):
                continue
            with torch.cuda.stream(comp):
                self._bind(k)
                if self.kreqs is not None:
                    ctx.build_bipred_keys(self.kreqs, self.key_count * self.F, comp.cuda_stream)
                ctx.nn_set_state(carry)
                out[:p] = ctx.refine_mv(self.jobs[:p], comp.cuda_stream)
            fixed += p
        self.fixed_jobs = fixed
        return fixed
```

Measured before the change: 917.1 million.

## Deepen batch overlap to three compute streams with per-batch tables ring

Widens the cross-batch overlap from two to three in-flight batches. Scan and schedule buffers now rotate over a four-entry ring, and a new search-end event lets batch N wait only on batch N-2's search instead of its full completion. Picture and lambda tables are now passed as kernel arguments to the front kernel, which writes them into a per-ring device copy. This removes the separate put_tables launch and its host-mapped staging from the batch path. The Python pipeline defaults to three compute streams and lags downloads by two steps. The cost is more events, more buffer memory and more complex dependency logic, with some risk of ordering bugs.

```diff
diff --git a/hm16.9-nn_fme_amd/csrc/fme_api.cpp b/hm16.9-nn_fme_amd/csrc/fme_api.cpp
--- a/hm16.9-nn_fme_amd/csrc/fme_api.cpp
+++ b/hm16.9-nn_fme_amd/csrc/fme_api.cpp
@@ -47,14 +47,15 @@
   std::unique_ptr<fme_ctx> c(new fme_ctx());
   c->device = device;
   c->cfg = *cfg;
-  HIP_TRY(c->d_pics.reserve(kOvSlots * FME_MAX_PICTURES));
-  HIP_TRY(c->d_mlambda.reserve(kOvSlots * FME_MAX_LAMBDAS));
+  HIP_TRY(c->d_pics.reserve((1 + kOvRing) * FME_MAX_PICTURES));
+  HIP_TRY(c->d_mlambda.reserve((1 + kOvRing) * FME_MAX_LAMBDAS));
   HIP_TRY(c->d_nn.reserve(kNnPkFloats));
   HIP_TRY(c->counts.reserve(kOvBlocks * kCountWords));
   HIP_TRY(hipMemset(c->counts.p, 0, kOvBlocks * kCountWords * sizeof(int32_t)));
-  HIP_TRY(c->d_sched.reserve(kOvSlots));
-  HIP_TRY(hipMemset(c->d_sched.p, 0, kOvSlots * sizeof(Schedule)));
+  HIP_TRY(c->d_sched.reserve(kOvRing));
+  HIP_TRY(hipMemset(c->d_sched.p, 0, kOvRing * sizeof(Schedule)));
   for (auto& e : c->done_ev) HIP_TRY(hipEventCreateWithFlags(&e, hipEventDisableTiming));
+  for (auto& e : c->search_ev) HIP_TRY(hipEventCreateWithFlags(&e, hipEventDisableTiming));
   c->sched_p = sched_params();
   {
     const char* m10 = std::getenv("FME_MAIN10_SEARCH");
@@ -72,8 +73,10 @@
     for (int b = 0; b < kOvSlots; b++) {
       HIP_TRY(c->cls[b].reserve(n));
       HIP_TRY(c->perm[b].reserve(n * kNumClasses));
-      HIP_TRY(c->blk_agg[b].reserve(nb * 9));
-      HIP_TRY(c->blk_prefix[b].reserve(nb * 9));
+    }
+    for (int r = 0; r < kOvRing; r++) {
+      HIP_TRY(c->blk_agg[r].reserve(nb * 9));
+      HIP_TRY(c->blk_prefix[r].reserve(nb * 9));
     }
   }
   *out_ctx = c.release();
@@ -83,11 +86,15 @@
 }
 static int srv_stop(fme_ctx* c);
 static hipEvent_t done_event(const fme_ctx* c, int back) {
-  if (back < 1 || back > 2 || !c->ov.live[back - 1]) return nullptr;
+  if (back < 1 || back > kOvBack || !c->ov.live[back - 1]) return nullptr;
   return c->done_ev[(c->ov.seq - back) % fme_ctx::kDoneRing];
 }
+static hipEvent_t search_event(const fme_ctx* c, int back) {
+  if (back < 1 || back > kOvBack || !c->ov.live[back - 1]) return nullptr;
+  return c->search_ev[(c->ov.seq - back) % fme_ctx::kDoneRing];
+}
 static int wait_batches(fme_ctx* c, hipStream_t s) {
-  for (int back = 1; back <= 2; back++)
+  for (int back = 1; back <= kOvBack; back++)
     if (hipEvent_t e = done_event(c, back))
       if (c->ov.stream[back - 1] != s) HIP_TRY(hipStreamWaitEvent(s, e, 0));
   return FME_OK;
@@ -147,11 +154,16 @@
   c->d_pics.release(); c->d_mlambda.release(); c->d_keys.release(); c->d_nn.release(); c->d_net.release();
   c->d_jobs.release(); c->d_res.release(); c->d_res1.release(); c->d_mv.release();
   for (int b = 0; b < kOvSlots; b++) {
-    c->koff[b].release(); c->cls[b].release(); c->perm[b].release(); c->blk_agg[b].release(); c->blk_prefix[b].release();
+    c->cls[b].release(); c->perm[b].release();
+  }
+  for (int r = 0; r < kOvRing; r++) {
+    c->koff[r].release(); c->blk_agg[r].release(); c->blk_prefix[r].release();
   }
   c->counts.release(); c->nn_state.release();
   c->d_sched.release();
   for (auto& e : c->done_ev)
+    if (e) (void)hipEventDestroy(e);
+  for (auto& e : c->search_ev)
     if (e) (void)hipEventDestroy(e);
   for (auto& e : c->state_read_ev)
     if (e) (void)hipEventDestroy(e);
@@ -442,27 +454,29 @@
   for (int b = 0; b < kOvSlots; b++) {
     HIP_TRY(c->cls[b].reserve(n));
     HIP_TRY(c->perm[b].reserve((size_t)n * kNumClasses));
-    HIP_TRY(c->blk_agg[b].reserve(nb * 9));
-    HIP_TRY(c->blk_prefix[b].reserve(nb * 9));
-    HIP_TRY(c->koff[b].reserve(n));
-  }
-  return FME_OK;
-}
-
-static WorkBufs work_bufs(fme_ctx* c, int slot, int block, int zeroed) {
+  }
+  for (int r = 0; r < kOvRing; r++) {
+    HIP_TRY(c->blk_agg[r].reserve(nb * 9));
+    HIP_TRY(c->blk_prefix[r].reserve(nb * 9));
+    HIP_TRY(c->koff[r].reserve(n));
+  }
+  return FME_OK;
+}
+
+static WorkBufs work_bufs(fme_ctx* c, const OverlapPlan& plan) {
   WorkBufs w{};
-  w.cls = c->cls[slot].p;
-  w.perm = c->perm[slot].p;
-  w.perm_cap = (int32_t)(c->perm[slot].cap / kNumClasses);
-  w.koff = c->koff[slot].p;
-  w.counts = c->counts.p + block * kCountWords;
-  w.counts_next = c->counts.p + zeroed * kCountWords;
+  w.cls = c->cls[plan.slot].p;
+  w.perm = c->perm[plan.slot].p;
+  w.perm_cap = (int32_t)(c->perm[plan.slot].cap / kNumClasses);
+  w.koff = c->koff[plan.ring].p;
+  w.counts = c->counts.p + plan.block * kCountWords;
+  w.counts_next = c->counts.p + plan.block_zeroed * kCountWords;
   w.cursor = w.counts + kCursorWord;
   w.tile_ctr = w.counts + kTileCtrWord;
-  w.blk_agg = c->blk_agg[slot].p;
-  w.blk_prefix = c->blk_prefix[slot].p;
+  w.blk_agg = c->blk_agg[plan.ring].p;
+  w.blk_prefix = c->blk_prefix[plan.ring].p;
   w.nn_state = c->nn_state.p;
-  w.sched = c->d_sched.p + slot;
+  w.sched = c->d_sched.p + plan.ring;
   w.mv_out = nullptr;
   return w;
 }
@@ -481,14 +495,18 @@
   return a;
 }
 
-static int put_tables(fme_ctx* c, int slot, hipStream_t s) {
+static int enter_stream(fme_ctx* c, hipStream_t s) {
   note_stream(c, s);
-  FME_TRY(srv_stop(c));
+  return srv_stop(c);
+}
+
+static int put_tables(fme_ctx* c, hipStream_t s) {
+  FME_TRY(enter_stream(c, s));
   if (c->tables_dirty) {
     c->tab_gen++;
     c->tables_dirty = false;
   }
-  if (c->slot_gen[slot] == c->tab_gen) return FME_OK;
+  if (c->shared_gen == c->tab_gen) return FME_OK;
   if (!c->h_tab) {
     void* p = nullptr;
     HIP_TRY(hipHostMalloc(&p, fme_ctx::kTabSlots * sizeof(TablesSlot), hipHostMallocMapped));
@@ -503,26 +521,32 @@
   if (c->tab_used[k]) HIP_TRY(hipEventSynchronize(c->tab_ev[k]));
   std::memcpy(c->h_tab[k].pics, c->pics, sizeof(c->pics));
   std::memcpy(c->h_tab[k].ml, c->mlambda, sizeof(c->mlambda));
-  HIP_TRY(launch_put_tables(c->d_pics.p + slot * FME_MAX_PICTURES, c->d_mlambda.p + slot * FME_MAX_LAMBDAS,
-                            c->h_tab_dev + k, s));
+  HIP_TRY(launch_put_tables(c->d_pics.p, c->d_mlambda.p, c->h_tab_dev + k, s));
   HIP_TRY(hipEventRecord(c->tab_ev[k], s));
   c->tab_used[k] = true;
-  c->slot_gen[slot] = c->tab_gen;
+  c->shared_gen = c->tab_gen;
   return FME_OK;
 }
 
 int fme::sync_tables(fme_ctx* c, hipStream_t s) {
   FME_TRY(wait_batches(c, s));
-  return put_tables(c, 0, s);
-}
-
-static int batch_begin(fme_ctx* c, const OverlapPlan& plan, hipStream_t s, hipEvent_t* done) {
-  hipEvent_t const prev_done = done_event(c, 1), slot_done = done_event(c, 2);
+  return put_tables(c, s);
+}
+
+static int batch_begin(fme_ctx* c, const OverlapPlan& plan, hipStream_t s, hipEvent_t* search_end, hipEvent_t* done) {
+  *search_end = c->search_ev[c->ov.seq % fme_ctx::kDoneRing];
   *done = c->done_ev[c->ov.seq % fme_ctx::kDoneRing];
   if (c->ov.seq >= fme_ctx::kDoneRing)
-    HIP_TRY(hipEventSynchronize(c->done_ev[(c->ov.seq + 2) % fme_ctx::kDoneRing]));
-  if (plan.wait_prev_front) HIP_TRY(hipStreamWaitEvent(s, prev_done, 0));
-  if (plan.wait_slot) HIP_TRY(hipStreamWaitEvent(s, slot_done, 0));
+    HIP_TRY(hipEventSynchronize(c->done_ev[(c->ov.seq + kOvBack) % fme_ctx::kDoneRing]));
+  if (plan.serial) {
+    if (plan.wait_prev_front) HIP_TRY(hipStreamWaitEvent(s, done_event(c, 1), 0));
+    if (plan.wait_slot) HIP_TRY(hipStreamWaitEvent(s, done_event(c, 2), 0));
+    if (plan.wait_back3) HIP_TRY(hipStreamWaitEvent(s, done_event(c, 3), 0));
+  } else if (plan.wait_front) {
+    HIP_TRY(hipStreamWaitEvent(s, search_event(c, 2), 0));
+  } else if (plan.wait_front_end) {
+    HIP_TRY(hipStreamWaitEvent(s, done_event(c, 2), 0));
+  }
   if (plan.fill_blocks) {
     FME_TRY(drain_ctx(c));
     HIP_TRY(hipMemsetAsync(c->counts.p, 0, kOvBlocks * kCountWords * sizeof(int32_t), s));
@@ -579,22 +603,28 @@
                             (c->cfg.bit_depth > 8 && c->main10_px ? kOvPx : 0u) |
                             (d_jobs && d_jobs == c->d_jobs.p ? kOvStaged : 0u) | (grows ? kOvGrow : 0u);
   const OverlapPlan plan = overlap_plan(c->ov, s, features);
-  hipEvent_t const prev_done = done_event(c, 1);
-  hipEvent_t done = nullptr;
-  FME_TRY(batch_begin(c, plan, s, &done));
-  FME_TRY(put_tables(c, plan.slot, s));
-
+  hipEvent_t const prev_done = done_event(c, 1), slot_done = done_event(c, 2);
+  hipEvent_t search_end = nullptr, done = nullptr;
+  FME_TRY(enter_stream(c, s));
+  FME_TRY(batch_begin(c, plan, s, &search_end, &done));
+
+  PicDesc* const d_pics = c->d_pics.p + (1 + plan.ring) * FME_MAX_PICTURES;
+  double* const d_ml = c->d_mlambda.p + (1 + plan.ring) * FME_MAX_LAMBDAS;
+  BatchTables tab;
+  for (int i = 0; i < FME_MAX_PICTURES; i++)
+    tab.pics[i] = BatchPic{c->pics[i].luma, c->pics[i].stride, c->pics[i].width, c->pics[i].height, 0};
+  std::memcpy(tab.ml, c->mlambda, sizeof(c->mlambda));
   BatchArgs a = batch_args(c, d_jobs, n);
-  a.pics = c->d_pics.p + plan.slot * FME_MAX_PICTURES;
-  a.mlambda = c->d_mlambda.p + plan.slot * FME_MAX_LAMBDAS;
+  a.pics = d_pics;
+  a.mlambda = d_ml;
   a.pjobs = d_jobs ? nullptr : d_pjobs;
   a.key_base = d_key_base;
-  a.koff = c->koff[plan.slot].p;
+  a.koff = c->koff[plan.ring].p;
   a.res = d_res;
   a.nn_mode = c->cfg.nn_mode ? 1 : 0;
   a.nn_in = c->nn_in;
   a.nn_in_cap = c->nn_in_cap;
-  WorkBufs w = work_bufs(c, plan.slot, plan.block, plan.block_zeroed);
+  WorkBufs w = work_bufs(c, plan);
   w.mv_out = d_mv;
 
   const bool prof = c->profiling;
@@ -611,8 +641,9 @@
     HIP_TRY(hipEventRecord(ev[0], s));
   }
   overlap_begin(c->ov);
-  HIP_TRY(launch_front(a, w, c->sched_p, s));
+  HIP_TRY(launch_front(a, w, c->sched_p, tab, d_pics, d_ml, s));
   if (prof) HIP_TRY(hipEventRecord(ev[3], s));
+  if (plan.wait_search) HIP_TRY(hipStreamWaitEvent(s, slot_done, 0));
   if (c->ev_search) HIP_TRY(hipEventRecord(c->ev_search, s));
   if (c->cfg.bit_depth > 8) {
     if (c->main10_px)
@@ -623,6 +654,7 @@
     HIP_TRY(launch_search_lane(a, w, c->search_reserve, s));
   }
   if (prof) HIP_TRY(hipEventRecord(ev[4], s));
+  HIP_TRY(hipEventRecord(search_end, s));
   if (plan.wait_prev_tail) HIP_TRY(hipStreamWaitEvent(s, prev_done, 0));
   if (c->state_read_last) {
     if (c->state_read_stream != s) HIP_TRY(hipStreamWaitEvent(s, c->state_read_last, 0));
@@ -640,6 +672,7 @@
   HIP_TRY(hipEventRecord(done, s));
   c->ev_done = done;
   c->last_slot = plan.slot;
+  c->last_ring = plan.ring;
   c->keys_fresh = false;
   overlap_commit(c->ov, s, features, plan);
   c->batch_issued = true;
@@ -648,7 +681,7 @@
 }
 
 int fme::check_rejected(fme_ctx* c, hipStream_t s, const char* name, const char* what) {
-  HIP_TRY(hipMemcpyAsync(c->h_counts, &c->d_sched.p[c->last_slot].invalid, sizeof(int32_t), hipMemcpyDeviceToHost, s));
+  HIP_TRY(hipMemcpyAsync(c->h_counts, &c->d_sched.p[c->last_ring].invalid, sizeof(int32_t), hipMemcpyDeviceToHost, s));
   HIP_TRY(hipStreamSynchronize(s));
   if (c->h_counts[0] > 0)
     return fail(FME_E_INVALID, "%s: %d job(s) %s", name, c->h_counts[0], what);
@@ -919,7 +952,7 @@
   HIP_TRY(hipSetDevice(c->device));
   HIP_TRY(hipEventSynchronize(c->ev_done));
   int32_t v = 0;
-  HIP_TRY(hipMemcpy(&v, &c->d_sched.p[c->last_slot].invalid, sizeof(v), hipMemcpyDeviceToHost));
+  HIP_TRY(hipMemcpy(&v, &c->d_sched.p[c->last_ring].invalid, sizeof(v), hipMemcpyDeviceToHost));
   return v;
 }
 
@@ -932,7 +965,7 @@
   HIP_TRY(hipSetDevice(c->device));
   HIP_TRY(hipEventSynchronize(c->ev_done));
   if (perm_out && perm_words) HIP_TRY(hipMemcpy(perm_out, c->perm[c->last_slot].p, (size_t)perm_words * sizeof(int32_t), hipMemcpyDeviceToHost));
-  if (sched_out && sched_words) HIP_TRY(hipMemcpy(sched_out, c->d_sched.p + c->last_slot, (size_t)sched_words * sizeof(int32_t), hipMemcpyDeviceToHost));
+  if (sched_out && sched_words) HIP_TRY(hipMemcpy(sched_out, c->d_sched.p + c->last_ring, (size_t)sched_words * sizeof(int32_t), hipMemcpyDeviceToHost));
   if (cap_out) *cap_out = (int32_t)(c->perm[c->last_slot].cap / kNumClasses);
   return FME_OK;
 }
@@ -963,9 +996,9 @@
   a.nn_in = c->nn_in;
   a.nn_in_cap = c->nn_in_cap;
   const OverlapPlan plan = overlap_plan(c->ov, s, kOvForeign);
-  hipEvent_t done = nullptr;
-  FME_TRY(batch_begin(c, plan, s, &done));
-  WorkBufs w = work_bufs(c, plan.slot, plan.block, plan.block_zeroed);
+  hipEvent_t search_end = nullptr, done = nullptr;
+  FME_TRY(batch_begin(c, plan, s, &search_end, &done));
+  WorkBufs w = work_bufs(c, plan);
   if (c->profiling) {
     if (!c->ev_tz[0]) {
       HIP_TRY(hipEventCreate(&c->ev_tz[0]));
@@ -1027,6 +1060,7 @@
   HIP_TRY(hipStreamWaitEvent(s, c->ev_join2, 0));
   if (c->profiling) HIP_TRY(hipEventRecord(c->ev_tz[1], s));
   c->tz_timed = c->profiling;
+  HIP_TRY(hipEventRecord(search_end, s));
   HIP_TRY(hipEventRecord(done, s));
   overlap_commit(c->ov, s, kOvForeign, plan);
   return FME_OK;
diff --git a/hm16.9-nn_fme_amd/csrc/fme_ctx.h b/hm16.9-nn_fme_amd/csrc/fme_ctx.h
--- a/hm16.9-nn_fme_amd/csrc/fme_ctx.h
+++ b/hm16.9-nn_fme_amd/csrc/fme_ctx.h
@@ -86,7 +86,7 @@
 
   fme::DevBuf<fme::PicDesc> d_pics;
   fme::DevBuf<double> d_mlambda;
-  unsigned long long tab_gen = 1, slot_gen[fme::kOvSlots] = {};
+  unsigned long long tab_gen = 1, shared_gen = 0;
   static constexpr int kTabSlots = 16;
   fme::TablesSlot* h_tab = nullptr;
   fme::TablesSlot* h_tab_dev = nullptr;
@@ -112,20 +112,22 @@
   fme::DevBuf<fme_result> d_res;
   fme::DevBuf<fme_result> d_res1;
   fme::DevBuf<fme_mv_result> d_mv;
-  fme::DevBuf<int32_t> koff[fme::kOvSlots];
   fme::DevBuf<uint8_t> cls[fme::kOvSlots];
   fme::DevBuf<int32_t> perm[fme::kOvSlots];
-  fme::DevBuf<int32_t> blk_agg[fme::kOvSlots];
-  fme::DevBuf<int32_t> blk_prefix[fme::kOvSlots];
+  fme::DevBuf<int32_t> koff[fme::kOvRing];
+  fme::DevBuf<int32_t> blk_agg[fme::kOvRing];
+  fme::DevBuf<int32_t> blk_prefix[fme::kOvRing];
   fme::DevBuf<int32_t> counts;
   fme::OverlapState ov;
   static constexpr int kDoneRing = 16;
   hipEvent_t done_ev[kDoneRing] = {};
+  hipEvent_t search_ev[kDoneRing] = {};
   hipEvent_t state_read_ev[kDoneRing] = {};
   long long state_reads = 0;
   hipEvent_t state_read_last = nullptr;
   hipStream_t state_read_stream = nullptr;
   int last_slot = 0;
+  int last_ring = 0;
   bool keys_fresh = false;
   fme::DevBuf<uint32_t> nn_state;
   int state_cur = 0;
diff --git a/hm16.9-nn_fme_amd/csrc/fme_device.h b/hm16.9-nn_fme_amd/csrc/fme_device.h
--- a/hm16.9-nn_fme_amd/csrc/fme_device.h
+++ b/hm16.9-nn_fme_amd/csrc/fme_device.h
@@ -241,14 +241,24 @@
 };
 hipError_t launch_tz_levels(const TzArgs& ta, const TzChain& ch, const int32_t* h_lvl_off, int bit_depth, hipStream_t s);
 
-hipError_t launch_front(const BatchArgs& a, const WorkBufs& w, const SchedParams& p, hipStream_t s);
+struct TablesSlot {
+  PicDesc pics[FME_MAX_PICTURES];
+  double ml[FME_MAX_LAMBDAS];
+};
+struct BatchPic {
+  const uint8_t* luma;
+  int32_t stride, width, height;
+  int32_t pad_;
+};
+struct BatchTables {
+  BatchPic pics[FME_MAX_PICTURES];
+  double ml[FME_MAX_LAMBDAS];
+};
+hipError_t launch_front(const BatchArgs& a, const WorkBufs& w, const SchedParams& p, const BatchTables& t,
+                        PicDesc* d_pics, double* d_ml, hipStream_t s);
 hipError_t launch_classify(const BatchArgs& a, const WorkBufs& w, hipStream_t s);
 hipError_t launch_scatter(const BatchArgs& a, const WorkBufs& w, const SchedParams& p, hipStream_t s);
 hipError_t launch_put_state(uint32_t* dst, const uint32_t* v12, hipStream_t s);
-struct TablesSlot {
-  PicDesc pics[FME_MAX_PICTURES];
-  double ml[FME_MAX_LAMBDAS];
-};
 hipError_t launch_put_tables(PicDesc* d_pics, double* d_ml, const TablesSlot* t_dev, hipStream_t s);
 hipError_t launch_search_lane(const BatchArgs& a, const WorkBufs& w, int reserve, hipStream_t s);
 hipError_t launch_search_px(const BatchArgs& a, const WorkBufs& w, int bit_depth, hipStream_t s, hipStream_t s_big);
diff --git a/hm16.9-nn_fme_amd/csrc/fme_kernels.hip b/hm16.9-nn_fme_amd/csrc/fme_kernels.hip
--- a/hm16.9-nn_fme_amd/csrc/fme_kernels.hip
+++ b/hm16.9-nn_fme_amd/csrc/fme_kernels.hip
@@ -88,12 +88,13 @@
   }
 }
 
-__device__ __forceinline__ void front_tables(const BatchArgs& a, FrontTables& T) {
+template <class Pic>
+__device__ __forceinline__ void front_tables(const BatchArgs& a, const Pic* pics, FrontTables& T) {
   const int tid = threadIdx.x;
   if (tid == 0) T.keys_bad = a.key_invalid ? *a.key_invalid : 0;
   T.lut[tid] = kClassLut.v[tid];
   if (tid < FME_MAX_PICTURES) {
-    const PicDesc p = a.pics[tid];
+    const Pic p = pics[tid];
     T.pic_w[tid] = p.luma ? p.width : -1;
     T.pic_h[tid] = p.height;
   }
@@ -133,7 +134,7 @@
   const int base = blockIdx.x * kJobsPerScanBlock;
   fme_job jb[kFrontQ];
   front_load(a, w, base, jb);
-  front_tables(a, T);
+  front_tables(a, a.pics, T);
   if (tid == 0) keyed = 0;
   if (tid < kNumClasses + 1) hist[tid] = 0;
   if (tid < 9) agg[tid] = -1;
@@ -261,7 +262,11 @@
   }
 }
 
-__global__ __launch_bounds__(kBlock) void k_front(BatchArgs a, WorkBufs w, SchedParams sp) {
+static_assert(sizeof(BatchArgs) + sizeof(WorkBufs) + sizeof(SchedParams) + sizeof(BatchTables) + 2 * sizeof(void*) + 256 <= 4096,
+              "k_front's arguments and the 256 hidden bytes must fit the 4 KB kernel-argument segment");
+static_assert(FME_MAX_PICTURES <= kBlock && FME_MAX_LAMBDAS <= kBlock, "one lane per table entry");
+__global__ __launch_bounds__(kBlock) void k_front(BatchArgs a, WorkBufs w, SchedParams sp, BatchTables tab,
+                                                  PicDesc* __restrict__ d_pics, double* __restrict__ d_ml) {
   constexpr int kSeg = kFrontQ * (kBlock / 64);
   __shared__ FrontTables T;
   __shared__ int32_t seg[kSeg][kNumClasses + 1];
@@ -272,7 +277,14 @@
   const int base = blockIdx.x * kJobsPerScanBlock;
   fme_job jb[kFrontQ];
   front_load(a, w, base, jb);
-  front_tables(a, T);
+  front_tables(a, tab.pics, T);
+  if (blockIdx.x == 0) {
+    if (tid < FME_MAX_PICTURES) {
+      const BatchPic p = tab.pics[tid];
+      d_pics[tid] = PicDesc{p.luma, p.stride, p.width, p.height, nullptr, nullptr, 0, 0};
+    }
+    if (tid < FME_MAX_LAMBDAS) d_ml[tid] = tab.ml[tid];
+  }
   if (tid == 0) keyed = 0;
   for (int k = tid; k < kSeg * (kNumClasses + 1); k += kBlock) (&seg[0][0])[k] = 0;
   if (tid < 9) agg[tid] = -1;
@@ -606,8 +618,9 @@
 
 static int nblocks(int n) { return (n + kJobsPerScanBlock - 1) / kJobsPerScanBlock; }
 
-hipError_t launch_front(const BatchArgs& a, const WorkBufs& w, const SchedParams& p, hipStream_t s) {
-  hipLaunchKernelGGL(k_front, dim3(nblocks(a.n)), dim3(kBlock), 0, s, a, w, p);
+hipError_t launch_front(const BatchArgs& a, const WorkBufs& w, const SchedParams& p, const BatchTables& t,
+                        PicDesc* d_pics, double* d_ml, hipStream_t s) {
+  hipLaunchKernelGGL(k_front, dim3(nblocks(a.n)), dim3(kBlock), 0, s, a, w, p, t, d_pics, d_ml);
   return hipGetLastError();
 }
 
diff --git a/hm16.9-nn_fme_amd/csrc/fme_overlap_host.h b/hm16.9-nn_fme_amd/csrc/fme_overlap_host.h
--- a/hm16.9-nn_fme_amd/csrc/fme_overlap_host.h
+++ b/hm16.9-nn_fme_amd/csrc/fme_overlap_host.h
@@ -5,7 +5,9 @@
 namespace fme {
 
 constexpr int kOvSlots = 2;
+constexpr int kOvRing = 4;
 constexpr int kOvBlocks = 4;
+constexpr int kOvBack = 3;
 
 enum : uint32_t {
   kOvKeys = 1u << 0,
@@ -26,28 +28,40 @@
   bool wait_slot = false;
   bool wait_prev_front = false;
   bool wait_prev_tail = false;
+  int ring = 0;
+  bool wait_front = false;
+  bool wait_search = false;
+  bool wait_back3 = false;
+  bool wait_front_end = false;
 };
 
 struct OverlapState {
   long long seq = 0;
   bool dirty = false;
-  const void* stream[2] = {nullptr, nullptr};
-  bool live[2] = {false, false};
+  const void* stream[kOvBack] = {nullptr, nullptr, nullptr};
+  bool live[kOvBack] = {false, false, false};
   uint32_t prev_features = 0;
+  uint32_t prev2_features = 0;
 };
 
 inline OverlapPlan overlap_plan(const OverlapState& st, const void* stream, uint32_t features) {
   OverlapPlan p;
   p.slot = (int)(st.seq % kOvSlots);
+  p.ring = (int)(st.seq % kOvRing);
   p.block = (int)(st.seq % kOvBlocks);
   p.block_zeroed = (int)((st.seq + 2) % kOvBlocks);
   p.fill_blocks = st.dirty;
   p.serial = features != 0 || st.dirty || st.prev_features != 0;
   const bool other1 = st.live[0] && st.stream[0] != stream;
   const bool other2 = st.live[1] && st.stream[1] != stream;
+  const bool other3 = st.live[2] && st.stream[2] != stream;
   p.wait_slot = other2;
+  p.wait_front = other2 && !p.serial && st.prev2_features == 0;
+  p.wait_front_end = other2 && !p.serial && st.prev2_features != 0;
+  p.wait_search = other2 && !p.serial && !p.wait_front_end;
   p.wait_prev_front = p.serial && other1;
   p.wait_prev_tail = other1 && !p.wait_prev_front;
+  p.wait_back3 = p.serial && other3;
   return p;
 }
 
@@ -55,10 +69,13 @@
 
 inline void overlap_commit(OverlapState& st, const void* stream, uint32_t features, const OverlapPlan& plan) {
   st.seq++;
+  st.prev2_features = st.prev_features;
   st.prev_features = features | (plan.fill_blocks ? (uint32_t)kOvFill : 0u);
   st.dirty = false;
-  st.stream[1] = st.stream[0];
-  st.live[1] = st.live[0];
+  for (int b = kOvBack - 1; b > 0; b--) {
+    st.stream[b] = st.stream[b - 1];
+    st.live[b] = st.live[b - 1];
+  }
   st.stream[0] = stream;
   st.live[0] = true;
 }
diff --git a/hm16.9-nn_fme_amd/nnfme/pipeline.py b/hm16.9-nn_fme_amd/nnfme/pipeline.py
--- a/hm16.9-nn_fme_amd/nnfme/pipeline.py
+++ b/hm16.9-nn_fme_amd/nnfme/pipeline.py
@@ -115,7 +115,7 @@
     def __init__(self, ctx, base_jobs, pool, lambda_of, n_steps, frames_per_step=1, world=1, rank=0, device=None,
                  group=None, defer_download=True, key_reqs=None, key_count=0, nn_rows=None,
                  download_engine="sdma", download_wgs=8, search_reserve=0, packed=True, copy_streams=1, slots=3,
-                 max_ahead=4, precreate_events=True, warm_engines=True, timeline=False, compute_streams=2):
+                 max_ahead=4, precreate_events=True, warm_engines=True, timeline=False, compute_streams=3):
         import torch
         from .abi import JOB_PACKED_DTYPE
         from .runtime import FmeError, pack_jobs
@@ -171,8 +171,8 @@
         self.org = torch.empty((n_steps * F, H, W), dtype=pdt, device=device)
         self.states = torch.zeros((n_steps, 12), dtype=torch.int32, device=device)
         self.s_comp = torch.cuda.default_stream(device)
-        if compute_streams not in (1, 2):
-            raise ValueError("compute_streams 1 or 2")
+        if compute_streams not in (1, 2, 3):
+            raise ValueError("compute_streams 1, 2 or 3")
         self.compute_streams = compute_streams
         self.s_comps = [self.s_comp] + [torch.cuda.Stream(device) for _ in range(compute_streams - 1)]
         self.s_copy = torch.cuda.Stream(device)
@@ -195,7 +195,8 @@
         self.download_engine, self.download_wgs = download_engine, int(download_wgs)
         ctx.set_search_reserve(int(search_reserve))
         ctx.set_search_event(None)
-        self.pending = None
+        self.pending = []
+        self.download_lag = 2 if (compute_streams == 3 and R >= 3 and defer_download) else 1
         self.fixed_jobs = 0
         self.last_prefix = 0
         self.r_out = {}
@@ -404,9 +405,9 @@
         if not self.defer_download:
             self._download(k, self.ev_comp[k])
         else:
-            if self.pending is not None:
-                self._download(self.pending, self.ev_search[k] if self.n > 0 else None)
-            self.pending = k
+            self.pending.append(k)
+            while len(self.pending) > self.download_lag:
+                self._download(self.pending.pop(0), self.ev_search[k] if self.n > 0 else None)
         t.append(pc())
         self.host_ms.append((t[-1] - t[0]) * 1e3)
         self.host_seg.append([round((t[i + 1] - t[i]) * 1e3, 3) for i in range(len(t) - 1)])
@@ -437,9 +438,9 @@
         self.ev_out[k].record(dn)
 
     def drain(self):
-        if self.pending is not None:
-            self._download(self.pending, self.ev_comp[self.pending])
-            self.pending = None
+        while self.pending:
+            j = self.pending.pop(0)
+            self._download(j, self.ev_comp[j])
         self.s_copy.synchronize()
         for sc in self.s_comps:
             sc.synchronize()
```

New measurement: 935.8 million (median of 6 runs). 1.02x the previous value.
